# MinChoi0129/StreamMOS

Hardware: AMD Instinct MI355X
Metric: LiDAR scans/sec (StreamMOS streaming inference + voxel voting) (higher is better)
Workload: dtype f32; 1 GPU; configs[1]: full StreamMOS streaming inference, 1 sequence per GPU, B=4 TTA x T=3 x N=160000 padded points (120k-point synthetic HDL-64E scans), 8-frame voxel voting on; tta=4, frame_point_num=160000, parallelism=sequence-shard x1, padding_tail=point head skipped (logits zero)

## Files before the change

include/smos.h:

```cpp
#ifndef SMOS_H_
#define SMOS_H_

#include <stdint.h>

#ifdef __cplusplus
extern "C" {
#endif

#define SMOS_ABI_VERSION 4

enum smos_status {
  SMOS_OK = 0,
  SMOS_ERR_ARG = 1,
  SMOS_ERR_UNSUPPORTED = 2,
  SMOS_ERR_LAUNCH = 3
};

enum smos_dtype { SMOS_F32 = 0, SMOS_F16 = 1, SMOS_F64 = 2 };

typedef void* smos_stream_t;

int smos_abi_version(void);
const char* smos_last_error(void);
int smos_debug_set_conv_grid_cap(int32_t blocks);

int smos_voxel_maxpool_fwd(const void* feat, const int64_t* feat_stride, const void* ind, void* out,
                           const int64_t* out_stride, int64_t* voxel_max_idx, int64_t BS, int64_t C,
                           int64_t N, int32_t D, const int64_t* out_size, const float* scale,
                           int32_t dtype, int32_t* flag_ws, smos_stream_t stream);

int smos_voxel_maxpool_bwd(const void* feat, const int64_t* feat_stride, const void* ind, const void* out,
                           const void* grad_out, const int64_t* out_stride, void* grad_feat, int64_t BS,
                           int64_t C, int64_t N, int32_t D, const int64_t* out_size, const float* scale,
                           int32_t dtype, smos_stream_t stream);

int smos_bilinear_gather_fwd(const float* grid, const int64_t* grid_stride, const float* coord, int32_t K,
                             float* out, const int64_t* out_stride, int64_t B, int64_t C, int64_t H,
                             int64_t W, int64_t N, const float* scale, smos_stream_t stream);

int smos_bilinear_gather_bwd(const float* grad_out, const int64_t* grad_out_stride, const float* coord, int32_t K,
                             float* grad_grid, const int64_t* grad_grid_stride, int64_t B, int64_t C, int64_t H,
                             int64_t W, int64_t N, const float* scale, smos_stream_t stream);

int32_t smos_segsum_chunk(void);
int64_t smos_bilinear_gather_bwd_det_work_bytes(int64_t B, int64_t C, int64_t H, int64_t W, int64_t N);
int smos_bilinear_gather_bwd_det(const float* grad_out, const int64_t* grad_out_stride, const float* coord, int32_t K,
                                 float* grad_grid, const int64_t* grad_grid_stride, int64_t B, int64_t C, int64_t H,
                                 int64_t W, int64_t N, const float* scale, void* work, int64_t work_bytes,
                                 smos_stream_t stream);

int smos_gather_scatter_train_fwd(const float* grid, const int64_t* grid_stride, const float* gcoord, int32_t Kg,
                                  const float* gscale, const float* scoord, int32_t Ks, const float* sscale, float* out,
                                  const int64_t* out_stride, float* pts, const int64_t* pts_stride, int64_t B, int64_t C,
                                  int64_t Hg, int64_t Wg, int64_t N, int64_t Ho, int64_t Wo, int32_t* flag_ws,
                                  smos_stream_t stream);

int smos_gather_scatter_train_bwd(const float* grid, const int64_t* grid_stride, const float* gcoord, int32_t Kg,
                                  const float* gscale, const float* scoord, int32_t Ks, const float* sscale, const float* out,
                                  const int64_t* out_stride, const float* grad_out, const int64_t* grad_out_stride,
                                  const float* grad_pts, const int64_t* grad_pts_stride, float* grad_grid,
                                  const int64_t* grad_grid_stride, int64_t B, int64_t C, int64_t Hg, int64_t Wg, int64_t N,
                                  int64_t Ho, int64_t Wo, smos_stream_t stream);

int smos_gather_scatter_train_point_grad(const float* grid, const int64_t* grid_stride, const float* gcoord, int32_t Kg,
                                         const float* gscale, const float* scoord, int32_t Ks, const float* sscale,
                                         const float* out, const int64_t* out_stride, const float* grad_out,
                                         const int64_t* grad_out_stride, const float* grad_pts, const int64_t* grad_pts_stride,
                                         float* x, const int64_t* x_stride, int64_t B, int64_t C, int64_t Hg, int64_t Wg,
                                         int64_t N, int64_t Ho, int64_t Wo, smos_stream_t stream);

int32_t smos_seg_loss_tile(void);
int64_t smos_seg_loss_work_bytes(int64_t n, int32_t C);
int smos_seg_loss_fwd(const float* pred, const int64_t* pred_stride, const int64_t* target, int64_t B, int32_t C,
                      int64_t P, int64_t k, float top_weight, float lovasz_weight, int64_t ignore_index, float* coef,
                      float* loss, float* stats, void* work, int64_t work_bytes, smos_stream_t stream);
int smos_seg_loss_bwd(const float* pred, const int64_t* pred_stride, const int64_t* target, const float* coef,
                      const float* stats, const float* grad_out, int64_t B, int32_t C, int64_t P, int64_t k,
                      float top_weight, float lovasz_weight, int64_t ignore_index, float* grad,
                      const int64_t* grad_stride, smos_stream_t stream);

int smos_msda_fwd(const void* value, const int64_t* spatial_shapes, const int64_t* level_start_index,
                  const void* sampling_loc, const void* attn_weight, void* out, int64_t N, int64_t S,
                  int64_t M, int64_t D, int64_t L, int64_t Lq, int64_t P, int32_t dtype,
                  smos_stream_t stream);

int smos_tta_argmax(const float* pred, int64_t B, int64_t K, int64_t N, uint8_t* labels, float* prob,
                    smos_stream_t stream);

#define SMOS_VOTE_NX 512
#define SMOS_VOTE_NY 512
#define SMOS_VOTE_NZ 30
#define SMOS_VOTE_CELLS (512LL * 512LL * 30LL)

int smos_vote_clear(uint64_t* table, smos_stream_t stream);
int smos_vote_accumulate(const float* pts, int64_t n, int64_t pt_stride, const uint8_t* labels,
                         const double* pose_diff, int32_t recip_quantize, uint64_t* table,
                         smos_stream_t stream);
int smos_vote_accumulate_frames(int32_t count, const float* const* pts, const int64_t* n, const int64_t* pt_stride,
                                const uint8_t* const* labels, const double* const* pose_diff, int32_t recip_quantize,
                                uint64_t* table, smos_stream_t stream);
int smos_vote_resolve(const float* pts, int64_t n, int64_t pt_stride, const uint8_t* labels,
                      int32_t recip_quantize, const uint64_t* table, const int32_t* lut,
                      int32_t* out_labels, smos_stream_t stream);

int64_t smos_dbscan_work_bytes(int64_t n);
int smos_dbscan(const float* pts, int64_t n, int64_t pt_stride, double eps, int32_t min_samples, int32_t* labels,
                void* work, int64_t work_bytes, int32_t max_sweeps, smos_stream_t stream);
int smos_box_vote(const float* pts, int64_t n, int64_t pt_stride, const uint8_t* labels, const double* pose_diff,
                  const float* boxes, int32_t K, uint32_t* counts, smos_stream_t stream);

int64_t smos_instance_work_bytes(int64_t n);
int smos_instance_cluster(const float* pts, int64_t n, int64_t pt_stride, const uint8_t* bf, double eps,
                          int32_t min_samples, int32_t min_points, float floor_lift, int32_t max_boxes, int32_t* names,
                          float* boxes, int32_t* slot_of, int32_t* k_dev, int32_t* status, void* work, int64_t work_bytes,
                          smos_stream_t stream);
int smos_box_vote_dev(int32_t count, const float* const* pts, const int64_t* n, const int64_t* pt_stride,
                      const uint8_t* const* labels, const double* const* pose_diff, const float* boxes,
                      const int32_t* k_dev, int32_t max_boxes, uint32_t* counts, smos_stream_t stream);
int smos_instance_apply(const int32_t* names, const int32_t* slot_of, const uint32_t* counts, const int32_t* k_dev,
                        int32_t max_boxes, int32_t* labels, int64_t n, smos_stream_t stream);

int smos_pointnet_scatter(const float* xyzi, const float* coord, int32_t K, const float* w1, const float* b1,
                          const float* w2, const float* b2, float* bev, float* pts_out, int64_t po_b, int64_t po_n,
                          int64_t B, int64_t T, int64_t N, int64_t H, int64_t W, int32_t cin, int32_t cmid,
                          int32_t cout, smos_stream_t stream);
int64_t smos_stem_scan_state_words(int64_t cells);
int smos_stem_mark(const float* coord, int32_t K, int64_t B, int64_t T, int64_t N, int64_t H, int64_t W, int32_t* flags,
                   uint64_t* scan_state, smos_stream_t stream);
int smos_stem_scan(int32_t* flags, int64_t B, int64_t H, int64_t W, uint64_t* scan_state, int32_t* row_cell, int32_t* row_of,
                   int32_t* meta, float* rows, int64_t row_floats, smos_stream_t stream);
int smos_stem_gemm(const float* bev, const int32_t* row_cell, const int32_t* meta, const float* const* wprep4, float* const* y4,
                   int64_t Cin, int64_t Cout, smos_stream_t stream);
int smos_stem_epilogue(const float* const* y4, const int32_t* meta, const int32_t* row_of, const float* bias, float* out,
                       int64_t out_pitch, int64_t B, int64_t H, int64_t W, int64_t C, smos_stream_t stream);
int smos_msda_fwd_qp(const float* value, const float* qp, float* out, int64_t N, int64_t H, int64_t W, int64_t M, int64_t D,
                     int64_t P, smos_stream_t stream);

int smos_tfusion_project(int32_t n_jobs, const float* const* x, const int64_t* x_pitch, const float* const* wstream,
                         const float* const* bias, float* const* out, const int64_t* out_pitch, const int64_t* cout,
                         const int64_t* tokens, smos_stream_t stream);
int64_t smos_tfusion_layer_param_floats(int64_t ffn);
int64_t smos_tfusion_layer_stream_floats(int64_t ffn, int32_t has_next);
int smos_tfusion_layer(const float* sampled, const float* query, int64_t q_pitch, const float* wstream, const float* params,
                       float* out, int64_t o_pitch, float* qp_next, int64_t nq, int64_t tokens, int64_t ffn, float eps1,
                       float eps2, smos_stream_t stream);

int smos_tap_products_bf16x3(int32_t n_jobs, const float* const* x, const int64_t* x_pitch, const void* const* wlimbs,
                             float* const* out, const int64_t* out_pitch, const int64_t* cout, const int64_t* tokens,
                             smos_stream_t stream);

int smos_add_layer_norm(const float* x, const float* res, const float* gamma, const float* beta, float* out, int64_t rows,
                        int64_t C, float eps, smos_stream_t stream);

int64_t smos_conv_cl_sum_chunks(int64_t Ho, int64_t Wo);
int smos_conv_rows_cl(const float* x, int64_t x_pitch, const float* wprep, const float* bias, const float* res, int64_t res_pitch,
                      float* out, int64_t out_pitch, int64_t B, int64_t H, int64_t W, int64_t Cin, int64_t Cout, int32_t KH,
                      int32_t KW, int32_t mt, int32_t act, float* chan_sums, smos_stream_t stream);
int smos_conv_cl(const float* x, int64_t x_pitch, const float* wprep, const float* bias, const float* res, int64_t res_pitch,
                 float* out, int64_t out_pitch, int64_t B, int64_t H, int64_t W, int64_t Cin, int64_t Cout, int32_t KH,
                 int32_t KW, int32_t stride, int32_t pad_h, int32_t pad_w, int32_t mt, int32_t act, float* chan_sums,
                 smos_stream_t stream);
int smos_conv_bf16_cl_supported(int64_t Cin, int64_t Cout, int32_t KH, int32_t KW, int32_t stride, int32_t has_res);
int smos_conv_bf16_cl(const float* x, int64_t x_pitch, const uint16_t* wprep, const float* bias, const float* res,
                      int64_t res_pitch, float* out, int64_t out_pitch, int64_t B, int64_t H, int64_t W, int64_t Cin,
                      int64_t Cout, int32_t KH, int32_t KW, int32_t stride, int32_t pad_h, int32_t pad_w, int32_t act,
                      float* chan_sums, smos_stream_t stream);
int64_t smos_conv_wino_sum_chunks(int64_t H, int64_t W);
int smos_conv_wino_cl(const float* x, int64_t x_pitch, const float* wprep, const float* bias, const float* res, int64_t res_pitch,
                      float* out, int64_t out_pitch, int64_t B, int64_t H, int64_t W, int64_t Cin, int64_t Cout, int32_t mb,
                      int32_t act, float* chan_sums, smos_stream_t stream);

int smos_conv_wino1d_cl(const float* x, int64_t x_pitch, const float* wprep, const float* bias, float* out, int64_t out_pitch,
                        int64_t B, int64_t H, int64_t W, int64_t Cin, int64_t Cout, int64_t KH, int64_t KW, int32_t mb, int32_t act,
                        smos_stream_t stream);

int smos_upconv_xy_ok(int64_t Hs, int64_t Ho);
int smos_upconv_xy(const float* conv_a, int64_t a_pitch, const float* bias, const float* z1, int64_t H1, int64_t W1, const float* z2,
                   int64_t H2, int64_t W2, float* out, int64_t out_pitch, int64_t B, int64_t Ho, int64_t Wo, int64_t C, int32_t act,
                   smos_stream_t stream);
int smos_upconv_xy_units(const float* conv_a, int64_t a_pitch, const float* bias, const float* z1, int64_t H1, int64_t W1,
                         const float* z2, int64_t H2, int64_t W2, float* out, int64_t out_pitch, int64_t B, int64_t Ho, int64_t Wo,
                         int64_t C, int32_t act, int32_t strip, int64_t max_blocks, smos_stream_t stream);
int smos_upconv_xpass(const float* z, float* t, int64_t B, int64_t Hs, int64_t Ws, int64_t C, int64_t Wo, smos_stream_t stream);
int smos_upconv_ypass(const float* conv_a, int64_t a_pitch, const float* bias, const float* t1, int64_t H1, const float* t2,
                      int64_t H2, float* out, int64_t out_pitch, int64_t B, int64_t Ho, int64_t Wo, int64_t C, int32_t act,
                      smos_stream_t stream);
int smos_upconv_bwd_window(int64_t n_src, int64_t n_dst);
int smos_upconv_bwd_ypass(const float* g, int64_t g_pitch, float* s, int64_t B, int64_t Ho, int64_t Wo, int64_t C, int64_t Hs,
                          int64_t max_blocks, smos_stream_t stream);
int smos_upconv_bwd_xpass(const float* s, float* gz, int64_t gz_pitch, int64_t B, int64_t Hs, int64_t Ws, int64_t C, int64_t Wo,
                          int64_t max_blocks, smos_stream_t stream);

int64_t smos_point_head_weight_floats(void);
int smos_point_head(const float* rows, int64_t row_pitch, const float* wprep, float* out, int64_t B, int64_t N, int64_t K1,
                    int64_t M1, int64_t M2, int64_t M3, const int32_t* n_live, smos_stream_t stream);

int smos_point_head_gather(const float* rows, int64_t row_pitch, const float* wprep, float* out, int64_t B, int64_t N,
                           int64_t K1, int64_t M1, int64_t M2, int64_t M3, const int32_t* n_live, const float* grid,
                           int64_t grid_pitch, int64_t Hg, int64_t Wg, const float* gcoord, int32_t Kg,
                           int64_t g_batch_stride, const float* gscale, smos_stream_t stream);

int smos_pointnet_scatter_rows(const float* xyzi, const float* coord, int32_t K, const float* w1, const float* b1,
                               const float* w2, const float* b2, float* rows, const int32_t* row_of, float* pts_out,
                               int64_t po_b, int64_t po_n, int64_t B, int64_t T, int64_t N, int64_t H, int64_t W, int32_t cin,
                               int32_t cmid, int32_t cout, const int32_t* n_live, smos_stream_t stream);

int smos_prep_transform_mask(const float* scan, int64_t n, const double* pose_diff, const double* range6, float* moved,
                             int32_t* mask, smos_stream_t stream);
int smos_prep_emit(const float* moved, const int32_t* mask, const int32_t* prefix, int64_t n, int32_t t, int32_t T, int64_t N,
                   int32_t V, const float* tta_sx, const float* tta_sy, const double* range6, const int64_t* bev_size3,
                   const double* rv4, float* xyzi, float* coord, float* sphere, smos_stream_t stream);
int smos_prep_unpad_labels(const uint8_t* labels, int64_t N, const int32_t* mask, const int32_t* prefix, int64_t n,
                           uint8_t* raw, smos_stream_t stream);

int64_t smos_train_prep_work_bytes(int64_t n_max);
int smos_train_prep_build(const void* const* scans, const void* const* label_words, const int64_t* n, const double* first_pose,
                          const double* second_pose, const double* range6, const int64_t* bev_size3, const double* rv4,
                          int64_t N, const uint32_t* words, const double* noise, uint64_t seed, uint64_t sample_index,
                          double noise_mean, double noise_std, const double* shift3, double scale, int32_t v_flip,
                          int32_t h_flip, double rot_cos, double rot_sin, const int32_t* lut, int32_t n_maps, int32_t lut_len,
                          void* const* xyzi, void* const* coord, void* const* sphere, void* const* targets, void* const* bev,
                          int32_t* counts, void* work, int64_t work_bytes, smos_stream_t stream);
int smos_train_prep_draws(uint64_t seed, uint64_t sample_index, int64_t N, double noise_mean, double noise_std,
                          uint32_t* words, double* noise, smos_stream_t stream);

int64_t smos_copy_paste_work_bytes(int64_t n0);
int smos_copy_paste_begin(const void* const* scans, const void* const* label_words, const int64_t* n, const double* first_pose,
                          int64_t slots, int32_t count, void* pts, void* words, void* angles, void* flags, int32_t* status,
                          smos_stream_t stream);
int smos_copy_paste_object(const void* scan0, const void* label_words0, const double* first_pose0, const int64_t* n, int64_t slots,
                           void* pts, void* words, void* angles, void* flags, int32_t* status, int32_t count, int32_t number,
                           const void* object_points, int32_t m, int64_t slot, const double* footprint, const double* shift_x5,
                           const double* shift_y5, const uint8_t* order20, const double* cos20, const double* sin20,
                           const double* noise, uint64_t seed, uint64_t sample_index, uint32_t paste_word, void* work,
                           int64_t work_bytes, smos_stream_t stream);
int smos_copy_paste_draws(uint64_t seed, uint64_t sample_index, int32_t number, int32_t m, double* noise, smos_stream_t stream);

int smos_msda_bwd(const void* grad_out, const void* value, const int64_t* spatial_shapes, const int64_t* level_start_index,
                  const void* sampling_loc, const void* attn_weight, void* grad_value, void* grad_sampling_loc,
                  void* grad_attn_weight, int64_t N, int64_t S, int64_t M, int64_t D, int64_t L, int64_t Lq, int64_t P,
                  int32_t dtype, smos_stream_t stream);

int64_t smos_msda_bwd_det_work_bytes(int64_t N, int64_t S, int64_t M, int64_t D, int64_t L, int64_t Lq, int64_t P);
int smos_msda_bwd_det(const float* grad_out, const float* value, const int64_t* spatial_shapes, const int64_t* level_start_index,
                      const float* sampling_loc, const float* attn_weight, float* grad_value, float* grad_sampling_loc,
                      float* grad_attn_weight, int64_t N, int64_t S, int64_t M, int64_t D, int64_t L, int64_t Lq, int64_t P,
                      void* work, int64_t work_bytes, smos_stream_t stream);

int smos_bias_act_cl(const float* x, int64_t x_pitch, const float* bias, const float* res, int64_t res_pitch, float* out,
                     int64_t out_pitch, int64_t P, int64_t C, int32_t act, smos_stream_t stream);
int smos_downsample_epilogue_cl(const float* a, int64_t a_pitch, const float* p, int64_t p_pitch, const float* bias, float* out,
                                int64_t out_pitch, int64_t B, int64_t C, int64_t H, int64_t W, int32_t stride,
                                smos_stream_t stream);
int smos_channel_gate_residual_cl(const float* y, int64_t y_pitch, const float* bias, const float* w1, const float* b1,
                                  const float* w2, const float* b2, const float* xres, int64_t res_pitch, float* out,
                                  int64_t out_pitch, float* ws, int64_t ws_floats, int64_t B, int64_t C, int64_t Cr, int64_t HW,
                                  smos_stream_t stream);
int smos_channel_gate_apply_cl(const float* y, int64_t y_pitch, const float* bias, const float* w1, const float* b1,
                               const float* w2, const float* b2, const float* xres, int64_t res_pitch, float* out,
                               int64_t out_pitch, const float* chan_sums, int64_t chunks, float* gate_ws, int64_t B, int64_t C,
                               int64_t Cr, int64_t HW, smos_stream_t stream);
int64_t smos_basic_block_ws_floats(int64_t B, int64_t H, int64_t W, int64_t C);
int smos_basic_block_cl(const float* x, int64_t x_pitch, const float* u1, const float* b1, const float* u2, const float* b2,
                        const float* gw1, const float* gb1, const float* gw2, const float* gb2, int64_t Cr, float* y,
                        int64_t y_pitch, float* out, int64_t out_pitch, float* ws, int64_t B, int64_t H, int64_t W, int64_t C,
                        int32_t mb, smos_stream_t stream);
int smos_unbalance_block_cl(const float* x, int64_t x_pitch, const float* ua, const float* ba, int64_t kha, int64_t kwa,
                            const float* ub, const float* bb, int64_t khb, int64_t kwb, const float* uc, const float* bc,
                            float* both, int64_t both_pitch, float* out, int64_t out_pitch, int64_t B, int64_t H, int64_t W,
                            int64_t C, int32_t mb, smos_stream_t stream);
int smos_zero_views_cl(int32_t n, float* const* ptrs, const int64_t* rows, const int64_t* row_floats, const int64_t* pitches,
                       smos_stream_t stream);
int smos_upsample_concat_cl(const float* const* src, const int64_t* src_c, const int64_t* src_h, const int64_t* src_w,
                            const int64_t* src_pitch, int32_t n_src, float* out, int64_t B, int64_t Ho, int64_t Wo,
                            smos_stream_t stream);
int smos_downsample_pool_branch(const float* x, int64_t x_pitch, const float* wpairs, const float* a, int64_t a_pitch,
                                const float* bias, float* out, int64_t out_pitch, int64_t B, int64_t H, int64_t W, int64_t Cin,
                                int64_t Cout, int32_t stride, smos_stream_t stream);
int smos_gather_scatter_cl(const float* grid, int64_t grid_pitch, const float* gcoord, int32_t Kg, int64_t g_batch_stride,
                           const float* gscale, const float* scoord, int32_t Ks, int64_t s_batch_stride, const float* sscale,
                           float* out, int64_t out_pitch, float* pts_out, int64_t po_b, int64_t po_n, int64_t B, int64_t C,
                           int64_t Hg, int64_t Wg, int64_t N, int64_t Ho, int64_t Wo, const int32_t* n_live,
                           smos_stream_t stream);

int smos_label_words(const uint8_t* labels, int64_t n, int32_t lut, int32_t* words, const uint32_t* gt, const int32_t* gt_map,
                     int32_t map_n, uint64_t* counts, smos_stream_t stream);
int smos_label_count_voted(const int32_t* voted, int64_t n, int32_t* words, const uint32_t* gt, const int32_t* gt_map,
                           int32_t map_n, uint64_t* counts, smos_stream_t stream);

int32_t smos_point_mlp_chunk(void);
int32_t smos_point_mlp_fold_floats(void);
int32_t smos_point_mlp_stat_doubles(void);
int64_t smos_point_mlp_work_bytes(int64_t P);
int smos_point_mlp_fwd(const float* x, int64_t S, int64_t N, int32_t training, const void* const* params, const double* eps_mom,
                       float* y, float* fold, double* dstat, void* work, int64_t work_bytes, smos_stream_t stream);
int smos_point_mlp_bwd(const float* x, const float* grad_y, int64_t S, int64_t N, int32_t training, const void* const* params,
                       const double* eps_mom, const float* fold, const double* dstat, void* const* grads, void* work,
                       int64_t work_bytes, smos_stream_t stream);

int32_t smos_point_head_train_chunk(void);
int32_t smos_point_head_train_fold_floats(void);
int32_t smos_point_head_train_stat_doubles(void);
int64_t smos_point_head_train_work_bytes(int64_t P);
int64_t smos_point_head_train_mask_words(int64_t P);
int smos_point_head_train_masks(const uint8_t* keep1, const uint8_t* keep2, const int64_t* seed, int64_t B, int64_t N,
                                uint32_t* masks, smos_stream_t stream);
int smos_point_head_train_fwd(const float* a, const float* b, const float* c, const int64_t* pitch, const uint32_t* masks,
                              double scale, int64_t B, int64_t N, int32_t training, const void* const* params,
                              const double* eps_mom, float* logits, float* fold, double* dstat, void* work, int64_t work_bytes,
                              smos_stream_t stream);
int smos_point_head_train_bwd(const float* a, const float* b, const float* c, const int64_t* pitch, const uint32_t* masks,
                              double scale, const float* grad_logits, int64_t B, int64_t N, int32_t training, const float* fold,
                              void* const* grads, void* work, int64_t work_bytes, smos_stream_t stream);

#ifdef __cplusplus
}
#endif
#endif
```

profiles/kinds.py:

```python
KIND = (
    (("conv_igemm", "conv_rows", "conv_wino"), "conv_cl[", 1),
    (("conv_bf16",), "conv_bf16[", 1),
    (("gather_scatter_cl",), "gather_scatter_cl[", 1),
    (("pointnet_scatter",), "pointnet_scatter[", 1),
    (("point_head",), "point_head[", 1),
    (("stem_gemm",), "stem_gemm[", 1),
    (("stem_epilogue",), "stem_epilogue[", 1),
    (("upconv_xpass",), "upconv_xpass[", 1),
    (("upconv_ypass", "upconv_fused"), "upconv_ypass[", 1),
    (("upconv_xy",), "upconv_xy[", 1),
    (("msda_fwd",), "msda_fwd[", 1),
    (("pool_branch",), "downsample_pool_branch[", 1),
    (("tfusion_layer",), "tfusion_layer[", 1),
    (("tfusion_project", "tap_bf16x3"), "tfusion_project[", 1),
    (("stem_mark", "stem_scan"), "stem_mark+scan[", 2),
)


def steady_step(rows, key):
    rows = sorted(rows, key=key)
    marks = [i for i, r in enumerate(rows) if "tta_argmax" in r["Kernel_Name"]]
    if len(marks) < 2:
        return rows
    return rows[marks[-2] + 1:marks[-1] + 1]


def match(step, labels):
    used, pairs, problems = set(), [], []
    for frags, prefix, per in KIND:
        want = [l for l in labels if l.startswith(prefix)]
        have = [i for i, r in enumerate(step) if any(f in r["Kernel_Name"] for f in frags)]
        if len(want) * per != len(have):
            if want or have:
                problems.append("%d dispatches of %s vs %d labels x %d" % (len(have), "/".join(frags), len(want), per))
            continue
        for k, l in enumerate(want):
            idx = have[k * per:(k + 1) * per]
            used.update(idx)
            pairs.append((l, [step[i] for i in idx]))
    for i, r in enumerate(step):
        if i not in used:
            pairs.append((None, [r]))
    return pairs, problems
```

profiles/label_durations.py:

```python
import collections
import csv
import json
import os
import sys

sys.path.insert(0, os.path.dirname(os.path.dirname(os.path.abspath(__file__))))
sys.path.insert(0, os.path.dirname(os.path.abspath(__file__)))
import kinds

import bench

rows = list(csv.DictReader(open(sys.argv[1])))
labels = json.load(open(sys.argv[2]))
ctx = {}
if len(sys.argv) > 3:
    try:
        line = json.loads(open(sys.argv[3]).read().strip().splitlines()[-1])
        if line.get("stem_rows_per_launch") is not None:
            ctx["stem_rows"] = line["stem_rows_per_launch"]
        if line.get("stem_class_rows"):
            ctx["stem_class_rows"] = line["stem_class_rows"]
        if line.get("live_fraction") is not None:
            ctx["live_fraction"] = line["live_fraction"]
    except (OSError, ValueError, IndexError):
        pass
step = kinds.steady_step(rows, key=lambda r: int(r["Start_Timestamp"]))
pairs, problems = kinds.match(step, labels)
for p in problems:
    sys.stderr.write("label_durations: %s -- left unlabelled\n" % p)
def family_of(label, kernel_name):
    for frag in ("conv_wino1d", "conv_wino", "conv_igemm", "conv_rows"):
        if frag in kernel_name:
            return frag
    return label.split("[", 1)[0] if label else kernel_name.split("(")[0].split("<")[0][:60]


agg = collections.OrderedDict()
for label, disp in pairs:
    name = label if label else disp[0]["Kernel_Name"].split("(")[0][:90]
    d = sum(int(r["End_Timestamp"]) - int(r["Start_Timestamp"]) for r in disp) / 1e3
    a = agg.setdefault(name, [0, 0.0, label is not None, family_of(label, disp[0]["Kernel_Name"])])
    a[0] += 1
    a[1] += d
w = csv.writer(sys.stdout)
w.writerow(["label", "family", "launches_per_step", "mean_us", "total_us", "alg_flops", "exec_flops", "alg_bytes", "bound", "achieved",
            "unit", "frac", "alg_frac"])
total = 0.0
fams = collections.OrderedDict()
for name, (n, us, labelled, fam) in sorted(agg.items(), key=lambda kv: -kv[1][1]):
    total += us
    mean = us / n
    fl = by = ex = 0
    if labelled:
        try:
            fl, by = bench.algorithmic_flops(name, ctx), bench.algorithmic_bytes(name, ctx)
            ex = bench.executed_launch_flops(name, ctx=ctx, family=fam)
        except (ValueError, KeyError, IndexError):
            pass
    f = fams.setdefault(fam, [0, 0.0, 0.0, 0.0, 0.0, labelled])
    f[0] += n
    f[1] += us
    f[2] += n * fl
    f[3] += n * ex
    f[4] += n * by
    t_m, t_h = ex / (bench.FP32_PEAK_TFLOPS * 1e12), by / (bench.HBM_PEAK_GBS * 1e9)
    if ex and t_m > t_h:
        ach = ex / (mean * 1e-6) / 1e12
        w.writerow([name, fam, n, "%.2f" % mean, "%.1f" % us, fl, ex, by, "mfma", "%.1f" % ach, "TFLOP/s", "%.4f" % (ach / bench.FP32_PEAK_TFLOPS),
                    "%.4f" % (fl / (mean * 1e-6) / 1e12 / bench.FP32_PEAK_TFLOPS)])
    elif by:
        ach = by / (mean * 1e-6) / 1e9
        w.writerow([name, fam, n, "%.2f" % mean, "%.1f" % us, fl, ex, by, "hbm", "%.1f" % ach, "GB/s", "%.4f" % (ach / bench.HBM_PEAK_GBS), ""])
    else:
        w.writerow([name, fam, n, "%.2f" % mean, "%.1f" % us, "", "", "", "", "", "", "", ""])
w.writerow(["# kernels of the step: %d, summed %.1f us" % (len(step), total)])
w.writerow(["# per kernel family (launches, us, FLOPs and bytes are sums over the step; frac as bench.py's roofline object computes it)"])
for fam, (n, us, fl, ex, by, labelled) in sorted(fams.items(), key=lambda kv: -kv[1][1]):
    t_m, t_h = ex / (bench.FP32_PEAK_TFLOPS * 1e12), by / (bench.HBM_PEAK_GBS * 1e9)
    if ex and t_m > t_h:
        ach = ex / (us * 1e-6) / 1e12
        w.writerow(["family:" + fam, fam, n, "%.2f" % (us / n), "%.1f" % us, int(fl), int(ex), int(by), "mfma", "%.1f" % ach, "TFLOP/s",
                    "%.4f" % (ach / bench.FP32_PEAK_TFLOPS), "%.4f" % (fl / (us * 1e-6) / 1e12 / bench.FP32_PEAK_TFLOPS)])
    elif by:
        ach = by / (us * 1e-6) / 1e9
        w.writerow(["family:" + fam, fam, n, "%.2f" % (us / n), "%.1f" % us, int(fl), int(ex), int(by), "hbm", "%.1f" % ach, "GB/s",
                    "%.4f" % (ach / bench.HBM_PEAK_GBS), ""])
    else:
        w.writerow(["family:" + fam, fam, n, "%.2f" % (us / n), "%.1f" % us, "", "", "", "", "", "", "", ""])
```

streammos_amd/_lib.py:

```python
import ctypes
import os

_PKG = os.path.dirname(os.path.abspath(__file__))
LIB_PATH = os.environ.get("SMOS_HIP_LIB") or os.path.join(_PKG, "lib", "libsmos_hip.so")

c_i64p = ctypes.POINTER(ctypes.c_int64)
c_f32p = ctypes.POINTER(ctypes.c_float)
c_f64p = ctypes.POINTER(ctypes.c_double)
vp = ctypes.c_void_p
i64 = ctypes.c_int64
i32 = ctypes.c_int32

SIGNATURES = {
    "smos_abi_version": [],
    "smos_debug_set_conv_grid_cap": [i32],
    "smos_voxel_maxpool_fwd": [vp, c_i64p, vp, vp, c_i64p, vp, i64, i64, i64, i32, c_i64p, c_f32p, i32, vp, vp],
    "smos_voxel_maxpool_bwd": [vp, c_i64p, vp, vp, vp, c_i64p, vp, i64, i64, i64, i32, c_i64p, c_f32p, i32, vp],
    "smos_bilinear_gather_fwd": [vp, c_i64p, vp, i32, vp, c_i64p, i64, i64, i64, i64, i64, c_f32p, vp],
    "smos_bilinear_gather_bwd": [vp, c_i64p, vp, i32, vp, c_i64p, i64, i64, i64, i64, i64, c_f32p, vp],
    "smos_segsum_chunk": [],
    "smos_bilinear_gather_bwd_det_work_bytes": [i64, i64, i64, i64, i64],
    "smos_bilinear_gather_bwd_det": [vp, c_i64p, vp, i32, vp, c_i64p, i64, i64, i64, i64, i64, c_f32p, vp, i64, vp],
    "smos_gather_scatter_train_fwd": [vp, c_i64p, vp, i32, c_f32p, vp, i32, c_f32p, vp, c_i64p, vp, c_i64p, i64, i64, i64, i64, i64, i64, i64, vp, vp],
    "smos_gather_scatter_train_bwd": [vp, c_i64p, vp, i32, c_f32p, vp, i32, c_f32p, vp, c_i64p, vp, c_i64p, vp, c_i64p, vp, c_i64p,
                                      i64, i64, i64, i64, i64, i64, i64, vp],
    "smos_gather_scatter_train_point_grad": [vp, c_i64p, vp, i32, c_f32p, vp, i32, c_f32p, vp, c_i64p, vp, c_i64p, vp, c_i64p, vp, c_i64p,
                                             i64, i64, i64, i64, i64, i64, i64, vp],
    "smos_seg_loss_tile": [],
    "smos_seg_loss_work_bytes": [i64, i32],
    "smos_seg_loss_fwd": [vp, c_i64p, vp, i64, i32, i64, i64, ctypes.c_float, ctypes.c_float, i64, vp, vp, vp, vp, i64, vp],
    "smos_seg_loss_bwd": [vp, c_i64p, vp, vp, vp, vp, i64, i32, i64, i64, ctypes.c_float, ctypes.c_float, i64, vp, c_i64p, vp],
    "smos_msda_fwd": [vp, vp, vp, vp, vp, vp, i64, i64, i64, i64, i64, i64, i64, i32, vp],
    "smos_msda_bwd": [vp, vp, vp, vp, vp, vp, vp, vp, vp, i64, i64, i64, i64, i64, i64, i64, i32, vp],
    "smos_msda_bwd_det_work_bytes": [i64, i64, i64, i64, i64, i64, i64],
    "smos_msda_bwd_det": [vp, vp, vp, vp, vp, vp, vp, vp, vp, i64, i64, i64, i64, i64, i64, i64, vp, i64, vp],
    "smos_tta_argmax": [vp, i64, i64, i64, vp, vp, vp],
    "smos_vote_clear": [vp, vp],
    "smos_vote_accumulate": [vp, i64, i64, vp, c_f64p, i32, vp, vp],
    "smos_vote_accumulate_frames": [i32, ctypes.POINTER(vp), c_i64p, c_i64p, ctypes.POINTER(vp), ctypes.POINTER(c_f64p), i32, vp, vp],
    "smos_vote_resolve": [vp, i64, i64, vp, i32, vp, vp, vp, vp],
    "smos_dbscan_work_bytes": [i64],
    "smos_dbscan": [vp, i64, i64, ctypes.c_double, i32, vp, vp, i64, i32, vp],
    "smos_box_vote": [vp, i64, i64, vp, c_f64p, vp, i32, vp, vp],
    "smos_instance_work_bytes": [i64],
    "smos_instance_cluster": [vp, i64, i64, vp, ctypes.c_double, i32, i32, ctypes.c_float, i32, vp, vp, vp, vp, vp, vp, i64, vp],
    "smos_box_vote_dev": [i32, ctypes.POINTER(vp), c_i64p, c_i64p, ctypes.POINTER(vp), ctypes.POINTER(c_f64p), vp, vp, i32, vp, vp],
    "smos_instance_apply": [vp, vp, vp, vp, i32, vp, i64, vp],
    "smos_pointnet_scatter": [vp, vp, i32, vp, vp, vp, vp, vp, vp, i64, i64, i64, i64, i64, i64, i64, i32, i32, i32, vp],
    "smos_stem_scan_state_words": [i64],
    "smos_stem_mark": [vp, i32, i64, i64, i64, i64, i64, vp, vp, vp],
    "smos_stem_scan": [vp, i64, i64, i64, vp, vp, vp, vp, vp, i64, vp],
    "smos_stem_gemm": [vp, vp, vp, ctypes.POINTER(vp), ctypes.POINTER(vp), i64, i64, vp],
    "smos_stem_epilogue": [ctypes.POINTER(vp), vp, vp, vp, vp, i64, i64, i64, i64, i64, vp],
    "smos_pointnet_scatter_rows": [vp, vp, i32, vp, vp, vp, vp, vp, vp, vp, i64, i64, i64, i64, i64, i64, i64, i32, i32, i32, vp, vp],
    "smos_point_head_weight_floats": [],
    "smos_point_head": [vp, i64, vp, vp, i64, i64, i64, i64, i64, i64, vp, vp],
    "smos_point_head_gather": [vp, i64, vp, vp, i64, i64, i64, i64, i64, i64, vp, vp, i64, i64, i64, vp, i32, i64, c_f32p, vp],
    "smos_conv_cl_sum_chunks": [i64, i64],
    "smos_conv_cl": [vp, i64, vp, vp, vp, i64, vp, i64, i64, i64, i64, i64, i64, i32, i32, i32, i32, i32, i32, i32, vp, vp],
    "smos_conv_rows_cl": [vp, i64, vp, vp, vp, i64, vp, i64, i64, i64, i64, i64, i64, i32, i32, i32, i32, vp, vp],
    "smos_conv_bf16_cl_supported": [i64, i64, i32, i32, i32, i32],
    "smos_conv_bf16_cl": [vp, i64, vp, vp, vp, i64, vp, i64, i64, i64, i64, i64, i64, i32, i32, i32, i32, i32, i32, vp, vp],
    "smos_conv_wino_sum_chunks": [i64, i64],
    "smos_conv_wino_cl": [vp, i64, vp, vp, vp, i64, vp, i64, i64, i64, i64, i64, i64, i32, i32, vp, vp],
    "smos_basic_block_ws_floats": [i64, i64, i64, i64],
    "smos_basic_block_cl": [vp, i64, vp, vp, vp, vp, vp, vp, vp, vp, i64, vp, i64, vp, i64, vp, i64, i64, i64, i64, i32, vp],
    "smos_unbalance_block_cl": [vp, i64, vp, vp, i64, i64, vp, vp, i64, i64, vp, vp, vp, i64, vp, i64, i64, i64, i64, i64, i32, vp],
    "smos_zero_views_cl": [i32, ctypes.POINTER(vp), c_i64p, c_i64p, c_i64p, vp],
    "smos_msda_fwd_qp": [vp, vp, vp, i64, i64, i64, i64, i64, i64, vp],
    "smos_add_layer_norm": [vp, vp, vp, vp, vp, i64, i64, ctypes.c_float, vp],
    "smos_tfusion_project": [i32, ctypes.POINTER(vp), c_i64p, ctypes.POINTER(vp), ctypes.POINTER(vp), ctypes.POINTER(vp), c_i64p, c_i64p, c_i64p, vp],
    "smos_tfusion_layer_param_floats": [i64],
    "smos_tfusion_layer_stream_floats": [i64, i32],
    "smos_tfusion_layer": [vp, vp, i64, vp, vp, vp, i64, vp, i64, i64, i64, ctypes.c_float, ctypes.c_float, vp],
    "smos_tap_products_bf16x3": [i32, ctypes.POINTER(vp), c_i64p, ctypes.POINTER(vp), ctypes.POINTER(vp), c_i64p, c_i64p, c_i64p, vp],
    "smos_conv_wino1d_cl": [vp, i64, vp, vp, vp, i64, i64, i64, i64, i64, i64, i64, i64, i32, i32, vp],
    "smos_upconv_xpass": [vp, vp, i64, i64, i64, i64, i64, vp],
    "smos_upconv_ypass": [vp, i64, vp, vp, i64, vp, i64, vp, i64, i64, i64, i64, i64, i32, vp],
    "smos_upconv_xy_ok": [i64, i64],
    "smos_upconv_xy": [vp, i64, vp, vp, i64, i64, vp, i64, i64, vp, i64, i64, i64, i64, i64, i32, vp],
    "smos_upconv_xy_units": [vp, i64, vp, vp, i64, i64, vp, i64, i64, vp, i64, i64, i64, i64, i64, i32, i32, i64, vp],
    "smos_upconv_bwd_window": [i64, i64],
    "smos_upconv_bwd_ypass": [vp, i64, vp, i64, i64, i64, i64, i64, i64, vp],
    "smos_upconv_bwd_xpass": [vp, vp, i64, i64, i64, i64, i64, i64, i64, vp],
    "smos_prep_transform_mask": [vp, i64, c_f64p, c_f64p, vp, vp, vp],
    "smos_prep_emit": [vp, vp, vp, i64, i32, i32, i64, i32, c_f32p, c_f32p, c_f64p, c_i64p, c_f64p, vp, vp, vp, vp],
    "smos_prep_unpad_labels": [vp, i64, vp, vp, i64, vp, vp],
    "smos_train_prep_work_bytes": [i64],
    "smos_train_prep_build": [ctypes.POINTER(vp), ctypes.POINTER(vp), c_i64p, c_f64p, c_f64p, c_f64p, c_i64p, c_f64p, i64, vp, vp,
                              ctypes.c_uint64, ctypes.c_uint64, ctypes.c_double, ctypes.c_double, c_f64p, ctypes.c_double, i32, i32,
                              ctypes.c_double, ctypes.c_double, vp, i32, i32, ctypes.POINTER(vp), ctypes.POINTER(vp),
                              ctypes.POINTER(vp), ctypes.POINTER(vp), ctypes.POINTER(vp), vp, vp, i64, vp],
    "smos_train_prep_draws": [ctypes.c_uint64, ctypes.c_uint64, i64, ctypes.c_double, ctypes.c_double, vp, vp, vp],
    "smos_copy_paste_work_bytes": [i64],
    "smos_copy_paste_begin": [ctypes.POINTER(vp), ctypes.POINTER(vp), c_i64p, c_f64p, i64, i32, vp, vp, vp, vp, vp, vp],
    "smos_copy_paste_object": [vp, vp, c_f64p, c_i64p, i64, vp, vp, vp, vp, vp, i32, i32, vp, i32, i64, vp, c_f64p, c_f64p,
                               ctypes.POINTER(ctypes.c_uint8), c_f64p, c_f64p, vp, ctypes.c_uint64, ctypes.c_uint64, ctypes.c_uint32,
                               vp, i64, vp],
    "smos_copy_paste_draws": [ctypes.c_uint64, ctypes.c_uint64, i32, i32, vp, vp],
    "smos_bias_act_cl": [vp, i64, vp, vp, i64, vp, i64, i64, i64, i32, vp],
    "smos_downsample_epilogue_cl": [vp, i64, vp, i64, vp, vp, i64, i64, i64, i64, i64, i32, vp],
    "smos_channel_gate_residual_cl": [vp, i64, vp, vp, vp, vp, vp, vp, i64, vp, i64, vp, i64, i64, i64, i64, i64, vp],
    "smos_channel_gate_apply_cl": [vp, i64, vp, vp, vp, vp, vp, vp, i64, vp, i64, vp, i64, vp, i64, i64, i64, i64, vp],
    "smos_upsample_concat_cl": [ctypes.POINTER(vp), c_i64p, c_i64p, c_i64p, c_i64p, i32, vp, i64, i64, i64, vp],
    "smos_downsample_pool_branch": [vp, i64, vp, vp, i64, vp, vp, i64, i64, i64, i64, i64, i64, i32, vp],
    "smos_gather_scatter_cl": [vp, i64, vp, i32, i64, c_f32p, vp, i32, i64, c_f32p, vp, i64, vp, i64, i64, i64, i64, i64, i64, i64, i64, i64, vp, vp],
    "smos_label_words": [vp, i64, i32, vp, vp, vp, i32, vp, vp],
    "smos_label_count_voted": [vp, i64, vp, vp, vp, i32, vp, vp],
    "smos_point_mlp_chunk": [],
    "smos_point_mlp_fold_floats": [],
    "smos_point_mlp_stat_doubles": [],
    "smos_point_mlp_work_bytes": [i64],
    "smos_point_mlp_fwd": [vp, i64, i64, i32, ctypes.POINTER(vp), c_f64p, vp, vp, vp, vp, i64, vp],
    "smos_point_mlp_bwd": [vp, vp, i64, i64, i32, ctypes.POINTER(vp), c_f64p, vp, vp, ctypes.POINTER(vp), vp, i64, vp],
    "smos_point_head_train_chunk": [],
    "smos_point_head_train_fold_floats": [],
    "smos_point_head_train_stat_doubles": [],
    "smos_point_head_train_work_bytes": [i64],
    "smos_point_head_train_mask_words": [i64],
    "smos_point_head_train_masks": [vp, vp, vp, i64, i64, vp, vp],
    "smos_point_head_train_fwd": [vp, vp, vp, c_i64p, vp, ctypes.c_double, i64, i64, i32, ctypes.POINTER(vp), c_f64p, vp, vp, vp, vp, i64, vp],
    "smos_point_head_train_bwd": [vp, vp, vp, c_i64p, vp, ctypes.c_double, vp, i64, i64, i32, vp, ctypes.POINTER(vp), vp, i64, vp],
}

INT64_RESULTS = (
    "smos_bilinear_gather_bwd_det_work_bytes", "smos_seg_loss_work_bytes", "smos_msda_bwd_det_work_bytes", "smos_dbscan_work_bytes",
    "smos_instance_work_bytes", "smos_stem_scan_state_words", "smos_point_head_weight_floats", "smos_conv_cl_sum_chunks",
    "smos_conv_wino_sum_chunks", "smos_basic_block_ws_floats", "smos_tfusion_layer_param_floats", "smos_tfusion_layer_stream_floats",
    "smos_train_prep_work_bytes", "smos_copy_paste_work_bytes", "smos_point_mlp_work_bytes",
    "smos_point_head_train_work_bytes", "smos_point_head_train_mask_words",
)

ABI_VERSION = 4

_lib = None


def load():
    global _lib
    if _lib is not None:
        return _lib
    if not os.path.isfile(LIB_PATH):
        raise RuntimeError(
            "streammos_amd: %s is missing -- the HIP kernels are not built. Run "
            "`python -m streammos_amd.build` (or __graft_entry__.build()). There is no CPU fallback." % LIB_PATH)
    import torch
    bundled = os.path.join(os.path.dirname(torch.__file__), "lib", "libamdhip64.so")
    if os.path.isfile(bundled):
        ctypes.CDLL(bundled, mode=ctypes.RTLD_GLOBAL)
    lib = ctypes.CDLL(LIB_PATH)
    lib.smos_abi_version.argtypes = []
    lib.smos_abi_version.restype = ctypes.c_int
    have = lib.smos_abi_version()
    if have != ABI_VERSION:
        raise RuntimeError("streammos_amd: %s has ABI version %d, this package binds version %d -- rebuild it "
                           "(`python -m streammos_amd.build -f`)" % (LIB_PATH, have, ABI_VERSION))
    for name, argtypes in SIGNATURES.items():
        fn = getattr(lib, name, None)
        if fn is None:
            raise RuntimeError("streammos_amd: %s has no %s -- it was built from an older tree; rebuild it "
                               "(`python -m streammos_amd.build -f`)" % (LIB_PATH, name))
        fn.argtypes = argtypes
        fn.restype = ctypes.c_int64 if name in INT64_RESULTS else ctypes.c_int
    lib.smos_last_error.argtypes = []
    lib.smos_last_error.restype = ctypes.c_char_p
    _lib = lib
    return lib


def check(rc, what):
    if rc != 0:
        msg = load().smos_last_error().decode(errors="replace")
        raise RuntimeError("%s failed (smos status %d): %s" % (what, rc, msg))


def entry(name):
    return getattr(_lib or load(), name)


def call(name, *args):
    rc = getattr(_lib or load(), name)(*args)
    if rc:
        check(rc, name)


def query(name, *args):
    return int(getattr(_lib or load(), name)(*args))


def i64_array(values):
    return (ctypes.c_int64 * len(values))(*[int(v) for v in values])


def f32_array(values):
    return (ctypes.c_float * len(values))(*[float(v) for v in values])


def f64_array(values):
    return (ctypes.c_double * len(values))(*[float(v) for v in values])
```

streammos_amd/csrc/blocks.hip:

```cpp
#include "smos_common.h"

extern "C" int64_t smos_basic_block_ws_floats(int64_t B, int64_t H, int64_t W, int64_t C) {
  return B * C * (smos_conv_wino_sum_chunks(H, W) + 1);
}

extern "C" int smos_basic_block_cl(const float* x, int64_t x_pitch, const float* u1, const float* b1, const float* u2,
                                   const float* b2, const float* gw1, const float* gb1, const float* gw2, const float* gb2,
                                   int64_t Cr, float* y, int64_t y_pitch, float* out, int64_t out_pitch, float* ws, int64_t B,
                                   int64_t H, int64_t W, int64_t C, int32_t mb, smos_stream_t stream) {
  SMOS_REQUIRE(x && u1 && u2 && y && out && y != out && x != y, "basic_block_cl: null pointer, or y aliases x / out");
  int rc = smos_conv_wino_cl(x, x_pitch, u1, b1, nullptr, 0, y, y_pitch, B, H, W, C, C, mb,  1, nullptr, stream);
  if (rc) return rc;
  if (!gw1)
    return smos_conv_wino_cl(y, y_pitch, u2, b2, x, x_pitch, out, out_pitch, B, H, W, C, C, mb, 1, nullptr, stream);
  SMOS_REQUIRE(gb1 && gw2 && gb2 && b2 && ws && Cr > 0 && x != out, "basic_block_cl: gate parameters / scratch missing, or out aliases x");
  const int64_t chunks = smos_conv_wino_sum_chunks(H, W);
  rc = smos_conv_wino_cl(y, y_pitch, u2, nullptr, nullptr, 0, out, out_pitch, B, H, W, C, C, mb,  0, ws, stream);
  if (rc) return rc;
  return smos_channel_gate_apply_cl(out, out_pitch, b2, gw1, gb1, gw2, gb2, x, x_pitch, out, out_pitch, ws, chunks,
                                    ws + B * chunks * C, B, C, Cr, H * W, stream);
}

extern "C" int smos_unbalance_block_cl(const float* x, int64_t x_pitch, const float* ua, const float* ba, int64_t kha, int64_t kwa,
                                       const float* ub, const float* bb, int64_t khb, int64_t kwb, const float* uc, const float* bc,
                                       float* both, int64_t both_pitch, float* out, int64_t out_pitch, int64_t B, int64_t H,
                                       int64_t W, int64_t C, int32_t mb, smos_stream_t stream) {
  SMOS_REQUIRE(x && ua && ub && uc && both && out && both != out && x != both && x != out && both_pitch >= 2 * C,
               "unbalance_block_cl: null pointer, aliasing maps, or `both` narrower than 2 C channels");
  int rc = smos_conv_wino1d_cl(x, x_pitch, ua, ba, both, both_pitch, B, H, W, C, C, kha, kwa, mb, 1, stream);
  if (rc) return rc;
  rc = smos_conv_wino1d_cl(x, x_pitch, ub, bb, both + C, both_pitch, B, H, W, C, C, khb, kwb, mb, 1, stream);
  if (rc) return rc;
  return smos_conv_wino_cl(both, both_pitch, uc, bc, x, x_pitch, out, out_pitch, B, H, W, 2 * C, C, mb, 1, nullptr, stream);
}
```

streammos_amd/engine.py:

```python
import itertools
import os

import torch
import torch.nn.functional as F

from . import ops, profiling, scratch

RELU, LEAKY, NONE = ops.ACT_RELU, ops.ACT_LEAKY, ops.ACT_NONE
_gated_tags = itertools.count()


def _fold(conv_w, conv_b, bn, pre=None):
    w = conv_w.detach().double()
    b = conv_b.detach().double() if conv_b is not None else torch.zeros(w.shape[0], dtype=torch.float64, device=w.device)
    if pre is not None:
        s_in = pre.weight.detach().double() / torch.sqrt(pre.running_var.detach().double() + pre.eps)
        o_in = pre.bias.detach().double() - pre.running_mean.detach().double() * s_in
        b = b + (w.flatten(2).sum(2) * o_in[None, :]).sum(1)
        w = w * s_in[None, :, None, None]
    if bn is not None:
        s = bn.weight.detach().double() / torch.sqrt(bn.running_var.detach().double() + bn.eps)
        w = w * s[:, None, None, None]
        b = (b - bn.running_mean.detach().double()) * s + bn.bias.detach().double()
    return w.float().contiguous(memory_format=torch.channels_last), b.float().contiguous()


def _block_call(eng):
    return eng.block_call and eng.own_conv and eng.wino and not profiling.enabled()


class DownBlock:
    kind = "down"
    __slots__ = ("wa", "wp", "bias", "stride", "pool_ok", "pool_pack")

    def __init__(self, m):
        self.wa, ba = _fold(m.conv_branch[0].weight, None, m.conv_branch[1])
        self.wp, bp = _fold(m.pool_branch[0].weight, None, m.pool_branch[1])
        self.bias = (ba + bp).contiguous()
        self.stride = m.conv_branch[0].stride[0]
        cout, cin = self.wp.shape[0], self.wp.shape[1]
        self.pool_ok = cin <= 64 and ops.pool_branch_ok(cin, cout, self.stride)
        self.pool_pack = None

    def run(self, eng, x, out=None):
        a = eng._conv(x, self.wa, None, NONE, stride=self.stride)
        if (self.pool_ok and eng.pool_fused and eng.own_conv and
                x.shape[0] * x.shape[2] * x.shape[3] * x.stride(3) * 4 < (1 << 31)):
            if self.pool_pack is None:
                self.pool_pack = ops.pool_branch_prepare(self.wp)
            return ops.downsample_pool_branch(x, self.pool_pack, a, self.bias, self.stride, out=out if out is not None else a)
        q = eng._conv(x, self.wp, None, NONE)
        return ops.downsample_epilogue_cl(a, q, self.bias, self.stride, out=out if out is not None else a)


class UnbalanceBlock:
    kind = "unbalance"
    __slots__ = ("wa", "ba", "pa", "wb", "bb", "pb", "wc", "bc", "plan_ok", "plan")

    def __init__(self, m):
        self.wa, self.ba = _fold(m.layer7x3[0].weight, None, m.layer7x3[1])
        self.wb, self.bb = _fold(m.layer3x7[0].weight, None, m.layer3x7[1])
        self.wc, self.bc = _fold(m.layer3x3[0].weight, None, m.layer3x3[1])
        self.pa, self.pb = m.layer7x3[0].padding, m.layer3x7[0].padding
        c = self.wa.shape[0]
        self.plan_ok = (c % 16 == 0 and tuple(self.wa.shape[:2]) == (c, c) and tuple(self.wb.shape[:2]) == (c, c) and
                        tuple(self.wc.shape) == (c, 2 * c, 3, 3) and ops.conv_wino1d_ok(tuple(self.wa.shape[2:]), 1, c, c) and
                        ops.conv_wino1d_ok(tuple(self.wb.shape[2:]), 1, c, c))
        self.plan = None

    def run(self, eng, x, out=None):
        if self.plan_ok and _block_call(eng) and eng.wino1d and 2 * x.numel() <= (1 << 26):
            if self.plan is None:
                self.plan = ops.UnbalanceBlockPlan(self.wa, self.ba, self.wb, self.bb, self.wc, self.bc)
            return ops.unbalance_block_cl(x, self.plan, out=out)
        b, c, h, w = x.shape
        both = ops.empty_cl(b, 2 * c, h, w, x.device)
        eng._conv(x, self.wa, self.ba, RELU, out=both[:, :c])
        eng._conv(x, self.wb, self.bb, RELU, out=both[:, c:])
        return eng._conv(both, self.wc, self.bc, RELU, residual=x, out=out)


class BasicBlock:
    kind = "basic"
    __slots__ = ("w1", "b1", "w2", "b2", "att", "cw1", "cb1", "cw2", "cb2", "plan_ok", "plan", "tag")

    def __init__(self, m):
        self.w1, self.b1 = _fold(m.layer[0].weight, None, m.layer[1])
        self.w2, self.b2 = _fold(m.layer[3].weight, None, m.layer[4])
        self.att = m.use_att
        self.cw1 = self.cb1 = self.cw2 = self.cb2 = None
        if m.use_att:
            c1, c2 = m.channel_att.cnet[1], m.channel_att.cnet[3]
            self.cw1 = c1.weight.detach().reshape(c1.weight.shape[0], -1).contiguous()
            self.cb1 = c1.bias.detach().contiguous()
            self.cw2 = c2.weight.detach().reshape(c2.weight.shape[0], -1).contiguous()
            self.cb2 = c2.bias.detach().contiguous()
        c = self.w1.shape[0]
        self.plan_ok = tuple(self.w1.shape) == (c, c, 3, 3) and tuple(self.w2.shape) == (c, c, 3, 3) and ops.basic_block_ok(c, self.att)
        self.plan = None
        self.tag = next(_gated_tags) if m.use_att else None

    def run(self, eng, x, out=None):
        if (self.plan_ok and _block_call(eng) and (eng.fused_gate_sums or not self.att) and x.numel() <= (1 << 26)):
            if self.plan is None:
                self.plan = ops.BasicBlockPlan(self.w1, self.b1, self.w2, self.b2,
                                               (self.cw1, self.cb1, self.cw2, self.cb2) if self.att else None)
            ws = None
            if self.att:
                bsz, c, h, w = x.shape
                ws = eng._block_ws(self, bsz * c * (ops.conv_wino_sum_chunks(h, w) + 1))
            return ops.basic_block_cl(x, self.plan, out=out, ws=ws)
        y = eng._conv(x, self.w1, self.b1, RELU)
        if not self.att:
            return eng._conv(y, self.w2, self.b2, RELU, residual=x, out=out)
        bsz, c, h, w = y.shape
        k2 = tuple(self.w2.shape[2:])
        if (eng.own_conv and eng.fused_gate_sums and ops.gate_channels_ok(c) and ops.conv_cl_supported(y, c, k2) and
                (not eng._bf16 or ops.conv_bf16_ok(y, c, k2, chan_sums=True))):
            family = "bf16" if eng._bf16 else ops.conv_route(c, c, k2, 1, bsz * h * w, False, True, eng)[0]
            chunks = ops.conv_wino_sum_chunks(h, w) if family == "wino" else ops.conv_sum_chunks(h, w)
            ws = eng._block_ws(self, bsz * c * (chunks + 1))
            sums = ws[:bsz * chunks * c].view(bsz, chunks, c)
            y2 = eng._conv(y, self.w2, None, NONE, chan_sums=sums)
            return ops.channel_gate_apply_cl(y2, self.b2, self.cw1, self.cb1, self.cw2, self.cb2, x, sums, ws[bsz * chunks * c:],
                                             out=out if out is not None else y2)
        y2 = eng._conv(y, self.w2, None, NONE)
        need = (y2.shape[2] * y2.shape[3] // 512 + 2) * y2.shape[0] * y2.shape[1]
        return ops.channel_gate_residual_cl(y2, self.b2, self.cw1, self.cb1, self.cw2, self.cb2, x, eng._block_ws(self, need),
                                            out=out if out is not None else y2)


class FusionLayer:
    __slots__ = ("heads", "points", "value", "qproj", "out", "norm1", "lin1", "lin2", "norm2", "tf", "wv_stream", "wq_stream")

    def __init__(self, lyr):
        ca = lyr.cross_attn
        self.heads, self.points = ca.n_heads, ca.n_points
        self.value = (ca.value_proj.weight.detach(), ca.value_proj.bias.detach())
        self.qproj = (torch.cat((ca.sampling_offsets.weight.detach(), ca.attention_weights.weight.detach()), 0).contiguous(),
                      torch.cat((ca.sampling_offsets.bias.detach(), ca.attention_weights.bias.detach()), 0).contiguous())
        self.out = (ca.output_proj.weight.detach(), ca.output_proj.bias.detach())
        self.norm1 = (lyr.norm1.weight.detach(), lyr.norm1.bias.detach(), lyr.norm1.eps)
        self.lin1 = (lyr.linear1.weight.detach(), lyr.linear1.bias.detach())
        self.lin2 = (lyr.linear2.weight.detach(), lyr.linear2.bias.detach())
        self.norm2 = (lyr.norm2.weight.detach(), lyr.norm2.bias.detach(), lyr.norm2.eps)
        self.tf = self.wv_stream = self.wq_stream = None


CONV_PRECISIONS = ("fp32", "bf16")

SWITCHES = (
    ("sparse_stem", "SMOS_SPARSE_STEM", True, "bool"),
    ("tfusion", "SMOS_TFUSION", True, "bool"),
    ("upconv", "SMOS_UPCONV", True, "bool"),
    ("fused_head", "SMOS_FUSED_HEAD", True, "bool"),
    ("head_gather", "SMOS_HEAD_GATHER", True, "bool"),
    ("own_conv", "SMOS_OWN_CONV", True, "bool"),
    ("conv_rows_mt", "SMOS_CONV_ROWS_MT", 1, "int"),
    ("conv_rows", "SMOS_CONV_ROWS", 3, "int"),
    ("fused_gate_sums", "SMOS_GATE_SUMS", True, "bool"),
    ("wino", "SMOS_WINO", True, "bool"),
    ("wino1d", "SMOS_WINO1D", True, "bool"),
    ("pool_fused", "SMOS_POOL_FUSED", True, "bool"),
    ("block_call", "SMOS_BLOCK_CALL", True, "bool"),
)

TRAIN_SWITCHES = (
    ("seg_loss_own", "SMOS_SEG_LOSS", True, "bool"),
)


def read_switches(obj, table):
    for attr, var, default, kind in table:
        v = os.environ.get(var)
        v = ops.env_on(v) if kind == "bool" else (None if v is None else int(v))
        setattr(obj, attr, default if v is None else v)


class InferenceEngine:
    def __init__(self, net, layout="cl", conv_precision="fp32"):
        if layout != "cl":
            raise ValueError("layout=%r: the NCHW engine was removed, 'cl' (channels-last) is the only layout" % (layout,))
        if conv_precision not in CONV_PRECISIONS:
            raise ValueError("conv_precision must be one of %s, got %r" % (CONV_PRECISIONS, conv_precision))
        self.layout = layout
        self.conv_precision = conv_precision
        self._bf16 = conv_precision == "bf16"
        self._conv_layers = {}
        self.scratch = scratch.Table()
        self.device = next(net.parameters()).device
        read_switches(self, SWITCHES)
        if self._bf16:
            self.block_call = False
        self.bev_hw = tuple(net.bev_wl_shape)
        enc = net.bev_net

        l0, l1 = net.point_pre.layer[0].layer, net.point_pre.layer[1].layer
        self.pp1 = _fold(l0[1].weight, None, l0[2], pre=l0[0])
        self.pp2 = _fold(l1[0].weight, None, l1[1])

        self.header_bev = [self._block(m) for m in enc.header_bev]
        self.stem_w = None
        p0 = self.header_bev[0]
        if (p0.kind == "down" and p0.stride == 2 and p0.wa.shape[0] == 32 and p0.wa.shape[1] == 192 and
                tuple(p0.wa.shape[2:]) == (3, 3)):
            self.stem_w = ops.stem_prepare_weights(p0.wa, p0.wp)
        self.header_rv = [self._block(m) for m in enc.header_rv]
        self.res1_bev = [self._block(m) for m in enc.res1_bev]
        self.res1_rv = [self._block(m) for m in enc.res1_rv]
        self.res2 = [self._block(m) for m in enc.res2]

        self.query_embed = enc.query_embed.weight.detach()
        self.layers = [FusionLayer(lyr) for lyr in enc.deformattn_module.deformattn_layers]

        self._tf_ok = False
        try:
            for i, L in enumerate(self.layers):
                nxt = self.layers[i + 1].qproj if i + 1 < len(self.layers) else None
                L.tf = ops.TfusionLayer(L.out, L.norm1, L.lin1, L.lin2, L.norm2, next_qproj=nxt)
                L.wv_stream = ops.tfusion_pack_linear(L.value[0])
                L.wq_stream = ops.tfusion_pack_linear(L.qproj[0]) if i == 0 else None
            self._tf_ok = all(L.value[0].shape[0] // L.heads == 32 and L.points <= 8 and L.qproj[0].shape[0] % 4 == 0 for L in self.layers)
        except RuntimeError:
            self._tf_ok = False

        self.conv_1 = _fold(enc.conv_1.conv.weight, None, enc.conv_1.bn)
        self.conv_2 = _fold(enc.conv_2.conv.weight, None, enc.conv_2.bn)
        heads = (enc.aux_head1, enc.aux_head2, enc.aux_head3)
        ncls = heads[0].weight.shape[0]
        cin = [h.weight.shape[1] for h in heads]
        w = torch.zeros((3 * ncls, sum(cin), 1, 1), device=self.device)
        off = 0
        for i, h in enumerate(heads):
            w[i * ncls:(i + 1) * ncls, off:off + cin[i]] = h.weight.detach()
            off += cin[i]
        self.aux = (w.contiguous(), torch.cat([h.bias.detach() for h in heads]).contiguous(), ncls)
        self.grid2point_scale = tuple(net.bev_grid2point.scale_rate)
        w1 = self.conv_1[0]
        self.conv_1a = w1[:, :cin[0]].contiguous(memory_format=torch.channels_last)
        self.conv_1z = (ops.upconv_tap_weights(w1, cin[0], cin[0] + cin[1]), ops.upconv_tap_weights(w1, cin[0] + cin[1], sum(cin)))
        self.aux_split = [(h.weight.detach().contiguous(), h.bias.detach().contiguous()) for h in heads]

        m = net.point_post.merge_layer
        self.post1 = _fold(m[0].weight, None, m[1])
        self.post2 = _fold(m[3].weight, None, m[4])
        p = net.pred_layer.pred_layer[0]
        self.pred = (p.weight.detach().contiguous(), p.bias.detach().contiguous())
        self.refine = None
        if hasattr(net, "refine"):
            rm = net.refine.bf_point_post.merge_layer
            rp = net.refine.bf_pred_layer.pred_layer[0]
            self.refine = (_fold(rm[0].weight, None, rm[1]), _fold(rm[3].weight, None, rm[4]),
                           (rp.weight.detach().contiguous(), rp.bias.detach().contiguous()))
        self.head_w = self.refine_w = None
        try:
            self.head_w = ops.point_head_prepare(self.post1, self.post2, self.pred)
            if self.refine is not None:
                self.refine_w = ops.point_head_prepare(*self.refine)
        except RuntimeError:
            self.head_w = self.refine_w = None
        self._shapes = None
        self._lsi = None
        self._hw = None
        self.miopen_search = True

    def _block(self, m):
        from .refapi.networks import backbone as bb
        from .refapi.networks import multi_view_encoder as mve
        for cls, module in ((DownBlock, bb.DownSample2D), (UnbalanceBlock, mve.Unbalance_BasicBlock), (BasicBlock, bb.BasicBlock)):
            if isinstance(m, module):
                return cls(m)
        raise RuntimeError("InferenceEngine: unexpected module %s" % type(m).__name__)

    @staticmethod
    def _linear_relu(x, wb):
        w = wb[0].view(wb[0].shape[0], -1)
        try:
            return torch._addmm_activation(wb[1], x, w.t(), use_gelu=False)
        except (RuntimeError, AttributeError):
            return torch.relu_(torch.addmm(wb[1], x, w.t()))

    def _head_gathers(self, fuse, bev_feat, o1, o2):
        return (self.head_gather and self.fused_head and self.head_w is not None and self.refine is None
                and (o1, o2) == (64, 128) and fuse.shape[2] == 192 and fuse.stride(1) % 4 == 0
                and bev_feat.data_ptr() % 16 == 0 and bev_feat.stride(3) % 4 == 0)

    def _point_heads(self, fuse, aux, k, x2, n_live=None, gather=None):
        bs, n = fuse.shape[0], fuse.shape[1]
        rows = fuse.view(bs * n, -1)
        a3 = tuple(aux) if isinstance(aux, (tuple, list)) else (aux[:, :k], aux[:, k:2 * k], aux[:, 2 * k:])

        def head(l1, l2, pr, fused):
            if self.fused_head and fused is not None and fuse.stride(1) % 4 == 0:
                return ops.point_head(fuse, fused[0], fused[1], n_live=n_live, gather=gather).unsqueeze(-1)
            if gather is not None:
                raise RuntimeError("InferenceEngine: the BEV rows were left to the fused point head, which does not run")
            z = self._linear_relu(self._linear_relu(rows, l1), l2)
            out = torch.addmm(pr[1], z, pr[0].view(pr[0].shape[0], -1).t())
            return out.view(bs, n, -1).permute(0, 2, 1).contiguous().unsqueeze(-1)

        pred = head(self.post1, self.post2, self.pred, self.head_w)
        if self.refine is not None:
            return (pred, head(*self.refine, self.refine_w)) + a3 + (x2,)
        return (pred,) + a3 + (x2,)

    def _block_ws(self, p, n_floats):
        return self.scratch.get(p.tag, (n_floats,), torch.float32, self.device, zero=True)

    @staticmethod
    def _add_norm(a, b, norm, c):
        if c in (64, 128, 256, 512):
            return ops.add_layer_norm(a.contiguous(), b.contiguous(), norm[0], norm[1], norm[2] if len(norm) > 2 else 1e-5)
        return F.layer_norm(a + b, (c,), norm[0], norm[1], norm[2] if len(norm) > 2 else 1e-5)

    def _temporal_fusion(self, x2, memory):
        b, c, hh, ww = x2.shape
        dev = x2.device
        if self._shapes is None or self._hw != (hh, ww):
            self._hw = (hh, ww)
            self._shapes = torch.tensor([[hh, ww]], dtype=torch.long, device=dev)
            self._lsi = torch.zeros((1,), dtype=torch.long, device=dev)
            ys = (torch.arange(hh, dtype=torch.float32, device=dev) + 0.5) / hh
            xs = (torch.arange(ww, dtype=torch.float32, device=dev) + 0.5) / ww
            self._ref = torch.stack((xs[None, :].expand(hh, ww), ys[:, None].expand(hh, ww)), -1).reshape(1, hh * ww, 1, 1, 1, 2)
            self._norm = torch.tensor([ww, hh], dtype=torch.float32, device=dev)
        src = x2.permute(0, 2, 3, 1).reshape(b, hh * ww, c)
        if memory is None:
            query = self.query_embed.unsqueeze(0).expand(b, -1, -1)
        else:
            query = memory.permute(0, 2, 3, 1).reshape(b, hh * ww, c)
        lq = hh * ww
        if self.tfusion and self._tf_ok and c == 128:
            query = query if query.is_contiguous() else query.contiguous()
            jobs = [(src, L.wv_stream, L.value[1]) for L in self.layers] + [(query, self.layers[0].wq_stream, self.layers[0].qproj[1])]
            outs = []
            for k in range(0, len(jobs), 8):
                outs += ops.tfusion_project(jobs[k:k + 8])
            qp = outs[-1]
            for i, L in enumerate(self.layers):
                sampled = ops.msda_fwd_qp(outs[i].view(b, lq, L.heads, 32), qp.view(b, lq, -1), hh, ww, L.points)
                query, qp = ops.tfusion_layer(sampled, query, L.tf)
            return query.view(b, hh, ww, c).permute(0, 3, 1, 2)
        for L in self.layers:
            h, p = L.heads, L.points
            value = F.linear(src, *L.value).view(b, lq, h, c // h)
            qp = F.linear(query, *L.qproj)
            if c // h == 32 and p <= 8:
                sampled = ops.msda_fwd_qp(value.contiguous(), qp.contiguous(), hh, ww, p)
            else:
                off = qp[..., :h * p * 2].reshape(b, lq, h, 1, p, 2)
                attn = F.softmax(qp[..., h * p * 2:].reshape(b, lq, h, p), -1).view(b, lq, h, 1, p)
                loc = (self._ref + off / self._norm).contiguous()
                sampled = ops.msda_fwd(value.contiguous(), self._shapes, self._lsi, loc, attn.contiguous())
            query = self._add_norm(query, F.linear(sampled, *L.out), L.norm1, c)
            ffn = F.linear(self._linear_relu(query.view(b * lq, c), L.lin1).view(b, lq, -1), *L.lin2)
            query = self._add_norm(query, ffn, L.norm2, c)
        return query.contiguous().view(b, hh, ww, c).permute(0, 3, 1, 2)

    @torch.no_grad()
    def stage_forward(self, point_feat, pcds_coord, pcds_sphere_coord, memory=None):
        return self.decode(self.encode(point_feat, pcds_coord, pcds_sphere_coord), memory)

    def _conv_flags(self):
        if self.own_conv:
            return ops._NO_GUARD
        return torch.backends.cudnn.flags(enabled=True, benchmark=self.miopen_search)

    def encode(self, point_feat, pcds_coord, pcds_sphere_coord, n_live=None):
        with torch.no_grad(), self._conv_flags():
            return self._encode_cl(point_feat, pcds_coord, pcds_sphere_coord, n_live)

    def decode(self, enc, memory=None, want_aux=True, n_live=None):
        return self.decode_heads(enc, self.decode_memory(enc, memory), want_aux, n_live)

    def decode_memory(self, enc, memory=None):
        with torch.no_grad(), self._conv_flags():
            return self._temporal_fusion(self._stage_cl(enc["x1cat"], self.res2), memory)

    def decode_heads(self, enc, x2, want_aux=True, n_live=None):
        with torch.no_grad(), self._conv_flags():
            return self._decode_cl(enc, x2, want_aux, n_live)

    def conv_precision_stats(self):
        ran = [layer.ran_bf16 for layer in self._conv_layers.values() if layer.ran_bf16 is not None]
        return {"bf16": sum(ran), "fallback": len(ran) - sum(ran)}

    def _conv_layer(self, w):
        layer = self._conv_layers.get(id(w))
        if layer is None:
            layer = self._conv_layers[id(w)] = ops.ConvLayer(w)
        return layer

    def _conv(self, x, w, bias, act, stride=1, residual=None, out=None, chan_sums=None):
        cout, cin, kh, kw = w.shape
        layer = self._conv_layer(w)
        if self._bf16:
            layer.ran_bf16 = self.own_conv and ops.conv_bf16_ok(x, cout, (kh, kw), stride, residual, out, chan_sums)
            if layer.ran_bf16:
                return ops.conv_bf16_cl(x, layer.operand("bf16"), bias, act, cout, (kh, kw), stride=stride, residual=residual,
                                        out=out, chan_sums=chan_sums)
        easy = (cin % 32 == 0 and cout % 32 == 0 and cout <= 4 * cin and kh <= 7 and kw <= 7 and (stride == 1 or stride == 2) and
                x.numel() <= (1 << 26))
        if not self.own_conv or not (easy or ops.conv_cl_supported(x, cout, (kh, kw), stride, residual, out)):
            if chan_sums is not None:
                raise RuntimeError("InferenceEngine._conv: channel sums need the own conv kernel")
            y = F.conv2d(x, w, None, stride, (kh // 2, kw // 2))
            if bias is None and act == NONE and residual is None and out is None:
                return y
            return ops.bias_act_cl(y, bias, act, out=out if out is not None else y, residual=residual)
        b, _, h, wd = x.shape
        ho, wo = (h + 2 * (kh // 2) - kh) // stride + 1, (wd + 2 * (kw // 2) - kw) // stride + 1
        route = ops.conv_route(cin, cout, (kh, kw), stride, b * ho * wo, residual is not None, chan_sums is not None, self)
        family, tile = route
        wp = layer.operand(route)
        if family == "wino":
            return ops.conv_wino_cl(x, wp, bias, act, cout, mb=tile, residual=residual, out=out, chan_sums=chan_sums)
        if family == "wino1d":
            return ops.conv_wino1d_cl(x, wp, bias, act, cout, (kh, kw), mb=tile, out=out)
        if family == "rows":
            return ops.conv_rows_cl(x, wp, bias, act, cout, (kh, kw), mt=tile, residual=residual, out=out, chan_sums=chan_sums)
        return ops.conv_cl(x, wp, bias, act, cout, (kh, kw), stride=stride, mt=tile, residual=residual, out=out, chan_sums=chan_sums)

    def _block_cl(self, x, p, out=None):
        return p.run(self, x, out)

    def _stage_cl(self, x, blocks, out=None):
        for i, p in enumerate(blocks):
            x = p.run(self, x, out if i == len(blocks) - 1 else None)
        return x

    def _cross_view_cl(self, cat_buf, c, bev_xy, sphere, rv_blocks, rv_hw, scale, point_rows=None, n_live=None, rv=None):
        b = cat_buf.shape[0]
        back = cat_buf[:, c:]
        if rv is None:
            rv = ops.empty_cl(b, c, rv_hw[0], rv_hw[1], cat_buf.device)
            ops.zero_views_cl([rv, back])
        ops.gather_scatter_cl(cat_buf[:, :c], bev_xy, scale, sphere, scale, out=rv)
        rv = self._stage_cl(rv, rv_blocks)
        ops.gather_scatter_cl(rv, sphere, scale, bev_xy, scale, out=back, pts_out=point_rows, n_live=n_live)

    def _stem_sparse_cl(self, bev_cl, pcds_coord):
        plan = ops.stem_plan(pcds_coord, bev_cl.shape[1], bev_cl.shape[2])
        return ops.sparse_downsample(bev_cl, plan, self.stem_w, self.header_bev[0].bias, compact=False)

    def _encode_cl(self, point_feat, pcds_coord, pcds_sphere_coord, n_live=None):
        bs, t, cin, n, _ = point_feat.shape
        dev = point_feat.device
        bev_xy = pcds_coord[:, 0, :, :2, 0]
        sphere = pcds_sphere_coord[:, 0, :, :, 0]
        cpt = self.pp2[0].shape[0]
        hb, wb = self.bev_hw
        c_dec, c1 = self.conv_2[0].shape[0], self.res1_bev[-1].w2.shape[0]
        o1, o2 = cpt, cpt + c_dec
        fuse = torch.empty((bs, n, cpt + c_dec + c1), dtype=torch.float32, device=dev)
        c0 = self.header_bev[-1].w2.shape[0]
        x0cat = ops.empty_cl(bs, 2 * c0, hb // 2, wb // 2, dev)
        x1cat = ops.empty_cl(bs, 2 * c1, hb // 4, wb // 4, dev)
        hw0, hw1 = (32, 1024), (16, 512)
        rv0, rv1 = ops.empty_cl(bs, c0, hw0[0], hw0[1], dev), ops.empty_cl(bs, c1, hw1[0], hw1[1], dev)
        ops.zero_views_cl([rv0, x0cat[:, c0:], rv1, x1cat[:, c1:]])
        if self.sparse_stem and self.stem_w is not None:
            plan = ops.stem_plan(pcds_coord, hb, wb, row_floats=t * cpt)
            rows = ops.pointnet_scatter_rows(point_feat.float(), pcds_coord, self.pp1[0], self.pp1[1], self.pp2[0], self.pp2[1],
                                             plan, pts_out=fuse[:, :, :o1], n_live=n_live)
            x = ops.sparse_downsample(rows, plan, self.stem_w, self.header_bev[0].bias, compact=True)
            self._stage_cl(x, self.header_bev[1:], out=x0cat[:, :c0])
        else:
            bev_cl = torch.empty((bs, hb, wb, t * cpt), dtype=torch.float32, device=dev)
            ops.pointnet_scatter(point_feat.float(), pcds_coord, self.pp1[0], self.pp1[1], self.pp2[0], self.pp2[1], bev_cl,
                                 pts_out=fuse[:, :, :o1], zero_fill=True)
            self._stage_cl(bev_cl.permute(0, 3, 1, 2), self.header_bev, out=x0cat[:, :c0])
        self._cross_view_cl(x0cat, c0, bev_xy, sphere, self.header_rv, hw0, (0.5, 0.5), rv=rv0)
        self._stage_cl(x0cat, self.res1_bev, out=x1cat[:, :c1])
        self._cross_view_cl(x1cat, c1, bev_xy, sphere, self.res1_rv, hw1, (0.25, 0.25), point_rows=fuse[:, :, o2:], n_live=n_live,
                            rv=rv1)
        return {"x0cat": x0cat, "x1cat": x1cat, "fuse": fuse, "bev_xy": bev_xy, "o1": o1, "o2": o2}

    def _decode_cl(self, enc, x2, want_aux=True, n_live=None):
        x0cat, x1cat, fuse, bev_xy, o1, o2 = enc["x0cat"], enc["x1cat"], enc["fuse"], enc["bev_xy"], enc["o1"], enc["o2"]
        k = self.aux[2]
        if self.upconv:
            y = ops.upconv3x3(self._conv(x0cat, self.conv_1a, None, NONE), self.conv_1[1],
                              [(x1cat, self.conv_1z[0]), (x2, self.conv_1z[1])], LEAKY)
            size = tuple(x0cat.shape[2:])

            def head1x1(src, wb):
                bb, cc, hh, ww = src.shape
                rows = src.permute(0, 2, 3, 1).reshape(bb * hh * ww, cc)
                return torch.addmm(wb[1], rows, wb[0].reshape(wb[0].shape[0], -1).t()).view(bb, hh, ww, -1).permute(0, 3, 1, 2)

            aux = (None, None, None)
            if want_aux:
                aux = [head1x1(x0cat, self.aux_split[0])]
                for src, wb in ((x1cat, self.aux_split[1]), (x2, self.aux_split[2])):
                    aux.append(F.interpolate(head1x1(src, wb), size=size, mode="bilinear", align_corners=True))
        else:
            dec_in = ops.upsample_concat_cl([x0cat, x1cat, x2], tuple(x0cat.shape[2:]))
            y = self._conv(dec_in, self.conv_1[0], self.conv_1[1], LEAKY)
            aux = F.conv2d(dec_in, self.aux[0], self.aux[1]) if want_aux else (None, None, None)
        bev_feat = self._conv(y, self.conv_2[0], self.conv_2[1], LEAKY)
        if self._head_gathers(fuse, bev_feat, o1, o2):
            return self._point_heads(fuse, aux, k, x2, n_live, gather=(bev_feat, bev_xy, self.grid2point_scale))
        ops.gather_scatter_cl(bev_feat, bev_xy, self.grid2point_scale, pts_out=fuse[:, :, o1:o2], n_live=n_live)
        return self._point_heads(fuse, aux, k, x2, n_live)
```

streammos_amd/ops.py:

```python
import collections
import ctypes
import os

import numpy as np
import torch

from . import _lib, profiling
from .scratch import _NO_GUARD, _dev_index, _on, _raw_stream, _stream, shared
from .scratch import release as release_stream_workspaces

_DTYPE_CODE = {torch.float32: 0, torch.float16: 1, torch.float64: 2}


def env_on(text):
    text = (text or "").strip().lower()
    return None if text == "" else text not in ("0", "false", "off", "no")


class Switch:
    __slots__ = ("var", "default", "fallback", "explicit")

    def __init__(self, var, default, fallback=None):
        self.var, self.default, self.fallback, self.explicit = var, default, fallback, None

    def __call__(self):
        if self.explicit is not None:
            return self.explicit
        on = env_on(os.environ.get(self.var))
        if on is None:
            on = bool(self.fallback()) if self.fallback is not None else self.default
        return on

    def set(self, flag):
        prev, self.explicit = self.explicit, (None if flag is None else bool(flag))
        return prev


is_deterministic = Switch("SMOS_DETERMINISTIC", False, lambda: torch.are_deterministic_algorithms_enabled())
point_mlp_fused = Switch("SMOS_POINT_MLP", False)
point_head_fused = Switch("SMOS_POINT_HEAD_TRAIN", False)
conv1_fused = Switch("SMOS_CONV1_TRAIN", False)
bilinear_bwd_own = Switch("SMOS_BILINEAR_BWD", True)
set_deterministic, set_point_mlp_fused, set_point_head_fused = is_deterministic.set, point_mlp_fused.set, point_head_fused.set
cross_view_fused = Switch("SMOS_CROSS_VIEW_TRAIN", False)
set_conv1_fused, set_bilinear_bwd_own, set_cross_view_fused = conv1_fused.set, bilinear_bwd_own.set, cross_view_fused.set


def _require_cuda(name, *tensors):
    for t in tensors:
        if t is not None and not t.is_cuda:
            raise RuntimeError("%s: expected a tensor in GPU memory, got device=%s (no CPU path here)" % (name, t.device))


def _ptr(t):
    return None if t is None else t.data_ptr()


def _live_ptr(name, n_live):
    if n_live is None:
        return None
    if n_live.dtype != torch.int32 or n_live.numel() < 1:
        raise RuntimeError("%s: n_live must be a device int32 tensor" % name)
    return n_live.data_ptr()


def _dtype_code(name, t):
    code = _DTYPE_CODE.get(t.dtype)
    if code is None:
        raise RuntimeError("%s: unsupported dtype %s" % (name, t.dtype))
    return code


def voxel_maxpool_fwd(feat, ind, out, out_size, scale, voxel_max_idx=None):
    _require_cuda("voxel_maxpool_fwd", feat, ind, out, voxel_max_idx)
    if feat.dtype != ind.dtype or feat.dtype != out.dtype:
        raise RuntimeError("voxel_maxpool_fwd: feat/ind/out dtypes differ (%s, %s, %s)" % (feat.dtype, ind.dtype, out.dtype))
    if not ind.is_contiguous():
        raise RuntimeError("voxel_maxpool_fwd: pcds_ind must be contiguous")
    bs, c, n = feat.shape[0], feat.shape[1], feat.shape[2]
    d = ind.shape[2]
    if len(out_size) != d or len(scale) != d or ind.shape[0] != bs or ind.shape[1] != n:
        raise RuntimeError("voxel_maxpool_fwd: shape mismatch feat %s ind %s out_size %s" % (tuple(feat.shape), tuple(ind.shape), tuple(out_size)))
    if tuple(out.shape) != (bs, c) + tuple(int(s) for s in out_size):
        raise RuntimeError("voxel_maxpool_fwd: out has shape %s" % (tuple(out.shape),))
    if voxel_max_idx is not None and (voxel_max_idx.dtype != torch.int64 or not voxel_max_idx.is_contiguous()):
        raise RuntimeError("voxel_maxpool_fwd: voxel_max_idx must be contiguous int64")
    label = "voxel_maxpool_fwd[%dx%dx%d->%s]" % (bs, c, n, "x".join(str(int(s)) for s in out_size))
    flag = shared.get("maxpool_flag", (4,), torch.int32, feat.device, zero=True)
    with _on(feat.device), profiling.span(label):
        _lib.call("smos_voxel_maxpool_fwd", feat.data_ptr(), _lib.i64_array(feat.stride()[:3]), ind.data_ptr(), out.data_ptr(),
                  _lib.i64_array(out.stride()), _ptr(voxel_max_idx), bs, c, n, d, _lib.i64_array(out_size), _lib.f32_array(scale),
                  _dtype_code("voxel_maxpool_fwd", feat), flag.data_ptr(), _stream(feat))
    return out


def voxel_maxpool_bwd(feat, ind, out, grad_out, grad_feat, out_size, scale):
    _require_cuda("voxel_maxpool_bwd", feat, ind, out, grad_out, grad_feat)
    def _same_layout(a, b):
        return all(sa == sb for sa, sb, n in zip(a.stride(), b.stride(), a.shape) if n > 1)
    if not _same_layout(grad_out, out):
        grad_out = grad_out.contiguous()
        if not _same_layout(grad_out, out):
            raise RuntimeError("voxel_maxpool_bwd: grad_out layout must match out")
    if not _same_layout(grad_feat, feat):
        raise RuntimeError("voxel_maxpool_bwd: grad_feat layout must match feat")
    bs, c, n = feat.shape[0], feat.shape[1], feat.shape[2]
    with _on(feat.device):
        _lib.call("smos_voxel_maxpool_bwd", feat.data_ptr(), _lib.i64_array(feat.stride()[:3]), ind.data_ptr(), out.data_ptr(),
                  grad_out.data_ptr(), _lib.i64_array(out.stride()), grad_feat.data_ptr(), bs, c, n, ind.shape[2],
                  _lib.i64_array(out_size), _lib.f32_array(scale), _dtype_code("voxel_maxpool_bwd", feat), _stream(feat))
    return grad_feat


def segsum_chunk():
    return _lib.query("smos_segsum_chunk")


def _bilinear_gather_fwd(grid, coord, scale, out, point_major):
    if coord.dim() == 4:
        coord = coord[..., 0]
    if not coord.is_contiguous():
        coord = coord.contiguous()
    b, c, h, w = grid.shape
    n, k = coord.shape[1], coord.shape[2]
    if out is None:
        if point_major:
            out = torch.empty((b, n, c), dtype=torch.float32, device=grid.device).permute(0, 2, 1)
        else:
            out = torch.empty((b, c, n), dtype=torch.float32, device=grid.device)
    with _on(grid.device), profiling.span_f("bilinear_gather[%dx%dx%dx%d->%d]", (b, c, h, w, n)):
        _lib.call("smos_bilinear_gather_fwd", grid.data_ptr(), _lib.i64_array(grid.stride()), coord.data_ptr(), k, out.data_ptr(),
                  _lib.i64_array(out.stride()[:3]), b, c, h, w, n, _lib.f32_array(scale), _stream(grid))
    return out


def bilinear_gather_backward(grad_out, coord, scale, grid_shape, channels_last=True, deterministic=None):
    _require_cuda("bilinear_gather_backward", grad_out, coord)
    if grad_out.dtype != torch.float32 or coord.dtype != torch.float32:
        raise RuntimeError("bilinear_gather_backward: float32 only (got %s, %s)" % (grad_out.dtype, coord.dtype))
    if coord.dim() == 4:
        coord = coord[..., 0]
    if grad_out.dim() == 4:
        grad_out = grad_out[..., 0]
    if not coord.is_contiguous():
        coord = coord.contiguous()
    b, c, n = grad_out.shape
    h, w = int(grid_shape[-2]), int(grid_shape[-1])
    k = coord.shape[2]
    if coord.shape[0] != b or coord.shape[1] != n or (len(grid_shape) == 4 and (int(grid_shape[0]), int(grid_shape[1])) != (b, c)):
        raise RuntimeError("bilinear_gather_backward: shape mismatch grad_out %s coord %s grid %s"
                           % (tuple(grad_out.shape), tuple(coord.shape), tuple(grid_shape)))
    if channels_last:
        grad_grid = torch.empty((b, h, w, c), dtype=torch.float32, device=grad_out.device).permute(0, 3, 1, 2)
    else:
        grad_grid = torch.empty((b, c, h, w), dtype=torch.float32, device=grad_out.device)
    if is_deterministic() if deterministic is None else deterministic:
        need = _lib.query("smos_bilinear_gather_bwd_det_work_bytes", b, c, h, w, n)
        if need < 0:
            raise RuntimeError("bilinear_gather_backward: the deterministic form takes B * N < 2^29 points and B * H * W < 2^31 - 1 "
                               "pixels (got %d, %d)" % (b * n, b * h * w))
        with _on(grad_out.device), profiling.span_f("bilinear_gather_bwd_det[%dx%dx%dx%d<-%d]", (b, c, h, w, n)):
            work = torch.empty((need,), dtype=torch.uint8, device=grad_out.device)
            _lib.call("smos_bilinear_gather_bwd_det", grad_out.data_ptr(), _lib.i64_array(grad_out.stride()), coord.data_ptr(), k,
                      grad_grid.data_ptr(), _lib.i64_array(grad_grid.stride()), b, c, h, w, n, _lib.f32_array(scale),
                      work.data_ptr(), need, _stream(grad_out))
        return grad_grid
    with _on(grad_out.device), profiling.span_f("bilinear_gather_bwd[%dx%dx%dx%d<-%d]", (b, c, h, w, n)):
        _lib.call("smos_bilinear_gather_bwd", grad_out.data_ptr(), _lib.i64_array(grad_out.stride()), coord.data_ptr(), k,
                  grad_grid.data_ptr(), _lib.i64_array(grad_grid.stride()), b, c, h, w, n, _lib.f32_array(scale), _stream(grad_out))
    return grad_grid


class _BilinearGather(torch.autograd.Function):

    @staticmethod
    def forward(ctx, grid, coord, scale, out_box, point_major):
        ctx.save_for_backward(coord)
        ctx.scale, ctx.grid_shape = tuple(float(v) for v in scale), tuple(grid.shape)
        res = _bilinear_gather_fwd(grid, coord, scale, out_box[0], point_major)
        return res.detach() if out_box[0] is not None else res

    @staticmethod
    def backward(ctx, grad_out):
        coord, = ctx.saved_tensors
        return bilinear_gather_backward(grad_out, coord, ctx.scale, ctx.grid_shape, channels_last=True), None, None, None, None


def bilinear_gather(grid, coord, scale, out=None, point_major=False):
    grad_mode = torch.is_grad_enabled()
    if grad_mode and coord.requires_grad:
        raise RuntimeError("bilinear_gather: no gradient with respect to coord (the coordinates are data); detach it")
    _require_cuda("bilinear_gather", grid, coord, out)
    if grid.dtype != torch.float32 or coord.dtype != torch.float32:
        raise RuntimeError("bilinear_gather: float32 only (got %s, %s)" % (grid.dtype, coord.dtype))
    if grad_mode and grid.requires_grad:
        return _BilinearGather.apply(grid, coord, scale, (out,), point_major)
    return _bilinear_gather_fwd(grid, coord, scale, out, point_major)


def _gst_coord(t):
    if t.dim() == 4:
        t = t[..., 0]
    return t if t.is_contiguous() else t.contiguous()


def _gst_common(grid, gcoord, gscale, scoord, sscale, out):
    b, c, hg, wg = grid.shape
    head = (grid.data_ptr(), _lib.i64_array(grid.stride()), gcoord.data_ptr(), gcoord.shape[2], _lib.f32_array(gscale),
            scoord.data_ptr(), scoord.shape[2], _lib.f32_array(sscale), out.data_ptr(), _lib.i64_array(out.stride()))
    return head, (b, c, hg, wg, gcoord.shape[1], out.shape[2], out.shape[3])


def _gst_strides(t):
    return None if t is None else _lib.i64_array(t.stride())


def _gather_scatter_train_fwd(grid, gcoord, gscale, scoord, out_size, sscale, want_points):
    b, c = grid.shape[:2]
    n = gcoord.shape[1]
    out = torch.zeros((b, c) + out_size, dtype=torch.float32, device=grid.device)
    pts = torch.empty((b, c, n), dtype=torch.float32, device=grid.device) if want_points else None
    flag = shared.get("maxpool_flag", (4,), torch.int32, grid.device, zero=True)
    head, sizes = _gst_common(grid, gcoord, gscale, scoord, sscale, out)
    with _on(grid.device), profiling.span_f("gather_scatter_train_fwd[%dx%dx%dx%d->%d->%dx%d]", sizes):
        _lib.call("smos_gather_scatter_train_fwd", *head, _ptr(pts), _gst_strides(pts), *sizes, flag.data_ptr(), _stream(grid))
    return out, pts


def gather_scatter_train_point_grad(grid, gcoord, gscale, scoord, sscale, out, grad_out, grad_pts=None, x=None):
    _require_cuda("gather_scatter_train_point_grad", grid, gcoord, scoord, out, grad_out, grad_pts, x)
    gcoord, scoord = _gst_coord(gcoord), _gst_coord(scoord)
    head, sizes = _gst_common(grid, gcoord, gscale, scoord, sscale, out)
    if x is None:
        x = torch.empty((sizes[0], sizes[1], sizes[4]), dtype=torch.float32, device=grid.device)
    with _on(grid.device), profiling.span_f("gather_scatter_train_point_grad[%dx%dx%dx%d->%d->%dx%d]", sizes):
        _lib.call("smos_gather_scatter_train_point_grad", *head, grad_out.data_ptr(), _lib.i64_array(grad_out.stride()),
                  _ptr(grad_pts), _gst_strides(grad_pts), x.data_ptr(), _lib.i64_array(x.stride()), *sizes, _stream(grid))
    return x


def gather_scatter_train_backward(grid, gcoord, gscale, scoord, sscale, out, grad_out, grad_pts=None, channels_last=True,
                                  deterministic=None):
    _require_cuda("gather_scatter_train_backward", grid, gcoord, scoord, out, grad_out, grad_pts)
    gcoord, scoord = _gst_coord(gcoord), _gst_coord(scoord)
    head, sizes = _gst_common(grid, gcoord, gscale, scoord, sscale, out)
    b, c, hg, wg, n = sizes[:5]
    if is_deterministic() if deterministic is None else deterministic:
        x = shared.get("cross_view_point_grad", (b, c, n), torch.float32, grid.device)
        gather_scatter_train_point_grad(grid, gcoord, gscale, scoord, sscale, out, grad_out, grad_pts, x=x)
        return bilinear_gather_backward(x, gcoord, gscale, (b, c, hg, wg), channels_last=channels_last, deterministic=True)
    if channels_last:
        grad_grid = torch.empty((b, hg, wg, c), dtype=torch.float32, device=grid.device).permute(0, 3, 1, 2)
    else:
        grad_grid = torch.empty((b, c, hg, wg), dtype=torch.float32, device=grid.device)
    with _on(grid.device), profiling.span_f("gather_scatter_train_bwd[%dx%dx%dx%d<-%d<-%dx%d]", sizes):
        _lib.call("smos_gather_scatter_train_bwd", *head, grad_out.data_ptr(), _lib.i64_array(grad_out.stride()), _ptr(grad_pts),
                  _gst_strides(grad_pts), grad_grid.data_ptr(), _lib.i64_array(grad_grid.stride()), *sizes, _stream(grid))
    return grad_grid


class _GatherScatterTrain(torch.autograd.Function):

    @staticmethod
    def forward(ctx, grid, gcoord, scoord, gscale, out_size, sscale, want_points):
        out, pts = _gather_scatter_train_fwd(grid, gcoord, gscale, scoord, out_size, sscale, want_points)
        ctx.set_materialize_grads(False)
        if ctx.needs_input_grad[0]:
            ctx.save_for_backward(grid, gcoord, scoord, out)
            ctx.scales = (gscale, sscale)
        return (out, pts) if want_points else out

    @staticmethod
    @torch.autograd.function.once_differentiable
    def backward(ctx, grad_out, grad_pts=None):
        if grad_out is None and grad_pts is None:
            return (None,) * 7
        grid, gcoord, scoord, out = ctx.saved_tensors
        gscale, sscale = ctx.scales
        if grad_out is None:
            grad_out = torch.zeros_like(out)
        return (gather_scatter_train_backward(grid, gcoord, gscale, scoord, sscale, out, grad_out, grad_pts),
                None, None, None, None, None, None)


def gather_scatter_train(grid, gcoord, gscale, scoord, out_size, sscale, want_points=False):
    name = "gather_scatter_train"
    _require_cuda(name, grid, gcoord, scoord)
    if grid.dtype != torch.float32 or gcoord.dtype != torch.float32 or scoord.dtype != torch.float32:
        raise RuntimeError("%s: float32 only (got %s, %s, %s)" % (name, grid.dtype, gcoord.dtype, scoord.dtype))
    if gcoord.requires_grad or scoord.requires_grad:
        raise RuntimeError("%s: no gradient with respect to the coordinates (they are data); detach them" % name)
    gcoord, scoord = _gst_coord(gcoord), _gst_coord(scoord)
    out_size = tuple(int(v) for v in out_size)
    gscale, sscale = tuple(float(v) for v in gscale), tuple(float(v) for v in sscale)
    if (grid.dim() != 4 or gcoord.dim() != 3 or scoord.dim() != 3 or gcoord.shape[0] != grid.shape[0] or gcoord.shape[2] < 2
            or scoord.shape[2] < 2 or tuple(scoord.shape[:2]) != tuple(gcoord.shape[:2]) or len(out_size) != 2 or len(gscale) != 2
            or len(sscale) != 2 or min(out_size) < 1 or grid.shape[2] < 1 or grid.shape[3] < 1):
        raise RuntimeError("%s: shape mismatch grid %s gcoord %s scoord %s out_size %s"
                           % (name, tuple(grid.shape), tuple(gcoord.shape), tuple(scoord.shape), out_size))
    if gcoord.device != grid.device or scoord.device != grid.device:
        raise RuntimeError("%s: coordinates on %s / %s, grid on %s" % (name, gcoord.device, scoord.device, grid.device))
    if torch.is_grad_enabled() and grid.requires_grad:
        return _GatherScatterTrain.apply(grid, gcoord, scoord, gscale, out_size, sscale, bool(want_points))
    out, pts = _gather_scatter_train_fwd(grid, gcoord, gscale, scoord, out_size, sscale, bool(want_points))
    return (out, pts) if want_points else out


def seg_loss_tile():
    return _lib.query("smos_seg_loss_tile")


def _seg_loss_args(name, pred, target):
    _require_cuda(name, pred, target)
    if pred.dtype != torch.float32:
        raise RuntimeError("%s: float32 logits only (got %s)" % (name, pred.dtype))
    if target.dtype.is_floating_point or target.dtype.is_complex or target.dtype == torch.bool:
        raise RuntimeError("%s: integer labels only (got %s)" % (name, target.dtype))
    if pred.dim() == 4 and pred.shape[3] == 1:
        pred = pred[..., 0]
    if target.dim() == 3 and target.shape[2] == 1:
        target = target[..., 0]
    if pred.dim() != 3 or target.dim() != 2 or pred.shape[0] != target.shape[0] or pred.shape[2] != target.shape[1]:
        raise RuntimeError("%s: shape mismatch pred %s target %s (want [B,C,P(,1)] and [B,P(,1)])"
                           % (name, tuple(pred.shape), tuple(target.shape)))
    if pred.shape[1] not in (2, 3):
        raise RuntimeError("%s: %d classes; the kernels are built for C = 2 and C = 3" % (name, pred.shape[1]))
    if pred.shape[0] * pred.shape[2] == 0:
        raise RuntimeError("%s: no positions (pred %s)" % (name, tuple(pred.shape)))
    if target.device != pred.device:
        raise RuntimeError("%s: pred on %s, target on %s" % (name, pred.device, target.device))
    return pred, target.to(torch.int64).contiguous()


class _SegLoss(torch.autograd.Function):

    @staticmethod
    def forward(ctx, pred, target, k, top_weight, ignore_index, lovasz_weight):
        p3 = pred[..., 0] if pred.dim() == 4 else pred
        b, c, p = p3.shape
        n = b * p
        need = _lib.query("smos_seg_loss_work_bytes", n, c)
        if need <= 0:
            raise RuntimeError("seg_loss: %d positions x %d classes is more than the sort is set up for" % (n, c))
        dev = pred.device
        work = shared.get("seg_loss", (need,), torch.uint8, dev)
        coef = torch.empty((c + 1, n), dtype=torch.float32, device=dev)
        loss = torch.empty((), dtype=torch.float32, device=dev)
        stats = torch.empty(2, dtype=torch.float32, device=dev)
# ... 519 lines not shown
    if k.dtype != torch.int32 or k.numel() != 1 or k.device != labels.device:
        raise RuntimeError("instance_apply: k must be an int32 [1] tensor on the labels' device")
    with _on(labels.device):
        _lib.call("smos_instance_apply", names.data_ptr(), slot_of.data_ptr(), counts.data_ptr(), k.data_ptr(), counts.shape[0],
                  labels.data_ptr(), n, _stream(labels))
    return labels


def _label_args(name, words, gt, gt_map, counts, n, device):
    _require_cuda(name, words, gt, gt_map, counts)
    if words is not None and (words.dtype != torch.int32 or not words.is_contiguous() or words.numel() < n
                              or words.data_ptr() % 16 or words.device != device):
        raise RuntimeError("%s: words must be a contiguous, 16-byte aligned int32 tensor of >= n elements on the labels' device" % name)
    if gt is None:
        return _ptr(words), None, None, 0, None
    if gt_map is None or counts is None:
        raise RuntimeError("%s: counting needs gt_map and counts" % name)
    if gt.dtype not in (torch.int32, torch.uint32) or not gt.is_contiguous() or gt.numel() != n or gt.data_ptr() % 16:
        raise RuntimeError("%s: gt must be a contiguous, 16-byte aligned 32-bit tensor with one word per label" % name)
    if gt_map.dtype != torch.int32 or not gt_map.is_contiguous() or gt_map.dim() != 1:
        raise RuntimeError("%s: gt_map must be a contiguous int32 vector" % name)
    if counts.dtype not in (torch.int64, torch.uint64) or not counts.is_contiguous() or counts.numel() != 6:
        raise RuntimeError("%s: counts must be a contiguous 64-bit tensor of 6 counters" % name)
    if not (gt.device == gt_map.device == counts.device == device):
        raise RuntimeError("%s: every tensor must be on the labels' device" % name)
    return _ptr(words), gt.data_ptr(), gt_map.data_ptr(), gt_map.numel(), counts.data_ptr()


def label_words(labels, words=None, lut=True, gt=None, gt_map=None, counts=None):
    _require_cuda("label_words", labels)
    if labels.dtype != torch.uint8 or labels.dim() != 1 or not labels.is_contiguous() or labels.data_ptr() % 4:
        raise RuntimeError("label_words: labels must be a contiguous, 4-byte aligned uint8 vector")
    n = labels.shape[0]
    if words is None:
        words = torch.empty(n, dtype=torch.int32, device=labels.device)
    w, g, gm, mn, c = _label_args("label_words", words, gt, gt_map, counts, n, labels.device)
    with _on(labels.device):
        _lib.call("smos_label_words", labels.data_ptr(), n, 1 if lut else 0, w, g, gm, mn, c, _stream(labels))
    return words


def voted_label_counts(voted, gt, gt_map, counts, words=None):
    _require_cuda("voted_label_counts", voted)
    if voted.dtype != torch.int32 or voted.dim() != 1 or not voted.is_contiguous() or voted.data_ptr() % 16:
        raise RuntimeError("voted_label_counts: voted must be a contiguous, 16-byte aligned int32 vector")
    n = voted.shape[0]
    w, g, gm, mn, c = _label_args("voted_label_counts", words, gt, gt_map, counts, n, voted.device)
    with _on(voted.device):
        _lib.call("smos_label_count_voted", voted.data_ptr(), n, w, g, gm, mn, c, _stream(voted))
    return words


ACT_NONE, ACT_RELU, ACT_LEAKY = 0, 1, 2


def _rows(name, t, c):
    if t.dim() != 3 or t.shape[2] != c or t.stride(2) != 1:
        raise RuntimeError("%s: expected point rows [B, N, %d] with contiguous channels, got %s / %s" % (name, c, tuple(t.shape), t.stride()))
    return t.stride(0), t.stride(1)


def pointnet_scatter(xyzi, coord, w1, b1, w2, b2, bev, pts_out=None, zero_fill=False):
    _require_cuda("pointnet_scatter", xyzi, coord, w1, b1, w2, b2, bev, pts_out)
    b, t, cin, n = xyzi.shape[:4]
    k = coord.shape[3]
    if not (xyzi.is_contiguous() and coord.is_contiguous() and bev.is_contiguous()):
        raise RuntimeError("pointnet_scatter: xyzi, coord and bev must be contiguous")
    h, w = bev.shape[1], bev.shape[2]
    cout = w2.shape[0]
    if bev.shape[3] != t * cout:
        raise RuntimeError("pointnet_scatter: bev has %d channels, expected %d" % (bev.shape[3], t * cout))
    po_b = po_n = 0
    if pts_out is not None:
        po_b, po_n = _rows("pointnet_scatter", pts_out, cout)
    with _on(xyzi.device), profiling.span_f("pointnet_scatter[%dx%dx%d->%dx%d]", (b, t, n, h, w)):
        if zero_fill:
            bev.zero_()
        _lib.call("smos_pointnet_scatter", xyzi.data_ptr(), coord.data_ptr(), k, w1.data_ptr(), b1.data_ptr(), w2.data_ptr(),
                  b2.data_ptr(), bev.data_ptr(), _ptr(pts_out), po_b, po_n, b, t, n, h, w, cin, w1.shape[0], cout, _stream(xyzi))
    return bev


def point_head_k_order():
    s = torch.arange(96)[:, None]
    h = torch.arange(2)[None, :]
    return 64 * (s >> 5) + 32 * h + (s & 31)


def point_head_prepare(l1, l2, l3):
    w1, b1 = l1[0].reshape(l1[0].shape[0], -1).float(), l1[1].float()
    w2, b2 = l2[0].reshape(l2[0].shape[0], -1).float(), l2[1].float()
    w3, b3 = l3[0].reshape(l3[0].shape[0], -1).float(), l3[1].float()
    if tuple(w1.shape) != (96, 192) or tuple(w2.shape) != (64, 96) or w3.shape[1] != 64 or w3.shape[0] > 32:
        raise RuntimeError("point_head_prepare: expected 192 -> 96 -> 64 -> (<=32), got %s %s %s" % (tuple(w1.shape), tuple(w2.shape), tuple(w3.shape)))
    dev = w1.device
    lane = torch.arange(64, device=dev)
    m, h = lane & 31, lane >> 5
    a1 = w1.view(3, 32, 192)[:, :, point_head_k_order().to(dev)].permute(0, 2, 3, 1).reshape(3, 96, 64)

    def acc_order(n_steps):
        s = torch.arange(n_steps, device=dev)[:, None]
        return 32 * (s >> 4) + 8 * ((s & 15) >> 2) + 4 * h[None, :] + (s & 3)
    ch2 = acc_order(48)
    a2 = torch.stack([w2[mt * 32 + m[None, :].expand(48, 64), ch2] for mt in range(2)])
    w3p = torch.zeros((32, 64), device=dev)
    w3p[:w3.shape[0]] = w3
    a3 = w3p[m[None, :].expand(32, 64), acc_order(32)]
    b3p = torch.zeros(32, device=dev)
    b3p[:b3.shape[0]] = b3
    flat = torch.cat([a1.reshape(-1), a2.reshape(-1), a3.reshape(-1), b1, b2, b3p]).contiguous()
    if flat.numel() != _lib.query("smos_point_head_weight_floats"):
        raise RuntimeError("point_head_prepare: weight block has %d floats" % flat.numel())
    return flat, int(w3.shape[0])


def point_head(rows, wprep, m3, out=None, n_live=None, gather=None):
    _require_cuda("point_head", rows, wprep, out, n_live)
    if rows.dtype != torch.float32 or rows.dim() != 3 or rows.stride(2) != 1 or rows.stride(0) != rows.shape[1] * rows.stride(1):
        raise RuntimeError("point_head: rows must be a float32 [B, N, C] tensor with dense point rows")
    live = _live_ptr("point_head", n_live)
    b, n = rows.shape[0], rows.shape[1]
    if gather is not None:
        grid, gcoord, gscale = gather
        _require_cuda("point_head", grid, gcoord)
        if grid.dtype != torch.float32 or grid.shape[0] != b or grid.shape[1] != 64:
            raise RuntimeError("point_head: the gathered map must be a float32 channels-last [B, 64, Hg, Wg] view, got %s" % (tuple(grid.shape),))
        gp = _cl("point_head", grid)
        kg, gbs = _coord_view("point_head", gcoord, b, n)
    if out is None:
        out = torch.empty((b, m3, n), dtype=torch.float32, device=rows.device)
    head = (rows.data_ptr(), rows.stride(1), wprep.data_ptr(), out.data_ptr(), b, n, 192, 96, 64, m3, live)
    with _on(rows.device), profiling.span_f("point_head[%dx%d]", (b, n)):
        if gather is None:
            _lib.call("smos_point_head", *head, _stream(rows))
        else:
            _lib.call("smos_point_head_gather", *head, grid.data_ptr(), gp, grid.shape[2], grid.shape[3], gcoord.data_ptr(), kg, gbs,
                      _lib.f32_array(gscale), _stream(rows))
    return out


def conv_prepare(w, mt, order="taps"):
    cout, cin, kh, kw = w.shape
    if cin % 32 or cout % (32 * mt) or mt not in (1, 2, 4) or order not in ("taps", "rows") or (order == "rows" and mt > 2):
        raise RuntimeError("conv_prepare: Cin %% 32 == 0 and Cout %% (32 * mt) == 0 required (got %s, mt=%d, order=%s)" % (tuple(w.shape), mt, order))
    v = w.float().reshape(cout // (32 * mt), mt, 32, cin // 32, 4, 2, 4, kh, kw)
    if order == "rows":
        v = v.permute(0, 7, 3, 8, 4, 1, 5, 2, 6)
    else:
        v = v.permute(0, 7, 8, 3, 4, 1, 5, 2, 6)
    return v.reshape(-1).contiguous()


def conv_cl_supported(x, cout, kernel, stride=1, residual=None, out=None):
    kh, kw = kernel
    b, cin, h, w = x.shape
    if cin % 32 or cout % 32 or cout > 2048 or not (1 <= kh <= 7 and 1 <= kw <= 7) or stride not in (1, 2):
        return False
    ho, wo = (h + 2 * (kh // 2) - kh) // stride + 1, (w + 2 * (kw // 2) - kw) // stride + 1
    if ho <= 0 or wo <= 0:
        return False

    def pitch(t, c):
        return t.stride(3) if t is not None and t.dim() == 4 and t.stride(1) == 1 else c
    limit = 1 << 31
    if b * h * w * pitch(x, cin) * 4 >= limit or b * ho * wo * pitch(out, cout) * 4 >= limit:
        return False
    if residual is not None and b * ho * wo * pitch(residual, cout) * 4 >= limit:
        return False
    return True


def conv_rows_ok(kernel, stride, cin, cout):
    kh, kw = kernel
    return stride == 1 and kw in (3, 5, 7) and kh in (1, 3, 5, 7) and cin % 32 == 0 and cout % 32 == 0


def _conv_operands(name, x, wprep, bias, cout, ho, wo, residual=None, out=None, chan_sums=None, sum_chunks=None):
    _require_cuda(name, x, wprep, bias, residual, out, chan_sums)
    b = x.shape[0]
    if out is None:
        out = empty_cl(b, cout, ho, wo, x.device)
    elif tuple(out.shape) != (b, cout, ho, wo):
        raise RuntimeError("%s: out has shape %s, expected %s" % (name, tuple(out.shape), (b, cout, ho, wo)))
    if residual is not None and tuple(residual.shape) != (b, cout, ho, wo):
        raise RuntimeError("%s: residual has shape %s" % (name, tuple(residual.shape)))
    if chan_sums is not None and (residual is not None or not chan_sums.is_contiguous() or chan_sums.dtype != torch.float32 or
                                  tuple(chan_sums.shape) != (b, sum_chunks(ho, wo), cout)):
        raise RuntimeError("%s: chan_sums must be contiguous float32 [B, %s(Ho, Wo), Cout], without a residual"
                           % (name, sum_chunks.__name__))
    return out, (x.data_ptr(), _cl(name, x), wprep.data_ptr(), _ptr(bias), _ptr(residual),
                 _cl(name, residual) if residual is not None else 0,
                 out.data_ptr(), _cl(name, out))


def _conv_label(name, x, cout, ho, wo, kernel, residual=None):
    return "%s[%dx%dx%dx%d->%dx%dx%dk%dx%d%s]" % ((name,) + tuple(x.shape) + (cout, ho, wo) + tuple(kernel) +
                                                ("+res" if residual is not None else "",))


def _conv_launch(fn_name, family, args, keep, x, label_fn):
    dev = x.device
    if not profiling.enabled():
        fn = _lib.entry(fn_name)
        with _on(dev):
            rc = fn(*args, _raw_stream(_dev_index(dev)))
        if rc:
            _lib.check(rc, fn_name)
        return
    label = label_fn()
    with _on(dev), profiling.span(label, family):
        _lib.call(fn_name, *args, _stream(x))
    if profiling._replay_label == label:
        def again(keep=keep):
            with _on(keep[0].device), profiling.span(label, family):
                _lib.call(fn_name, *args, _stream(keep[0]))
        profiling.offer_replay(label, again)


def conv_rows_cl(x, wprep, bias, act, cout, kernel, mt=1, residual=None, out=None, chan_sums=None):
    b, cin, h, w = x.shape
    kh, kw = kernel
    if not conv_rows_ok(kernel, 1, cin, cout) or wprep.numel() != cout * cin * kh * kw or mt not in (1, 2) or cout % (32 * mt):
        raise RuntimeError("conv_rows_cl: unsupported shape %s k%dx%d -> %d" % (tuple(x.shape), kh, kw, cout))
    out, head = _conv_operands("conv_rows_cl", x, wprep, bias, cout, h, w, residual, out, chan_sums, conv_sum_chunks)
    args = head + (b, h, w, cin, cout, kh, kw, int(mt), int(act), _ptr(chan_sums))
    _conv_launch("smos_conv_rows_cl", "conv_rows", args, (x, wprep, bias, residual, out, chan_sums), x,
                 lambda: _conv_label("conv_cl", x, cout, h, w, kernel, residual))
    return out


_CONV_MIN_WAVE_TILES = int(os.environ.get("SMOS_CONV_MIN_WAVE_TILES", "2048"))


def conv_mt(cout, n_pixels, residual=False):
    tiles32 = (n_pixels + 31) // 32
    for mt in ((2, 1) if residual else (4, 2, 1)):
        if cout % (32 * mt) == 0 and tiles32 * (cout // (32 * mt)) >= _CONV_MIN_WAVE_TILES:
            return mt
    return 1


def conv_sum_chunks(ho, wo):
    return ((ho + 3) // 4) * ((wo + 31) // 32) * 4


def conv_cl(x, wprep, bias, act, cout, kernel, stride=1, padding=None, mt=1, residual=None, out=None, chan_sums=None):
    b, cin, h, w = x.shape
    kh, kw = kernel
    ph, pw = padding if padding is not None else (kh // 2, kw // 2)
    ho, wo = (h + 2 * ph - kh) // stride + 1, (w + 2 * pw - kw) // stride + 1
    if wprep.numel() != cout * cin * kh * kw:
        raise RuntimeError("conv_cl: weight block has %d floats, expected %d" % (wprep.numel(), cout * cin * kh * kw))
    out, head = _conv_operands("conv_cl", x, wprep, bias, cout, ho, wo, residual, out, chan_sums, conv_sum_chunks)
    args = head + (b, h, w, cin, cout, kh, kw, stride, ph, pw, mt, int(act), _ptr(chan_sums))
    _conv_launch("smos_conv_cl", "conv_igemm", args, (x, wprep, bias, residual, out, chan_sums), x,
                 lambda: _conv_label("conv_cl", x, cout, ho, wo, kernel, residual))
    return out


def conv_bf16_prepare(w):
    cout, cin, kh, kw = w.shape
    if cin % 32 or cout % 32:
        raise RuntimeError("conv_bf16_prepare: Cin %% 32 == 0 and Cout %% 32 == 0 required (got %s)" % (tuple(w.shape),))
    v = w.detach().float().reshape(cout // 32, 32, cin // 32, 2, 2, 8, kh, kw)
    v = v.permute(2, 6, 7, 0, 3, 4, 1, 5)
    return v.to(torch.bfloat16).reshape(-1).contiguous()


_bf16_shape_ok = {}


def conv_bf16_ok(x, cout, kernel, stride=1, residual=None, out=None, chan_sums=None):
    if chan_sums is not None and residual is not None:
        return False
    if not conv_cl_supported(x, cout, kernel, stride, residual, out):
        return False
    kh, kw = kernel
    key = (x.shape[1], cout, kh, kw, stride, residual is not None)
    ok = _bf16_shape_ok.get(key)
    if ok is None:
        ok = _bf16_shape_ok[key] = bool(_lib.query("smos_conv_bf16_cl_supported", *key[:5], int(key[5])))
    return ok


def conv_bf16_cl(x, wprep, bias, act, cout, kernel, stride=1, padding=None, residual=None, out=None, chan_sums=None):
    b, cin, h, w = x.shape
    kh, kw = kernel
    ph, pw = padding if padding is not None else (kh // 2, kw // 2)
    ho, wo = (h + 2 * ph - kh) // stride + 1, (w + 2 * pw - kw) // stride + 1
    if wprep.dtype != torch.bfloat16 or wprep.numel() != cout * cin * kh * kw:
        raise RuntimeError("conv_bf16_cl: weight block must hold %d bf16 (conv_bf16_prepare), got %d %s" %
                           (cout * cin * kh * kw, wprep.numel(), wprep.dtype))
    if x.dtype != torch.float32 or (bias is not None and (bias.dtype != torch.float32 or bias.numel() != cout)):
        raise RuntimeError("conv_bf16_cl: x and bias must be float32 (bias of Cout entries)")
    if (out is not None and out.dtype != torch.float32) or (residual is not None and residual.dtype != torch.float32):
        raise RuntimeError("conv_bf16_cl: out and residual must be float32")
    out, head = _conv_operands("conv_bf16_cl", x, wprep, bias, cout, ho, wo, residual, out, chan_sums, conv_sum_chunks)
    args = head + (b, h, w, cin, cout, kh, kw, stride, ph, pw, int(act), _ptr(chan_sums))
    _conv_launch("smos_conv_bf16_cl", "conv_bf16", args, (x, wprep, bias, residual, out, chan_sums), x,
                 lambda: _conv_label("conv_bf16", x, cout, ho, wo, kernel, residual))
    return out


_WINO_G = ((1.0, 0.0, 0.0), (0.5, 0.5, 0.5), (0.5, -0.5, 0.5), (0.0, 0.0, 1.0))


def conv_wino_prepare(w, mb):
    cout, cin, kh, kw = w.shape
    if (kh, kw) != (3, 3) or cin % 16 or mb not in (1, 2) or cout % (16 * mb):
        raise RuntimeError("conv_wino_prepare: 3x3 kernel, Cin %% 16 == 0 and Cout %% (16 * mb) == 0 required (got %s, mb=%d)"
                           % (tuple(w.shape), mb))
    g = torch.tensor(_WINO_G, dtype=torch.float64, device=w.device)
    u = (g @ w.double() @ g.t()).float()
    v = u.reshape(cout // (16 * mb), mb, 16, cin // 16, 4, 4, 4, 4)
    v = v.permute(0, 3, 5, 1, 6, 4, 2, 7)
    return v.reshape(-1).contiguous()


def conv_wino_ok(kernel, stride, cin, cout):
    return tuple(kernel) == (3, 3) and stride == 1 and cin % 16 == 0 and cout % 16 == 0


def conv_wino_mb(cout, n_items16=None):
    return 2 if cout % 32 == 0 else 1


def conv_wino_sum_chunks(h, w):
    return ((h + 7) // 8) * ((w + 31) // 32) * 4


def conv_wino_cl(x, wprep, bias, act, cout, mb=2, residual=None, out=None, chan_sums=None):
    b, cin, h, w = x.shape
    if not conv_wino_ok((3, 3), 1, cin, cout) or mb not in (1, 2) or cout % (16 * mb) or wprep.numel() != 16 * cout * cin:
        raise RuntimeError("conv_wino_cl: unsupported shape %s -> %d (mb=%d)" % (tuple(x.shape), cout, mb))
    out, head = _conv_operands("conv_wino_cl", x, wprep, bias, cout, h, w, residual, out, chan_sums, conv_wino_sum_chunks)
    args = head + (b, h, w, cin, cout, int(mb), int(act), _ptr(chan_sums))
    _conv_launch("smos_conv_wino_cl", "conv_wino", args, (x, wprep, bias, residual, out, chan_sums), x,
                 lambda: _conv_label("conv_cl", x, cout, h, w, (3, 3), residual))
    return out


class BasicBlockPlan:
    __slots__ = ("c", "mb", "gated", "cr", "ptrs", "_keep")

    def __init__(self, w1, b1, w2, b2, gate=None):
        c = w1.shape[0]
        if tuple(w1.shape) != (c, c, 3, 3) or tuple(w2.shape) != (c, c, 3, 3) or c % 16:
            raise RuntimeError("BasicBlockPlan: two [C, C, 3, 3] weights with C %% 16 == 0 expected, got %s / %s"
                               % (tuple(w1.shape), tuple(w2.shape)))
        _require_cuda("BasicBlockPlan", w1, b1, w2, b2, *(gate or ()))
        self.c, self.mb = c, conv_wino_mb(c)
        u1, u2 = conv_wino_prepare(w1, self.mb), conv_wino_prepare(w2, self.mb)
        b1, b2 = b1.float().contiguous(), b2.float().contiguous()
        self.gated = gate is not None
        g = [t.float().contiguous() for t in gate] if self.gated else []
        if self.gated and (tuple(g[0].shape) != (g[0].shape[0], c) or tuple(g[2].shape) != (c, g[0].shape[0])):
            raise RuntimeError("BasicBlockPlan: gate MLP must be [Cr, C], [Cr], [C, Cr], [C]")
        self.cr = g[0].shape[0] if self.gated else 0
        self._keep = (u1, b1, u2, b2, g)
        self.ptrs = (u1.data_ptr(), b1.data_ptr(), u2.data_ptr(), b2.data_ptr()) + \
            (tuple(t.data_ptr() for t in g) if self.gated else (None, None, None, None)) + (self.cr,)


class UnbalanceBlockPlan:
    __slots__ = ("c", "mb", "ptrs_a", "ptrs_b", "ptrs_c", "_keep")

    def __init__(self, wa, ba, wb, bb, wc, bc):
        c = wa.shape[0]
        ka, kb = tuple(wa.shape[2:]), tuple(wb.shape[2:])
        if (tuple(wa.shape[:2]) != (c, c) or tuple(wb.shape[:2]) != (c, c) or tuple(wc.shape) != (c, 2 * c, 3, 3) or
                not conv_wino1d_ok(ka, 1, c, c) or not conv_wino1d_ok(kb, 1, c, c)):
            raise RuntimeError("UnbalanceBlockPlan: unexpected weights %s %s %s" % (tuple(wa.shape), tuple(wb.shape), tuple(wc.shape)))
        _require_cuda("UnbalanceBlockPlan", wa, ba, wb, bb, wc, bc)
        self.c, self.mb = c, conv_wino_mb(c)
        ua, ub = conv_wino1d_prepare(wa, self.mb), conv_wino1d_prepare(wb, self.mb)
        uc = conv_wino_prepare(wc, self.mb)
        ba, bb, bc = (t.float().contiguous() for t in (ba, bb, bc))
        self._keep = (ua, ub, uc, ba, bb, bc)
        self.ptrs_a = (ua.data_ptr(), ba.data_ptr(), ka[0], ka[1])
        self.ptrs_b = (ub.data_ptr(), bb.data_ptr(), kb[0], kb[1])
        self.ptrs_c = (uc.data_ptr(), bc.data_ptr())


def unbalance_block_cl(x, plan, both=None, out=None):
    _require_cuda("unbalance_block_cl", x, both, out)
    b, c, h, w = x.shape
    if c != plan.c:
        raise RuntimeError("unbalance_block_cl: %d channels, the block has %d" % (c, plan.c))
    dev = x.device
    if both is None:
        both = empty_cl(b, 2 * c, h, w, dev)
    if out is None:
        out = empty_cl(b, c, h, w, dev)
    if both.shape != (b, 2 * c, h, w) or out.shape != x.shape:
        raise RuntimeError("unbalance_block_cl: both must be [B,2C,H,W] and out have x's shape %s" % (tuple(x.shape),))
    with _on(dev):
        _lib.call("smos_unbalance_block_cl", x.data_ptr(), _cl("unbalance_block_cl", x), *plan.ptrs_a, *plan.ptrs_b, *plan.ptrs_c,
                  both.data_ptr(), _cl("unbalance_block_cl", both), out.data_ptr(), _cl("unbalance_block_cl", out), b, h, w, c,
                  plan.mb, _raw_stream(_dev_index(dev)))
    return out


def gate_channels_ok(c):
    return c % 32 == 0 and c <= 256 and 1024 % c == 0


def basic_block_ok(c, gated):
    return c % 16 == 0 and (not gated or gate_channels_ok(c))


def basic_block_cl(x, plan, y=None, out=None, ws=None):
    _require_cuda("basic_block_cl", x, y, out, ws)
    b, c, h, w = x.shape
    if c != plan.c:
        raise RuntimeError("basic_block_cl: %d channels, the block has %d" % (c, plan.c))
    dev = x.device
    if y is None:
        y = empty_cl(b, c, h, w, dev)
    if out is None:
        out = empty_cl(b, c, h, w, dev)
    if y.shape != x.shape or out.shape != x.shape:
        raise RuntimeError("basic_block_cl: y / out must have x's shape %s" % (tuple(x.shape),))
    wsp = None
    if plan.gated:
        if (ws is None or ws.dtype != torch.float32 or not ws.is_contiguous() or
                ws.numel() < _lib.query("smos_basic_block_ws_floats", b, h, w, c)):
            raise RuntimeError("basic_block_cl: a gated block needs smos_basic_block_ws_floats floats of contiguous scratch")
        wsp = ws.data_ptr()
    with _on(dev):
        _lib.call("smos_basic_block_cl", x.data_ptr(), _cl("basic_block_cl", x), *plan.ptrs, y.data_ptr(), _cl("basic_block_cl", y),
                  out.data_ptr(), _cl("basic_block_cl", out), wsp, b, h, w, c, plan.mb, _raw_stream(_dev_index(dev)))
    return out


def msda_fwd_qp(value, qp, h, w, points):
    _require_cuda("msda_fwd_qp", value, qp)
    n, s, m, d = value.shape
    if not (value.is_contiguous() and qp.is_contiguous()) or s != h * w or qp.shape[-1] != m * points * 3 or value.dtype != torch.float32:
        raise RuntimeError("msda_fwd_qp: expected contiguous float32 value [N,H*W,M,D] and qp [N,H*W,M*P*3]")
    out = torch.empty((n, s, m * d), dtype=torch.float32, device=value.device)
    with _on(value.device), profiling.span_f("msda_fwd[%dx%dx%dx%d]", (n, s, m, d)):
        _lib.call("smos_msda_fwd_qp", value.data_ptr(), qp.data_ptr(), out.data_ptr(), n, h, w, m, d, points, _stream(value))
    return out


def add_layer_norm(x, res, gamma, beta, eps=1e-5):
    _require_cuda("add_layer_norm", x, res, gamma, beta)
    if not x.is_contiguous() or (res is not None and (not res.is_contiguous() or res.shape != x.shape)):
        raise RuntimeError("add_layer_norm: x and res must be contiguous and of equal shape")
    c = x.shape[-1]
    out = torch.empty_like(x)
    with _on(x.device):
        _lib.call("smos_add_layer_norm", x.data_ptr(), _ptr(res), gamma.data_ptr(), beta.data_ptr(), out.data_ptr(), x.numel() // c,
                  c, float(eps), _stream(x))
    return out


def _tf_pairs(w):
    o, k = w.shape
    v = w.float().reshape(o // 16, 16, k // 16, 4, 4)
    return v.permute(0, 2, 3, 1, 4).reshape(o // 16, k // 16, 64, 4)


def tfusion_pack_linear(w):
    cout, k = w.shape
    if k != 128 or cout > 2048:
        raise RuntimeError("tfusion_pack_linear: expected [<=2048, 128], got %s" % (tuple(w.shape),))
    pad = (cout + 63) // 64 * 64
    wp = torch.zeros((pad, k), dtype=torch.float32, device=w.device)
    wp[:cout] = w
    return _tf_pairs(wp).reshape(-1).contiguous()


class TfusionLayer:

    def __init__(self, out, norm1, lin1, lin2, norm2, next_qproj=None):
        wo, bo = out
        w1, b1 = lin1
        w2, b2 = lin2
        ffn = w1.shape[0]
        if tuple(wo.shape) != (128, 128) or w1.shape[1] != 128 or tuple(w2.shape) != (128, ffn) or ffn % 32:
            raise RuntimeError("TfusionLayer: built for d_model 128 and an FFN width that is a multiple of 32")
        dev = wo.device
        po, p1, p2 = _tf_pairs(wo), _tf_pairs(w1), _tf_pairs(w2)
        slots = [po.reshape(8, 8, 64, 4)]
        l2 = p2.permute(1, 0, 2, 3)
        n_t = ffn // 16
        slots.append(p1[0:1])
        if n_t > 1:
            slots.append(torch.stack((p1[1:], l2[:-1]), 1).reshape(-1, 8, 64, 4))
        slots.append(l2[-1:])
        self.nq = 0
        bq = torch.zeros(64, dtype=torch.float32, device=dev)
        if next_qproj is not None:
            wq, bqv = next_qproj
            self.nq = int(wq.shape[0])
            if self.nq > 64 or self.nq % 4 or wq.shape[1] != 128:
                raise RuntimeError("TfusionLayer: the next projection must have 4..64 output channels (multiple of 4)")
            wqp = torch.zeros((64, 128), dtype=torch.float32, device=dev)
            wqp[:self.nq] = wq
            bq[:self.nq] = bqv
            slots.append(_tf_pairs(wqp).reshape(4, 8, 64, 4))
        self.stream = torch.cat(slots).reshape(-1).contiguous()
        self.params = torch.cat([bo.float(), norm1[0].float(), norm1[1].float(), b1.float(), b2.float(), norm2[0].float(),
                                 norm2[1].float(), bq]).contiguous()
        self.ffn = int(ffn)
        self.eps1 = float(norm1[2]) if len(norm1) > 2 else 1e-5
        self.eps2 = float(norm2[2]) if len(norm2) > 2 else 1e-5
        if (self.stream.numel() != _lib.query("smos_tfusion_layer_stream_floats", self.ffn, 1 if self.nq else 0) or
                self.params.numel() != _lib.query("smos_tfusion_layer_param_floats", self.ffn)):
            raise RuntimeError("TfusionLayer: packed sizes disagree with the kernel's")


def _token_rows(name, t):
    c = t.shape[-1]
    if t.dtype != torch.float32 or t.stride(-1) != 1:
        raise RuntimeError("%s: float32 rows with contiguous channels expected" % name)
    rows = t.reshape(-1, c) if t.is_contiguous() else t
    if rows.dim() != 2:
        raise RuntimeError("%s: a dense [..., C] tensor or a pitched [tokens, C] view expected, got %s / %s" % (name, tuple(t.shape), t.stride()))
    return rows.shape[0], rows.stride(0)


def tfusion_project(jobs):
    n = len(jobs)
    if not 1 <= n <= 8:
        raise RuntimeError("tfusion_project: 1..8 jobs")
    xs, pit, ws, bs, outs, ops_, couts, toks = ((ctypes.c_void_p * n)(), (ctypes.c_int64 * n)(), (ctypes.c_void_p * n)(), (ctypes.c_void_p * n)(),
                                                (ctypes.c_void_p * n)(), (ctypes.c_int64 * n)(), (ctypes.c_int64 * n)(), (ctypes.c_int64 * n)())
    res = []
    for j, job in enumerate(jobs):
        x, w, b = job[0], job[1], job[2]
        bias = None if isinstance(b, int) else b
        _require_cuda("tfusion_project", x, w, bias)
        tk, pitch = _token_rows("tfusion_project", x)
        if x.shape[-1] != 128:
            raise RuntimeError("tfusion_project: 128-channel token rows expected")
        cout = int(b) if bias is None else int(bias.shape[0])
        if w.numel() != (cout + 63) // 64 * 64 * 128:
            raise RuntimeError("tfusion_project: weight stream of %d floats for %d outputs" % (w.numel(), cout))
        if len(job) > 3 and job[3] is not None:
            out = job[3]
            _require_cuda("tfusion_project", out)
            if out.dim() != 2 or tuple(out.shape) != (tk, cout) or out.stride(1) != 1 or out.dtype != torch.float32:
                raise RuntimeError("tfusion_project: out must be a float32 [tokens, cout] view with contiguous channels")
        else:
            out = torch.empty((tk, cout), dtype=torch.float32, device=x.device)
        res.append(out)
        xs[j], pit[j], ws[j], outs[j], ops_[j], couts[j], toks[j] = x.data_ptr(), pitch, w.data_ptr(), out.data_ptr(), out.stride(0), cout, tk
        bs[j] = _ptr(bias)
    x0 = jobs[0][0]
    label = ("tfusion_project[%s]" % ",".join("%dx128->%d" % (int(toks[j]), int(couts[j])) for j in range(n))
             if profiling.enabled() else None)
    with _on(x0.device), profiling.span(label):
        _lib.call("smos_tfusion_project", n, xs, pit, ws, bs, outs, ops_, couts, toks, _stream(x0))
    return res


def tfusion_layer(sampled, query, prep, out=None):
    _require_cuda("tfusion_layer", sampled, query, out)
    tokens, sp = _token_rows("tfusion_layer", sampled)
    tq, qp = _token_rows("tfusion_layer", query)
    if sp != 128 or tq != tokens or sampled.shape[-1] != 128 or query.shape[-1] != 128:
        raise RuntimeError("tfusion_layer: sampled must be dense [tokens, 128] and query hold as many 128-channel rows")
    if out is None:
        out = torch.empty((tokens, 128), dtype=torch.float32, device=sampled.device)
    to, op = _token_rows("tfusion_layer", out)
    if to != tokens or out.shape[-1] != 128:
        raise RuntimeError("tfusion_layer: out must hold [tokens, 128]")
    nxt = torch.empty((tokens, prep.nq), dtype=torch.float32, device=sampled.device) if prep.nq else None
    with _on(sampled.device), profiling.span_f("tfusion_layer[%dx128x%d%s]", (tokens, prep.ffn, "+q%d" % prep.nq if prep.nq else "")):
        _lib.call("smos_tfusion_layer", sampled.data_ptr(), query.data_ptr(), qp, prep.stream.data_ptr(), prep.params.data_ptr(),
                  out.data_ptr(), op, _ptr(nxt), prep.nq, tokens, prep.ffn, prep.eps1, prep.eps2, _stream(sampled))
    return out, nxt


def tap_limbs_split(w):
    w = w.float()
    hi = w.to(torch.bfloat16)
    r = w - hi.float()
    mid = r.to(torch.bfloat16)
    lo = (r - mid.float()).to(torch.bfloat16)
    return lo, mid, hi


def tap_limbs_pack(w):
    cout, k = w.shape
    if k != 128 or cout > 2048:
        raise RuntimeError("tap_limbs_pack: expected [<=2048, 128], got %s" % (tuple(w.shape),))
    pad = (cout + 31) // 32 * 32
    wp = torch.zeros((pad, k), dtype=torch.float32, device=w.device)
    wp[:cout] = w
    v = torch.stack(tap_limbs_split(wp)).reshape(3, pad // 32, 32, 8, 2, 8)
    return v.permute(1, 3, 0, 4, 2, 5).reshape(-1).contiguous()


def tap_limbs_unpack(stream, cout):
    pad = (cout + 31) // 32 * 32
    v = stream.reshape(pad // 32, 8, 3, 2, 32, 8).permute(2, 0, 4, 1, 3, 5)
    return tuple(v.reshape(3, pad, 128)[:, :cout].float())


def tap_products_bf16x3(jobs):
    n = len(jobs)
    if not 1 <= n <= 8:
        raise RuntimeError("tap_products_bf16x3: 1..8 jobs")
    xs, pit, ws, outs, ops_, couts, toks = ((ctypes.c_void_p * n)(), (ctypes.c_int64 * n)(), (ctypes.c_void_p * n)(), (ctypes.c_void_p * n)(),
                                            (ctypes.c_int64 * n)(), (ctypes.c_int64 * n)(), (ctypes.c_int64 * n)())
    res = []
    for j, job in enumerate(jobs):
        x, w, cout = job[0], job[1], int(job[2])
        _require_cuda("tap_products_bf16x3", x, w)
        tk, pitch = _token_rows("tap_products_bf16x3", x)
        if x.shape[-1] != 128:
            raise RuntimeError("tap_products_bf16x3: 128-channel token rows expected")
        if w.dtype != torch.bfloat16 or w.numel() != (cout + 31) // 32 * 32 * 128 * 3 or not w.is_contiguous():
            raise RuntimeError("tap_products_bf16x3: limb stream of %d %s elements for %d outputs" % (w.numel(), w.dtype, cout))
        if len(job) > 3 and job[3] is not None:
            out = job[3]
            _require_cuda("tap_products_bf16x3", out)
            if out.dim() != 2 or tuple(out.shape) != (tk, cout) or out.stride(1) != 1 or out.dtype != torch.float32:
                raise RuntimeError("tap_products_bf16x3: out must be a float32 [tokens, cout] view with contiguous channels")
        else:
            out = torch.empty((tk, cout), dtype=torch.float32, device=x.device)
        res.append(out)
        xs[j], pit[j], ws[j], outs[j], ops_[j], couts[j], toks[j] = x.data_ptr(), pitch, w.data_ptr(), out.data_ptr(), out.stride(0), cout, tk
    x0 = jobs[0][0]
    label = ("tfusion_project[%s]" % ",".join("%dx128->%d" % (int(toks[j]), int(couts[j])) for j in range(n))
             if profiling.enabled() else None)
    with _on(x0.device), profiling.span(label):
        _lib.call("smos_tap_products_bf16x3", n, xs, pit, ws, outs, ops_, couts, toks, _stream(x0))
    return res


class TapWeights:

    def __init__(self, w, c0, c1):
        cout = w.shape[0]
        self.cout, self.cin = cout, c1 - c0
        self.nk = w[:, c0:c1].permute(2, 3, 0, 1).reshape(9 * cout, c1 - c0).float().contiguous()
        self.kn = self.nk.t().contiguous()
        self.zero = torch.zeros(9 * cout, dtype=torch.float32, device=w.device)
        self._conv = None
        self._stream = None
        self._limbs = None

    def stream(self, parts=1):
        if self._stream is None:
            self._stream = {}
        if parts not in self._stream:
            n = self.nk.shape[0] // parts
            self._stream[parts] = [tfusion_pack_linear(self.nk[i * n:(i + 1) * n]) for i in range(parts)]
        return self._stream[parts]

    def limb_stream(self, parts=1):
        if self._limbs is None:
            self._limbs = {}
        if parts not in self._limbs:
            n = self.nk.shape[0] // parts
            self._limbs[parts] = [tap_limbs_pack(self.nk[i * n:(i + 1) * n]) for i in range(parts)]
        return self._limbs[parts]

    def conv_operand(self):
        if self._conv is None:
            self._conv = conv_prepare(self.nk.view(9 * self.cout, self.cin, 1, 1), 4)
        return self._conv


def upconv_tap_weights(w, c0, c1):
    return TapWeights(w, c0, c1)


_TAP_GEMM = os.environ.get("SMOS_TAP_GEMM", "x3")
_TAP_GEMM_OWN = _TAP_GEMM == "conv"
_TAP_PARTS = int(os.environ.get("SMOS_TAP_PARTS", "3"))
_UPCONV_XY = os.environ.get("SMOS_UPCONV_XY", "1") != "0"
_TAP_JOB_BYTES = (1 << 31) - 4096
_TAP_JOB_ROWS = (1 << 22) - 64


def upconv_tap_products(x, wt):
    b, cin, hs, ws = x.shape
    if _TAP_GEMM_OWN and cin % 32 == 0 and (9 * wt.cout) % 128 == 0:
        return conv_cl(x, wt.conv_operand(), None, 0, 9 * wt.cout, (1, 1), mt=4).permute(0, 2, 3, 1).reshape(b * hs * ws, 9 * wt.cout)
    rows = x.permute(0, 2, 3, 1).reshape(b * hs * ws, cin)
    return torch.addmm(wt.zero, rows, wt.kn)


def upconv3x3(conv_a, bias, sources, act, out=None):
    _require_cuda("upconv3x3", conv_a, bias, out)
    b, c, ho, wo = conv_a.shape
    if out is None:
        out = conv_a
    st = _stream(conv_a)
    if not 1 <= len(sources) <= 2:
        raise RuntimeError("upconv3x3: one or two upsampled sources, got %d" % len(sources))
    fused = _UPCONV_XY and all(_lib.query("smos_upconv_xy_ok", src[0].shape[2], ho) for src in sources)
    zs, ts = [], []
    pre = {}
    if _TAP_GEMM in ("tf", "x3"):
# ... 36 lines not shown
            z2, h2, w2 = zs[1] if len(zs) > 1 else (None, 0, 0)
            with profiling.span("upconv_xy[%dx%dx%dx%d<-%s]" % (b, ho, wo, c, "+".join("%dx%d" % (h, w) for _, h, w in zs))
                                if profiling.enabled() else None):
                _lib.call("smos_upconv_xy", conv_a.data_ptr(), _cl("upconv3x3", conv_a), bias.data_ptr(), z1.data_ptr(), h1, w1,
                          _ptr(z2), h2, w2, out.data_ptr(), _cl("upconv3x3", out), b, ho, wo, c, int(act), st)
            return out
        t1, h1 = ts[0]
        t2, h2 = ts[1] if len(ts) > 1 else (None, 0)
        with profiling.span_f("upconv_ypass[%dx%dx%dx%d]", (b, ho, wo, c)):
            _lib.call("smos_upconv_ypass", conv_a.data_ptr(), _cl("upconv3x3", conv_a), bias.data_ptr(), t1.data_ptr(), h1,
                      _ptr(t2), h2, out.data_ptr(), _cl("upconv3x3", out), b, ho, wo, c, int(act), st)
    return out


def upconv_xy_units(conv_a, bias, z1, z2, act, strip, max_blocks=0, out=None):
    _require_cuda("upconv_xy_units", conv_a, bias, out, z1 and z1[0], z2 and z2[0])
    b, c, ho, wo = conv_a.shape
    if out is None:
        out = conv_a
    for z in (z1, z2):
        if z is not None and (tuple(z[0].shape) != (b * z[1] * z[2], 9 * c) or not z[0].is_contiguous()):
            raise RuntimeError("upconv_xy_units: tap products must be a contiguous [B*Hs*Ws, 9*C] matrix, got %s" % (tuple(z[0].shape),))
    (p1, h1, w1), (p2, h2, w2) = ((z[0].data_ptr(), z[1], z[2]) if z is not None else (None, 0, 0) for z in (z1, z2))
    with _on(conv_a.device):
        _lib.call("smos_upconv_xy_units", conv_a.data_ptr(), _cl("upconv_xy_units", conv_a), bias.data_ptr(), p1, h1, w1, p2, h2,
                  w2, out.data_ptr(), _cl("upconv_xy_units", out), b, ho, wo, c, int(act), int(strip), int(max_blocks),
                  _stream(conv_a))
    return out


_CONV1_OUT = os.environ.get("SMOS_CONV1_OUT", "cl")


def _as_cl(t, dense=False):
    b, c, h, w = t.shape
    s0, s1, s2, pitch = t.stride()
    if s1 == 1 and s2 == w * pitch and (b == 1 or s0 == h * w * pitch) and (pitch == c if dense else pitch >= c) and pitch % 4 == 0 \
            and t.data_ptr() % 16 == 0:
        return t
    out = empty_cl(b, c, h, w, t.device)
    out.copy_(t)
    return out


def upconv_adjoint(g, hs, ws, max_blocks=0, out=None, scratch=None):
    _require_cuda("upconv_adjoint", g, out, scratch)
    if g.dim() != 4 or g.dtype != torch.float32:
        raise RuntimeError("upconv_adjoint: g must be a float32 [B,C,Ho,Wo] map, got %s %s" % (tuple(g.shape), g.dtype))
    b, c, ho, wo = g.shape
    hs, ws = int(hs), int(ws)
    gp = _cl("upconv_adjoint", g)
    if scratch is None:
        scratch = torch.empty((b, 3, hs, wo, c), dtype=torch.float32, device=g.device)
    elif scratch.dtype != torch.float32 or scratch.numel() != b * 3 * hs * wo * c or not scratch.is_contiguous():
        raise RuntimeError("upconv_adjoint: scratch must be a contiguous float32 [B,3,Hs,Wo,C] tensor")
    if out is None:
        out = torch.empty((b * hs * ws, 9 * c), dtype=torch.float32, device=g.device)
    elif out.dim() != 2 or tuple(out.shape) != (b * hs * ws, 9 * c) or out.stride(1) != 1 or out.dtype != torch.float32:
        raise RuntimeError("upconv_adjoint: out must be a float32 [B*Hs*Ws, 9*C] view with contiguous channels")
    zp = out.stride(0) if out.shape[0] > 1 else max(out.stride(0), 9 * c)
    with _on(g.device):
        st = _stream(g)
        with profiling.span_f("upconv_bwd_ypass[%dx%dx%dx%d->%d]", (b, ho, wo, c, hs)):
            _lib.call("smos_upconv_bwd_ypass", g.data_ptr(), gp, scratch.data_ptr(), b, ho, wo, c, hs, int(max_blocks), st)
        with profiling.span_f("upconv_bwd_xpass[%dx%dx%dx%d<-%d]", (b, hs, ws, c, wo)):
            _lib.call("smos_upconv_bwd_xpass", scratch.data_ptr(), out.data_ptr(), zp, b, hs, ws, c, wo, int(max_blocks), st)
    return out


def _upconv_dx(gz, w, shape):
    b, cin, hs, ws = shape
    nk = w.permute(2, 3, 0, 1).reshape(-1, cin).float()
    return torch.mm(gz, nk).view(b, hs, ws, cin).permute(0, 3, 1, 2)


def _upconv_dw(gz, x):
    cin = x.shape[1]
    rows = _as_cl(x, dense=True).permute(0, 2, 3, 1).reshape(-1, cin)
    return torch.mm(gz.t(), rows).view(3, 3, -1, cin).permute(2, 3, 0, 1)


class _Upconv3x3Train(torch.autograd.Function):

    @staticmethod
    def forward(ctx, conv_a, *xw):
        b, c, ho, wo = conv_a.shape
        a = _as_cl(conv_a)
        out = a if a is not conv_a else empty_cl(b, c, ho, wo, conv_a.device)
        srcs = [(_as_cl(xw[i], dense=True), TapWeights(xw[i + 1], 0, xw[i + 1].shape[1])) for i in range(0, len(xw), 2)]
        upconv3x3(a, torch.zeros(c, dtype=torch.float32, device=conv_a.device), srcs, 0, out=out)
        ctx.save_for_backward(*xw)
        return out.contiguous() if _CONV1_OUT == "nchw" else out

    @staticmethod
    @torch.autograd.function.once_differentiable
    def backward(ctx, g):
        xw = ctx.saved_tensors
        need = ctx.needs_input_grad
        grads = [g if need[0] else None]
        gcl = None
        for i in range(0, len(xw), 2):
            x, w = xw[i], xw[i + 1]
            dx = dw = None
            if need[1 + i] or need[2 + i]:
                if gcl is None:
                    gcl = _as_cl(g.float())
                gz = upconv_adjoint(gcl, x.shape[2], x.shape[3])
                if need[1 + i]:
                    dx = _upconv_dx(gz, w, x.shape)
                if need[2 + i]:
                    dw = _upconv_dw(gz, x)
            grads += [dx, dw]
        return tuple(grads)


def upconv3x3_train(conv_a, sources):
    _require_cuda("upconv3x3_train", conv_a)
    if conv_a.dim() != 4 or conv_a.dtype != torch.float32 or conv_a.numel() == 0:
        raise RuntimeError("upconv3x3_train: conv_a must be a non-empty float32 [B,C,Ho,Wo] map, got %s %s" % (tuple(conv_a.shape), conv_a.dtype))
    b, c = conv_a.shape[:2]
    if c % 4 or 9 * c > 2048:
        raise RuntimeError("upconv3x3_train: %d output channels; the tap-product kernels take multiples of 4 up to 224" % c)
    sources = list(sources)
    if not 1 <= len(sources) <= 2:
        raise RuntimeError("upconv3x3_train: one or two upsampled sources, got %d" % len(sources))
    flat = []
    for i, src in enumerate(sources):
        if len(src) != 2:
            raise RuntimeError("upconv3x3_train: source %d must be (x_src, w_src)" % i)
        x, w = src
        _require_cuda("upconv3x3_train", x, w)
        if x.dim() != 4 or x.dtype != torch.float32 or x.shape[0] != b or x.shape[1] != 128 or x.numel() == 0:
            raise RuntimeError("upconv3x3_train: source %d is %s %s, want float32 [%d,128,Hs,Ws]" % (i, tuple(x.shape), x.dtype, b))
        if tuple(w.shape) != (c, 128, 3, 3) or w.dtype != torch.float32:
            raise RuntimeError("upconv3x3_train: weights of source %d are %s %s, want float32 [%d,128,3,3]" % (i, tuple(w.shape), w.dtype, c))
        if x.device != conv_a.device or w.device != conv_a.device:
            raise RuntimeError("upconv3x3_train: source %d on %s / %s, conv_a on %s" % (i, x.device, w.device, conv_a.device))
        flat += [x, w]
    return _Upconv3x3Train.apply(conv_a, *flat)


STEM_TAPS = (1, 2, 2, 4)
_STEM_Y = ("stem_y0", "stem_y1", "stem_y2", "stem_y3")


def stem_prepare_weights(wa, wp):
    cout, cin = wa.shape[0], wa.shape[1]
    out = []
    for cls in range(4):
        ey, ex = cls >> 1, cls & 1
        kys, kxs = ((0, 2) if ey else (1,)), ((0, 2) if ex else (1,))
        w = torch.cat([wa[:, :, ky, kx] for ky in kys for kx in kxs] + [wp[:, :, 0, 0]], 0).float()
        km = w.shape[0] // 32
        out.append(w.view(km, 32, 2, cin // 2).permute(0, 3, 2, 1).reshape(km, cin // 2, 64).contiguous())
    return out


class StemPlan:

    def __init__(self, b, h, w, row_cell, row_of, meta, rows):
        self.b, self.h, self.w = b, h, w
        self.row_cell, self.row_of, self.meta, self.rows = row_cell, row_of, meta, rows

    def class_rows(self):
        return self.meta[8:12] - self.meta[4:8]


def stem_plan(coord, h, w, row_floats=0):
    _require_cuda("stem_plan", coord)
    if coord.dtype != torch.float32 or not coord.is_contiguous():
        raise RuntimeError("stem_plan: coord must be contiguous float32")
    b, t, n, k = coord.shape[:4]
    dev = coord.device
    cells = b * h * w
    words = _lib.query("smos_stem_scan_state_words", cells)
    if words < 0:
        raise RuntimeError("stem_plan: grid too large for the scan")
    flags = shared.get("stem_flags", (cells,), torch.int32, dev, zero=True)
    state = shared.get("stem_scan_state", (words,), torch.int64, dev)
    row_cell = shared.get("stem_row_cell", (cells,), torch.int32, dev)
    row_of = shared.get("stem_row_of", (cells,), torch.int32, dev)
    meta = shared.get("stem_meta", (12,), torch.int32, dev, zero=True)
    rows = None
    if row_floats:
        rows = shared.get("stem_rows", (min(cells, b * t * n), row_floats), torch.float32, dev)
    st = _stream(coord)
    with _on(dev), profiling.span_f("stem_mark+scan[%dx%dx%d]", (b, h, w)):
        _lib.call("smos_stem_mark", coord.data_ptr(), k, b, t, n, h, w, flags.data_ptr(), state.data_ptr(), st)
        _lib.call("smos_stem_scan", flags.data_ptr(), b, h, w, state.data_ptr(), row_cell.data_ptr(), row_of.data_ptr(),
                  meta.data_ptr(), _ptr(rows), row_floats, st)
    return StemPlan(b, h, w, row_cell, row_of, meta, rows)


def pointnet_scatter_rows(xyzi, coord, w1, b1, w2, b2, plan, pts_out=None, n_live=None):
    _require_cuda("pointnet_scatter_rows", xyzi, coord, w1, b1, w2, b2, pts_out, n_live)
    live = _live_ptr("pointnet_scatter_rows", n_live)
    b, t, cin, n = xyzi.shape[:4]
    k = coord.shape[3]
    if not (xyzi.is_contiguous() and coord.is_contiguous()):
        raise RuntimeError("pointnet_scatter_rows: xyzi and coord must be contiguous")
    cout = w2.shape[0]
    rows = plan.rows
    if rows is None or rows.shape[1] != t * cout:
        raise RuntimeError("pointnet_scatter_rows: the plan carries no row table of %d floats per row" % (t * cout))
    po_b = po_n = 0
    if pts_out is not None:
        po_b, po_n = _rows("pointnet_scatter_rows", pts_out, cout)
    st = _stream(xyzi)
    with _on(xyzi.device), profiling.span_f("pointnet_scatter[%dx%dx%d->%dx%d]", (b, t, n, plan.h, plan.w)):
        _lib.call("smos_pointnet_scatter_rows", xyzi.data_ptr(), coord.data_ptr(), k, w1.data_ptr(), b1.data_ptr(), w2.data_ptr(),
                  b2.data_ptr(), rows.data_ptr(), plan.row_of.data_ptr(), _ptr(pts_out), po_b, po_n, b, t, n, plan.h, plan.w, cin,
                  w1.shape[0], cout, live, st)
    return rows


def sparse_downsample(src, plan, wprep, bias, compact, out=None):
    _require_cuda("sparse_downsample", src, bias, out, *wprep)
    b, h, w = plan.b, plan.h, plan.w
    cin = src.shape[-1]
    dev = src.device
    if src.dtype != torch.float32 or not src.is_contiguous() or (not compact and src.numel() != b * h * w * cin):
        raise RuntimeError("sparse_downsample: src must be contiguous float32 with B*H*W rows of Cin")
    if compact and src.dim() != 2:
        raise RuntimeError("sparse_downsample: the compact row table is [rows, Cin]")
    cout = bias.shape[0]
    per = b * (h // 2) * (w // 2)
    ys = [shared.get(tag, (per, (taps + 1) * cout), torch.float32, dev)
          for tag, taps in zip(_STEM_Y, STEM_TAPS)]
    if out is None:
        out = empty_cl(b, cout, (h + 2 - 3) // 2 + 1, (w + 2 - 3) // 2 + 1, dev)
    y_ptrs = (ctypes.c_void_p * 4)(*[y.data_ptr() for y in ys])
    w_ptrs = (ctypes.c_void_p * 4)(*[wt.data_ptr() for wt in wprep])
    st = _stream(src)
    tag = "[%dx%dx%dx%d]" % (b, h, w, cin) if profiling.enabled() else ""
    with _on(dev):
        with profiling.span("stem_gemm" + tag):
            _lib.call("smos_stem_gemm", src.data_ptr(), None if compact else plan.row_cell.data_ptr(), plan.meta.data_ptr(), w_ptrs,
                      y_ptrs, cin, cout, st)
        with profiling.span("stem_epilogue" + tag):
            _lib.call("smos_stem_epilogue", y_ptrs, plan.meta.data_ptr(), plan.row_of.data_ptr(), bias.data_ptr(), out.data_ptr(),
                      _cl("sparse_downsample", out), b, h, w, cout, st)
    return out


_WINO1D_KERNELS = ((5, 3), (7, 3), (3, 5), (3, 7))


def conv_wino1d_ok(kernel, stride, cin, cout, residual=None, chan_sums=None):
    return (tuple(kernel) in _WINO1D_KERNELS and stride == 1 and cin % 16 == 0 and cout % 16 == 0 and residual is None and
            chan_sums is None)


def conv_wino1d_prepare(w, mb):
    cout, cin, kh, kw = w.shape
    if (kh, kw) not in _WINO1D_KERNELS or cin % 16 or mb not in (1, 2) or cout % (16 * mb):
        raise RuntimeError("conv_wino1d_prepare: 5x3 / 7x3 / 3x5 / 3x7 kernel, Cin %% 16 == 0 and Cout %% (16 * mb) == 0 required "
                           "(got %s, mb=%d)" % (tuple(w.shape), mb))
    g = torch.tensor(_WINO_G, dtype=torch.float64, device=w.device)
    wl = w.double() if kw == 3 else w.double().transpose(2, 3)
    kl = wl.shape[2]
    u = (wl @ g.t()).float()
    v = u.reshape(cout // (16 * mb), mb, 16, cin // 16, 4, 4, kl, 4)
    v = v.permute(0, 3, 5, 6, 1, 4, 2, 7)
    return v.reshape(-1).contiguous()


def conv_wino1d_cl(x, wprep, bias, act, cout, kernel, mb=2, out=None):
    b, cin, h, w = x.shape
    kh, kw = kernel
    if not conv_wino1d_ok(kernel, 1, cin, cout) or mb not in (1, 2) or cout % (16 * mb) or wprep.numel() != 4 * max(kh, kw) * cout * cin:
        raise RuntimeError("conv_wino1d_cl: unsupported shape %s -> %d k%dx%d (mb=%d)" % (tuple(x.shape), cout, kh, kw, mb))
    out, head = _conv_operands("conv_wino1d_cl", x, wprep, bias, cout, h, w, out=out)
    args = head[:4] + head[6:] + (b, h, w, cin, cout, kh, kw, int(mb), int(act))
    _conv_launch("smos_conv_wino1d_cl", "conv_wino1d", args, (x, wprep, bias, out), x,
                 lambda: _conv_label("conv_cl", x, cout, h, w, kernel))
    return out


ConvSwitches = collections.namedtuple("ConvSwitches", "wino wino1d conv_rows conv_rows_mt", defaults=(True, True, 3, 1))


def conv_route(cin, cout, kernel, stride, n_out_pixels, has_residual, has_sums, switches):
    if switches.wino and conv_wino_ok(kernel, stride, cin, cout):
        return "wino", conv_wino_mb(cout)
    if switches.wino1d and not has_residual and not has_sums and conv_wino1d_ok(kernel, stride, cin, cout):
        return "wino1d", conv_wino_mb(cout)
    mt = conv_mt(cout, n_out_pixels, has_residual)
    if switches.conv_rows and mt <= switches.conv_rows_mt and conv_rows_ok(kernel, stride, cin, cout) and kernel[1] >= switches.conv_rows:
        return "rows", mt
    return "igemm", mt


class ConvLayer:
    __slots__ = ("w", "packed", "ran_bf16")
    _PREPARE = {"wino": conv_wino_prepare, "wino1d": conv_wino1d_prepare, "igemm": conv_prepare,
                "rows": lambda w, mt: conv_prepare(w, mt, order="rows")}

    def __init__(self, w):
        self.w, self.packed, self.ran_bf16 = w, {}, None

    def operand(self, key):
        wp = self.packed.get(key)
        if wp is None:
            wp = self.packed[key] = conv_bf16_prepare(self.w) if key == "bf16" else self._PREPARE[key[0]](self.w, key[1])
        return wp


def empty_cl(b, c, h, w, device, zero=False):
    if zero:
        return torch.zeros((b, h, w, c), dtype=torch.float32, device=device).permute(0, 3, 1, 2)
    return torch.empty_strided((b, c, h, w), (h * w * c, 1, w * c, c), dtype=torch.float32, device=device)


def _cl(name, t):
    b, c, h, w = t.shape
    s0, s1, s2, pitch = t.stride()
    if s1 != 1 or s2 != w * pitch or (b > 1 and s0 != h * w * pitch) or pitch < c:
        raise RuntimeError("%s: expected a channels-last [B,C,H,W] view, got shape %s strides %s" % (name, tuple(t.shape), t.stride()))
    return pitch


def bias_act_cl(x, bias, act, out=None, residual=None):
    _require_cuda("bias_act_cl", x, bias, out, residual)
    b, c, h, w = x.shape
    if out is None:
        out = empty_cl(b, c, h, w, x.device)
    with _on(x.device):
        _lib.call("smos_bias_act_cl", x.data_ptr(), _cl("bias_act_cl", x), _ptr(bias), _ptr(residual),
                  _cl("bias_act_cl", residual) if residual is not None else 0, out.data_ptr(), _cl("bias_act_cl", out), b * h * w,
                  c, act, _stream(x))
    return out


def downsample_epilogue_cl(a, p, bias, stride, out=None):
    _require_cuda("downsample_epilogue_cl", a, p, bias, out)
    b, c, h, w = p.shape
    if out is None:
        out = empty_cl(b, c, a.shape[2], a.shape[3], a.device)
    with _on(a.device):
        _lib.call("smos_downsample_epilogue_cl", a.data_ptr(), _cl("downsample_epilogue_cl", a), p.data_ptr(),
                  _cl("downsample_epilogue_cl", p), bias.data_ptr(), out.data_ptr(), _cl("downsample_epilogue_cl", out), b, c, h, w,
                  stride, _stream(a))
    return out


def pool_branch_prepare(w):
    w2 = w.reshape(w.shape[0], -1)
    if w2.shape[0] != w2.shape[1] or w2.shape[0] not in (32, 64, 128):
        raise RuntimeError("pool_branch_prepare: Cin == Cout in {32, 64, 128} expected, got %s" % (tuple(w.shape),))
    return _tf_pairs(w2).reshape(-1).contiguous()


def pool_branch_ok(cin, cout, stride):
    return cin == cout and cin in (32, 64, 128) and stride in (1, 2) and not (cin == 128 and stride == 1)


def downsample_pool_branch(x, wpairs, a, bias, stride, out=None):
    _require_cuda("downsample_pool_branch", x, wpairs, a, bias, out)
    b, c, h, w = x.shape
    ho, wo = (h + 2 - 3) // stride + 1, (w + 2 - 3) // stride + 1
    if tuple(a.shape) != (b, c, ho, wo) or wpairs.numel() != c * c or not pool_branch_ok(c, c, stride):
        raise RuntimeError("downsample_pool_branch: unsupported shapes x %s a %s stride %d" % (tuple(x.shape), tuple(a.shape), stride))
    if out is None:
        out = empty_cl(b, c, ho, wo, x.device)
    elif tuple(out.shape) != (b, c, ho, wo):
        raise RuntimeError("downsample_pool_branch: out has shape %s" % (tuple(out.shape),))
    with _on(x.device), profiling.span_f("downsample_pool_branch[%dx%dx%dx%d/s%d]", (b, c, h, w, stride)):
        _lib.call("smos_downsample_pool_branch", x.data_ptr(), _cl("downsample_pool_branch", x), wpairs.data_ptr(), a.data_ptr(),
                  _cl("downsample_pool_branch", a), bias.data_ptr(), out.data_ptr(), _cl("downsample_pool_branch", out), b, h, w, c,
                  c, int(stride), _stream(x))
    return out


def channel_gate_residual_cl(y, bias, w1, b1, w2, b2, xres, ws, out=None):
    _require_cuda("channel_gate_residual_cl", y, bias, w1, b1, w2, b2, xres, ws, out)
    b, c, h, w = y.shape
    if out is None:
        out = empty_cl(b, c, h, w, y.device)
    with _on(y.device):
        _lib.call("smos_channel_gate_residual_cl", y.data_ptr(), _cl("channel_gate_residual_cl", y), bias.data_ptr(), w1.data_ptr(),
                  b1.data_ptr(), w2.data_ptr(), b2.data_ptr(), xres.data_ptr(), _cl("channel_gate_residual_cl", xres),
                  out.data_ptr(), _cl("channel_gate_residual_cl", out), ws.data_ptr(), ws.numel(), b, c, w1.shape[0], h * w,
                  _stream(y))
    return out


def channel_gate_apply_cl(y, bias, w1, b1, w2, b2, xres, chan_sums, gate_ws, out=None):
    _require_cuda("channel_gate_apply_cl", y, bias, w1, b1, w2, b2, xres, chan_sums, gate_ws, out)
    b, c, h, w = y.shape
    if chan_sums.dim() != 3 or chan_sums.shape[0] != b or chan_sums.shape[2] != c or not chan_sums.is_contiguous() or gate_ws.numel() < b * c:
        raise RuntimeError("channel_gate_apply_cl: chan_sums must be contiguous [B, chunks, C] and gate_ws hold B*C floats")
    if out is None:
        out = empty_cl(b, c, h, w, y.device)
    with _on(y.device):
        _lib.call("smos_channel_gate_apply_cl", y.data_ptr(), _cl("channel_gate_apply_cl", y), bias.data_ptr(), w1.data_ptr(),
                  b1.data_ptr(), w2.data_ptr(), b2.data_ptr(), xres.data_ptr(), _cl("channel_gate_apply_cl", xres), out.data_ptr(),
                  _cl("channel_gate_apply_cl", out), chan_sums.data_ptr(), chan_sums.shape[1], gate_ws.data_ptr(), b, c,
                  w1.shape[0], h * w, _stream(y))
    return out


def upsample_concat_cl(sources, size):
    import ctypes
    _require_cuda("upsample_concat_cl", *sources)
    b = sources[0].shape[0]
    ctot = sum(s.shape[1] for s in sources)
    out = empty_cl(b, ctot, size[0], size[1], sources[0].device)
    ptrs = (ctypes.c_void_p * len(sources))(*[s.data_ptr() for s in sources])
    with _on(out.device):
        _lib.call("smos_upsample_concat_cl", ptrs, _lib.i64_array([s.shape[1] for s in sources]),
                  _lib.i64_array([s.shape[2] for s in sources]), _lib.i64_array([s.shape[3] for s in sources]),
                  _lib.i64_array([_cl("upsample_concat_cl", s) for s in sources]), len(sources), out.data_ptr(), b, size[0],
                  size[1], _stream(out))
    return out


def zero_views_cl(views):
    if not 1 <= len(views) <= 4:
        raise RuntimeError("zero_views_cl: 1 .. 4 views")
    _require_cuda("zero_views_cl", *views)
    k = len(views)
    ptrs, rows, rf, pit = (ctypes.c_void_p * k)(), (ctypes.c_int64 * k)(), (ctypes.c_int64 * k)(), (ctypes.c_int64 * k)()
    for i, v in enumerate(views):
        b, c, h, w = v.shape
        if v.dtype != torch.float32 or v.device != views[0].device:
            raise RuntimeError("zero_views_cl: float32 views on one device")
        ptrs[i], rows[i], rf[i], pit[i] = v.data_ptr(), b * h * w, c, _cl("zero_views_cl", v)
    with _on(views[0].device):
        _lib.call("smos_zero_views_cl", k, ptrs, rows, rf, pit, _stream(views[0]))


def _coord_view(name, t, b, n):
    if t.dtype != torch.float32 or t.dim() != 3 or t.shape[0] != b or (n is not None and t.shape[1] != n) or t.shape[2] < 2:
        raise RuntimeError("%s: coordinates must be float32 [B, N, K >= 2], got %s %s" % (name, tuple(t.shape), t.dtype))
    s0, s1, s2 = t.stride()
    if s2 != 1 or s1 < 2 or s0 < 0:
        raise RuntimeError("%s: coordinate view with strides %s (the last dimension must be dense)" % (name, t.stride()))
    return s1, s0


def gather_scatter_cl(grid, gcoord, gscale, scoord=None, sscale=None, out=None, pts_out=None, n_live=None):
    _require_cuda("gather_scatter_cl", grid, gcoord, scoord, out, pts_out, n_live)
    live = _live_ptr("gather_scatter_cl", n_live)
    b, c, hg, wg = grid.shape
    n = gcoord.shape[1]
    kg, gbs = _coord_view("gather_scatter_cl", gcoord, b, None)
    ho = wo = ks = op = sbs = 0
    sc = ss = None
    if out is not None:
        ho, wo, op = out.shape[2], out.shape[3], _cl("gather_scatter_cl", out)
        ks, sbs = _coord_view("gather_scatter_cl", scoord, b, n)
        sc, ss = scoord.data_ptr(), _lib.f32_array(sscale)
    po_b = po_n = 0
    if pts_out is not None:
        po_b, po_n = _rows("gather_scatter_cl", pts_out, c)
    label = ("gather_scatter_cl[%dx%dx%dx%d->%d->%dx%d%s]" % (b, c, hg, wg, n, ho, wo,
                                                           "+pts" if pts_out is not None and out is not None else "")
             if profiling.enabled() else None)
    with _on(grid.device), profiling.span(label):
        _lib.call("smos_gather_scatter_cl", grid.data_ptr(), _cl("gather_scatter_cl", grid), gcoord.data_ptr(), kg, gbs,
                  _lib.f32_array(gscale), sc, ks, sbs, ss, _ptr(out), op, _ptr(pts_out), po_b, po_n, b, c, hg, wg, n, ho, wo, live,
                  _stream(grid))
```

Baseline: 343.9 scans/s.

## Add bf16x3 split-precision MFMA convolution for selected f32 layers

```diff
diff --git a/include/smos.h b/include/smos.h
--- a/include/smos.h
+++ b/include/smos.h
@@ -165,6 +165,10 @@
                       int64_t res_pitch, float* out, int64_t out_pitch, int64_t B, int64_t H, int64_t W, int64_t Cin,
                       int64_t Cout, int32_t KH, int32_t KW, int32_t stride, int32_t pad_h, int32_t pad_w, int32_t act,
                       float* chan_sums, smos_stream_t stream);
+int smos_conv_bf16x3_cl_supported(int64_t Cin, int64_t Cout, int32_t KH, int32_t KW, int32_t stride);
+int smos_conv_bf16x3_cl(const float* x, int64_t x_pitch, const uint16_t* wlimbs, const float* bias, float* out,
+                        int64_t out_pitch, int64_t B, int64_t H, int64_t W, int64_t Cin, int64_t Cout, int32_t KH, int32_t KW,
+                        int32_t stride, int32_t pad_h, int32_t pad_w, int32_t act, smos_stream_t stream);
 int64_t smos_conv_wino_sum_chunks(int64_t H, int64_t W);
 int smos_conv_wino_cl(const float* x, int64_t x_pitch, const float* wprep, const float* bias, const float* res, int64_t res_pitch,
                       float* out, int64_t out_pitch, int64_t B, int64_t H, int64_t W, int64_t Cin, int64_t Cout, int32_t mb,
@@ -269,6 +273,10 @@
                             const float* ub, const float* bb, int64_t khb, int64_t kwb, const float* uc, const float* bc,
                             float* both, int64_t both_pitch, float* out, int64_t out_pitch, int64_t B, int64_t H, int64_t W,
                             int64_t C, int32_t mb, smos_stream_t stream);
+int smos_unbalance_block_x3_cl(const float* x, int64_t x_pitch, const void* wa, const float* ba, int64_t kha, int64_t kwa,
+                               int32_t x3a, const void* wb, const float* bb, int64_t khb, int64_t kwb, int32_t x3b, const float* uc,
+                               const float* bc, float* both, int64_t both_pitch, float* out, int64_t out_pitch, int64_t B, int64_t H,
+                               int64_t W, int64_t C, int32_t mb, smos_stream_t stream);
 int smos_zero_views_cl(int32_t n, float* const* ptrs, const int64_t* rows, const int64_t* row_floats, const int64_t* pitches,
                        smos_stream_t stream);
 int smos_upsample_concat_cl(const float* const* src, const int64_t* src_c, const int64_t* src_h, const int64_t* src_w,
diff --git a/profiles/kinds.py b/profiles/kinds.py
--- a/profiles/kinds.py
+++ b/profiles/kinds.py
@@ -1,6 +1,6 @@
 KIND = (
-    (("conv_igemm", "conv_rows", "conv_wino"), "conv_cl[", 1),
-    (("conv_bf16",), "conv_bf16[", 1),
+    (("conv_igemm", "conv_rows", "conv_wino", "conv_bf16x3<"), "conv_cl[", 1),
+    (("conv_bf16<",), "conv_bf16[", 1),
     (("gather_scatter_cl",), "gather_scatter_cl[", 1),
     (("pointnet_scatter",), "pointnet_scatter[", 1),
     (("point_head",), "point_head[", 1),
diff --git a/profiles/label_durations.py b/profiles/label_durations.py
--- a/profiles/label_durations.py
+++ b/profiles/label_durations.py
@@ -29,7 +29,7 @@
 for p in problems:
     sys.stderr.write("label_durations: %s -- left unlabelled\n" % p)
 def family_of(label, kernel_name):
-    for frag in ("conv_wino1d", "conv_wino", "conv_igemm", "conv_rows"):
+    for frag in ("conv_bf16x3", "conv_wino1d", "conv_wino", "conv_igemm", "conv_rows"):
         if frag in kernel_name:
             return frag
     return label.split("[", 1)[0] if label else kernel_name.split("(")[0].split("<")[0][:60]
diff --git a/streammos_amd/_lib.py b/streammos_amd/_lib.py
--- a/streammos_amd/_lib.py
+++ b/streammos_amd/_lib.py
@@ -61,11 +61,15 @@
     "smos_conv_rows_cl": [vp, i64, vp, vp, vp, i64, vp, i64, i64, i64, i64, i64, i64, i32, i32, i32, i32, vp, vp],
     "smos_conv_bf16_cl_supported": [i64, i64, i32, i32, i32, i32],
     "smos_conv_bf16_cl": [vp, i64, vp, vp, vp, i64, vp, i64, i64, i64, i64, i64, i64, i32, i32, i32, i32, i32, i32, vp, vp],
+    "smos_conv_bf16x3_cl_supported": [i64, i64, i32, i32, i32],
+    "smos_conv_bf16x3_cl": [vp, i64, vp, vp, vp, i64, i64, i64, i64, i64, i64, i32, i32, i32, i32, i32, i32, vp],
     "smos_conv_wino_sum_chunks": [i64, i64],
     "smos_conv_wino_cl": [vp, i64, vp, vp, vp, i64, vp, i64, i64, i64, i64, i64, i64, i32, i32, vp, vp],
     "smos_basic_block_ws_floats": [i64, i64, i64, i64],
     "smos_basic_block_cl": [vp, i64, vp, vp, vp, vp, vp, vp, vp, vp, i64, vp, i64, vp, i64, vp, i64, i64, i64, i64, i32, vp],
     "smos_unbalance_block_cl": [vp, i64, vp, vp, i64, i64, vp, vp, i64, i64, vp, vp, vp, i64, vp, i64, i64, i64, i64, i64, i32, vp],
+    "smos_unbalance_block_x3_cl": [vp, i64, vp, vp, i64, i64, i32, vp, vp, i64, i64, i32, vp, vp, vp, i64, vp, i64, i64, i64, i64, i64, i32,
+                                   vp],
     "smos_zero_views_cl": [i32, ctypes.POINTER(vp), c_i64p, c_i64p, c_i64p, vp],
     "smos_msda_fwd_qp": [vp, vp, vp, i64, i64, i64, i64, i64, i64, vp],
     "smos_add_layer_norm": [vp, vp, vp, vp, vp, i64, i64, ctypes.c_float, vp],
diff --git a/streammos_amd/csrc/blocks.hip b/streammos_amd/csrc/blocks.hip
--- a/streammos_amd/csrc/blocks.hip
+++ b/streammos_amd/csrc/blocks.hip
@@ -33,3 +33,21 @@
   if (rc) return rc;
   return smos_conv_wino_cl(both, both_pitch, uc, bc, x, x_pitch, out, out_pitch, B, H, W, 2 * C, C, mb, 1, nullptr, stream);
 }
+
+extern "C" int smos_unbalance_block_x3_cl(const float* x, int64_t x_pitch, const void* wa, const float* ba, int64_t kha, int64_t kwa,
+                                          int32_t x3a, const void* wb, const float* bb, int64_t khb, int64_t kwb, int32_t x3b,
+                                          const float* uc, const float* bc, float* both, int64_t both_pitch, float* out,
+                                          int64_t out_pitch, int64_t B, int64_t H, int64_t W, int64_t C, int32_t mb,
+                                          smos_stream_t stream) {
+  SMOS_REQUIRE(x && wa && wb && uc && both && out && both != out && x != both && x != out && both_pitch >= 2 * C,
+               "unbalance_block_x3_cl: null pointer, aliasing maps, or `both` narrower than 2 C channels");
+  auto branch = [&](const void* w, const float* b, int64_t kh, int64_t kw, int32_t x3, float* dst) {
+    if (x3)
+      return smos_conv_bf16x3_cl(x, x_pitch, static_cast<const uint16_t*>(w), b, dst, both_pitch, B, H, W, C, C, (int32_t)kh, (int32_t)kw,
+                                 1, (int32_t)(kh / 2), (int32_t)(kw / 2), 1, stream);
+    return smos_conv_wino1d_cl(x, x_pitch, static_cast<const float*>(w), b, dst, both_pitch, B, H, W, C, C, kh, kw, mb, 1, stream);
+  };
+  if (int rc = branch(wa, ba, kha, kwa, x3a, both)) return rc;
+  if (int rc = branch(wb, bb, khb, kwb, x3b, both + C)) return rc;
+  return smos_conv_wino_cl(both, both_pitch, uc, bc, x, x_pitch, out, out_pitch, B, H, W, 2 * C, C, mb, 1, nullptr, stream);
+}
diff --git a/streammos_amd/csrc/conv_bf16x3.hip b/streammos_amd/csrc/conv_bf16x3.hip
--- /dev/null
+++ b/streammos_amd/csrc/conv_bf16x3.hip
@@ -0,0 +1,397 @@
+#include "conv_common.h"
+
+namespace smos {
+
+typedef __bf16 bf16x8 __attribute__((ext_vector_type(8)));
+
+struct ConvX3Args {
+  const float* x;
+  const u32x4* w;
+  const float* bias;
+  float* out;
+  int64_t xp, op;
+  int B, H, W, Ho, Wo;
+  int KH, KW, S, PH, PW;
+  int ntap, nstage;
+  int wc, rgn, rb;
+  int nq;
+  int nct, hb, xt;
+  int n_items;
+  int rr, cc, n_units;
+  float slope;
+  int x_bytes, o_bytes, w_bytes, cout;
+};
+
+constexpr int kX3PixQ = 12;
+constexpr int x3_units(int mt, int rw) { return mt * rw >= 4 ? 4 : mt * rw == 2 ? 6 : 8; }
+constexpr int x3_wquads(int mt) { return mt == 4 ? 6 : 3; }
+constexpr int kX3BlockQ = 192;
+constexpr int kX3LdsBudget = 80 * 1024;
+
+__device__ __forceinline__ unsigned x3_pack_bf16(float lo, float hi) {
+  unsigned r;
+  asm("v_cvt_pk_bf16_f32 %0, %1, %2" : "=v"(r) : "v"(lo), "v"(hi));
+  return r;
+}
+
+__device__ __forceinline__ void x3_split(unsigned u0, unsigned u1, unsigned& hi, unsigned& mid, unsigned& lo) {
+  const float v0 = __uint_as_float(u0), v1 = __uint_as_float(u1);
+  hi = x3_pack_bf16(v0, v1);
+  float r0 = __fsub_rn(v0, __uint_as_float(hi << 16)), r1 = __fsub_rn(v1, __uint_as_float(hi & 0xffff0000u));
+  mid = x3_pack_bf16(r0, r1);
+  r0 = __fsub_rn(r0, __uint_as_float(mid << 16));
+  r1 = __fsub_rn(r1, __uint_as_float(mid & 0xffff0000u));
+  lo = x3_pack_bf16(r0, r1);
+}
+
+__device__ __forceinline__ int x3_slot(int pix, int limb, int unit) { return pix * kX3PixQ + limb * 4 + (unit ^ ((pix >> 2) & 3)); }
+
+template <int MT, int RW, int KSS>
+__global__ __launch_bounds__(256, 2) void conv_bf16x3(ConvX3Args a) {
+  constexpr int NU = x3_units(MT, RW), WQ = x3_wquads(MT);
+  extern __shared__ __attribute__((aligned(16))) u32x4 lds[];
+  const int G = a.wc * MT;
+  const int piece_q = G * kX3BlockQ;
+  const int slot_q = KSS * piece_q;
+  u32x4* ring = lds;
+  u32x4* region = lds + 2 * slot_q;
+  float* bias_lds = reinterpret_cast<float*>(region + a.rr * a.cc * kX3PixQ);
+  const int tid = threadIdx.x;
+  const int lane = tid & 63, wave = __builtin_amdgcn_readfirstlane(tid >> 6);
+  const int p = lane & 31, h = lane >> 5;
+  const int wcg = wave % a.wc, wr = wave / a.wc;
+  const bool active = wr < a.rgn;
+
+  const int per_block = (a.n_items + (int)gridDim.x - 1) / (int)gridDim.x;
+  const int nb = (int)gridDim.x, xq = nb >> 3, xr = nb & 7, xcd = (int)blockIdx.x & 7;
+  const int lblock = (xcd < xr ? xcd * (xq + 1) : xr * (xq + 1) + (xcd - xr) * xq) + ((int)blockIdx.x >> 3);
+  const int first = lblock * per_block;
+  const int iters = a.n_items - first < per_block ? a.n_items - first : per_block;
+  const int total = iters * a.nstage;
+  if (total <= 0) return;
+
+  struct Item {
+    int b, yb, x0, ct;
+    bool valid;
+  };
+  auto item_of = [&](int it) __attribute__((always_inline)) {
+    Item t;
+    t.valid = it < iters;
+    const int q = t.valid ? first + it : first;
+    t.ct = q % a.nct;
+    int u = q / a.nct;
+    t.x0 = (u % a.xt) * 32;
+    u /= a.xt;
+    t.yb = (u % a.hb) * a.rb;
+    t.b = u / a.hb;
+    return t;
+  };
+
+  const __amdgpu_buffer_rsrc_t xsrd = __builtin_amdgcn_make_buffer_rsrc(const_cast<float*>(a.x), 0, a.x_bytes, 0x00020000);
+  const __amdgpu_buffer_rsrc_t wsrd = __builtin_amdgcn_make_buffer_rsrc(const_cast<u32x4*>(a.w), 0, a.w_bytes, 0x00020000);
+  const __amdgpu_buffer_rsrc_t osrd = __builtin_amdgcn_make_buffer_rsrc(a.out, 0, a.o_bytes, 0x00020000);
+  const __amdgpu_buffer_rsrc_t bsrd =
+      __builtin_amdgcn_make_buffer_rsrc(const_cast<float*>(a.bias), 0, a.bias ? a.cout * 4 : 0, 0x00020000);
+  float bias_r[8];
+#pragma unroll
+  for (int k = 0; k < 8; ++k) bias_r[k] = __uint_as_float(__builtin_amdgcn_raw_buffer_load_b32(bsrd, (unsigned)(tid + 256 * k) * 4u, 0, 0));
+
+  unsigned wvo[WQ];
+#pragma unroll
+  for (int k = 0; k < WQ; ++k) {
+    const int e = tid + 256 * k;
+    const int i = e >= piece_q ? 1 : 0;
+    wvo[k] = e < slot_q ? (unsigned)(i * a.nq * kX3BlockQ + (e - i * piece_q)) * 16u : 0x80000000u;
+  }
+  const int w_step = KSS * a.nq * kX3BlockQ * 16;
+  int pw_s = 0, pw_it = 0;
+  int w_soff = item_of(0).ct * G * kX3BlockQ * 16;
+  auto load_w = [&](u32x4 (&wr_)[WQ]) __attribute__((always_inline)) {
+#pragma unroll
+    for (int k = 0; k < WQ; ++k)
+      if (256 * k < slot_q) wr_[k] = __builtin_amdgcn_raw_buffer_load_b128(wsrd, wvo[k], w_soff, 0);
+    w_soff += w_step;
+    if (++pw_s == a.nstage) {
+      pw_s = 0;
+      if (pw_it + 1 < iters) ++pw_it;
+      w_soff = item_of(pw_it).ct * G * kX3BlockQ * 16;
+    }
+  };
+  auto park = [&](const u32x4 (&wr_)[WQ], int slot) __attribute__((always_inline)) {
+#pragma unroll
+    for (int k = 0; k < WQ; ++k)
+      if (tid + 256 * k < slot_q) ring[slot * slot_q + tid + 256 * k] = wr_[k];
+  };
+
+  int urc[NU];
+#pragma unroll
+  for (int k = 0; k < NU; ++k) {
+    const int u = tid + 256 * k;
+    const int pix = u >> 2;
+    urc[k] = u < a.n_units ? ((pix / a.cc) << 8) | (pix % a.cc) : -1;
+  }
+  u32x4 xr_[2 * NU];
+  auto load_region = [&](int it, int ch) __attribute__((always_inline)) {
+    const Item t = item_of(it);
+    const int y0 = t.yb * a.S - a.PH, x0 = t.x0 * a.S - a.PW;
+    const int xp = (int)a.xp;
+#pragma unroll
+    for (int k = 0; k < NU; ++k) {
+      const int yi = y0 + (urc[k] >> 8), xi = x0 + (urc[k] & 255);
+      const bool ok = t.valid & (urc[k] >= 0) & ((unsigned)yi < (unsigned)a.H) & ((unsigned)xi < (unsigned)a.W);
+      const unsigned off = ok ? (unsigned)(((t.b * a.H + yi) * a.W + xi) * xp + ch * 32 + (tid & 3) * 8) * 4u : 0x80000000u;
+      xr_[2 * k] = __builtin_amdgcn_raw_buffer_load_b128(xsrd, off, 0, 0);
+      xr_[2 * k + 1] = __builtin_amdgcn_raw_buffer_load_b128(xsrd, off + 16u, 0, 0);
+    }
+  };
+  auto write_region = [&]() __attribute__((always_inline)) {
+#pragma unroll
+    for (int k = 0; k < NU; ++k) {
+      const u32x4 lo = xr_[2 * k], hi = xr_[2 * k + 1];
+      unsigned fh[4], fm[4], fl[4];
+      x3_split(lo.x, lo.y, fh[0], fm[0], fl[0]);
+      x3_split(lo.z, lo.w, fh[1], fm[1], fl[1]);
+      x3_split(hi.x, hi.y, fh[2], fm[2], fl[2]);
+      x3_split(hi.z, hi.w, fh[3], fm[3], fl[3]);
+      const int u = tid + 256 * k;
+      if (urc[k] >= 0) {
+        const int s = x3_slot(u >> 2, 0, u & 3);
+        region[s] = u32x4{fh[0], fh[1], fh[2], fh[3]};
+        region[s + 4] = u32x4{fm[0], fm[1], fm[2], fm[3]};
+        region[s + 8] = u32x4{fl[0], fl[1], fl[2], fl[3]};
+      }
+    }
+  };
+
+  f32x16 acc[RW][MT];
+#pragma unroll
+  for (int rw = 0; rw < RW; ++rw)
+#pragma unroll
+    for (int mt = 0; mt < MT; ++mt)
+#pragma unroll
+      for (int r = 0; r < 16; ++r) acc[rw][mt][r] = 0.0f;
+
+  const int nch = a.nstage * KSS / (2 * a.ntap);
+  int c_s = 0, c_it = 0, c_ch = 0, c_ky = 0, c_kx = 0, c_ks = 0;
+  Item cur = item_of(0);
+
+  auto epilogue = [&]() __attribute__((always_inline)) {
+    const int x = cur.x0 + p;
+#pragma unroll
+    for (int rw = 0; rw < RW; ++rw) {
+      const int y = cur.yb + wr * RW + rw;
+      const bool store = (y < a.Ho) & (x < a.Wo);
+      const int pix = (cur.b * a.Ho + y) * a.Wo + x;
+#pragma unroll
+      for (int mt = 0; mt < MT; ++mt) {
+        const int cb = (cur.ct * G + wcg * MT + mt) * 32 + 4 * h;
+        const unsigned ooff = store ? (unsigned)(pix * (int)a.op + cb) * 4u : 0x80000000u;
+#pragma unroll
+        for (int g = 0; g < 4; ++g) {
+          const float4 bv = *reinterpret_cast<const float4*>(bias_lds + cb + 8 * g);
+          const float bb[4] = {bv.x, bv.y, bv.z, bv.w};
+          u32x4 ov;
+#pragma unroll
+          for (int c = 0; c < 4; ++c) {
+            ov[c] = __float_as_uint(conv_act(acc[rw][mt][4 * g + c] + bb[c], a.slope));
+            acc[rw][mt][4 * g + c] = 0.0f;
+          }
+          __builtin_amdgcn_raw_buffer_store_b128(ov, osrd, ooff + 32u * g, 0, 0);
+        }
+      }
+    }
+  };
+
+  auto compute = [&](int slot) __attribute__((always_inline)) {
+    const int pbase = (wr * RW * a.S + c_ky) * a.cc + c_kx + p * a.S;
+#pragma unroll
+    for (int i = 0; i < KSS; ++i) {
+      const int unit = 2 * (c_ks + i) + h;
+      bf16x8 xh[RW], xm[RW], xl[RW], wh[MT], wm[MT], wl[MT];
+#pragma unroll
+      for (int rw = 0; rw < RW; ++rw) {
+        const int s = x3_slot(pbase + rw * a.S * a.cc, 0, unit);
+        xh[rw] = __builtin_bit_cast(bf16x8, region[s]);
+        xm[rw] = __builtin_bit_cast(bf16x8, region[s + 4]);
+        xl[rw] = __builtin_bit_cast(bf16x8, region[s + 8]);
+      }
+      const u32x4* wq = ring + slot * slot_q + i * piece_q + wcg * MT * kX3BlockQ + lane;
+#pragma unroll
+      for (int mt = 0; mt < MT; ++mt) {
+        wl[mt] = __builtin_bit_cast(bf16x8, wq[mt * kX3BlockQ]);
+        wm[mt] = __builtin_bit_cast(bf16x8, wq[mt * kX3BlockQ + 64]);
+        wh[mt] = __builtin_bit_cast(bf16x8, wq[mt * kX3BlockQ + 128]);
+      }
+#define X3_PRODUCT(W_, X_)                                                                                        \
+  _Pragma("unroll") for (int rw = 0; rw < RW; ++rw) _Pragma("unroll") for (int mt = 0; mt < MT; ++mt)             \
+      acc[rw][mt] = __builtin_amdgcn_mfma_f32_32x32x16_bf16(W_[mt], X_[rw], acc[rw][mt], 0, 0, 0)
+      X3_PRODUCT(wh, xl);
+      X3_PRODUCT(wl, xh);
+      X3_PRODUCT(wm, xm);
+      X3_PRODUCT(wh, xm);
+      X3_PRODUCT(wm, xh);
+      X3_PRODUCT(wh, xh);
+#undef X3_PRODUCT
+    }
+  };
+
+  u32x4 wa[WQ], wb[WQ];
+#pragma unroll
+  for (int k = 0; k < WQ; ++k) wa[k] = wb[k] = u32x4{0u, 0u, 0u, 0u};
+  load_w(wa);
+  park(wa, 0);
+  load_w(wa);
+  load_w(wb);
+  load_region(0, 0);
+  write_region();
+#pragma unroll
+  for (int k = 0; k < 8; ++k)
+    if (256 * k + tid < a.cout) bias_lds[tid + 256 * k] = bias_r[k];
+  ring_barrier();
+
+  auto stage = [&](u32x4 (&wn)[WQ], int g) __attribute__((always_inline)) {
+    park(wn, (g + 1) & 1);
+    load_w(wn);
+    const bool chunk_first = (c_ky | c_kx | c_ks) == 0;
+    const bool chunk_last = c_ky == a.KH - 1 && c_kx == a.KW - 1 && c_ks + KSS == 2;
+    const bool item_last = c_s == a.nstage - 1;
+    if (chunk_first) {
+      if (c_ch + 1 < nch) load_region(c_it, c_ch + 1);
+      else load_region(c_it + 1, 0);
+    }
+    if (active) compute(g & 1);
+    if (chunk_last) {
+      ring_barrier();
+      write_region();
+    }
+    if (item_last && active) epilogue();
+    ring_barrier();
+    ++c_s;
+    c_ks += KSS;
+    if (c_ks == 2) {
+      c_ks = 0;
+      if (++c_kx == a.KW) {
+        c_kx = 0;
+        if (++c_ky == a.KH) {
+          c_ky = 0;
+          ++c_ch;
+        }
+      }
+    }
+    if (c_s == a.nstage) {
+      c_s = c_ch = 0;
+      ++c_it;
+      cur = item_of(c_it);
+    }
+  };
+
+  int g = 0;
+#pragma unroll 1
+  for (; g + 2 <= total; g += 2) {
+    stage(wa, g);
+    stage(wb, g + 1);
+  }
+  if (g < total) stage(wa, g);
+}
+
+}
+
+using namespace smos;
+
+namespace {
+
+struct X3Cfg {
+  int mt = 0, wc = 0, rw = 0, rgn = 0, rb = 0, rr = 0, cc = 0, kss = 0;
+  size_t lds = 0;
+};
+
+bool pick_cfg(int64_t Cout, int KH, int KW, int S, X3Cfg* out) {
+  const int64_t nq = Cout / 32;
+  bool found = false;
+  int64_t best_key = -1;
+  for (int mt : {4, 2, 1})
+    for (int wc : {1, 2, 4})
+      for (int rw : {2, 1})
+        for (int kss : {2, 1})
+          for (int idle : {1, 2, 4}) {
+          const int G = mt * wc, rgn = 4 / wc / idle;
+          if (G > 4 || nq % G || mt * rw > 4 || rgn < 1) continue;
+          const int rb = rgn * rw, rr = (rb - 1) * S + KH, cc = 31 * S + KW;
+          if (rr * cc * 4 > 256 * x3_units(mt, rw) || kss * G * kX3BlockQ > 256 * x3_wquads(mt)) continue;
+          const size_t lds = (size_t)(2 * kss * G * kX3BlockQ + rr * cc * kX3PixQ) * 16 + (size_t)Cout * 4;
+          if (lds > (size_t)kX3LdsBudget) continue;
+          const int64_t key = ((((4 - idle) * 8 + G) * 8 + mt) * 4 + rw) * 4 + kss;
+          if (key > best_key) {
+            best_key = key;
+            out->mt = mt; out->wc = wc; out->rw = rw; out->rgn = rgn; out->rb = rb; out->rr = rr; out->cc = cc; out->kss = kss; out->lds = lds;
+            found = true;
+          }
+        }
+  return found;
+}
+
+template <int MT, int RW, int KSS>
+int launch_x3(const ConvX3Args& a, size_t lds, hipStream_t s) {
+  KernelSetup ks;
+  if (int rc = kernel_setup(reinterpret_cast<const void*>(&conv_bf16x3<MT, RW, KSS>), kX3LdsBudget, 0, &ks, "conv_bf16x3_cl"))
+    return rc;
+  const int64_t cap = conv_grid_cap((int64_t)ks.cus * 2);
+  const unsigned grid = (unsigned)(a.n_items < cap ? a.n_items : cap);
+  hipLaunchKernelGGL((conv_bf16x3<MT, RW, KSS>), dim3(grid), dim3(256), lds, s, a);
+  return check_launch("conv_bf16x3_cl");
+}
+
+template <int KSS>
+int dispatch_x3(const ConvX3Args& a, const X3Cfg& c, hipStream_t s) {
+  if (c.mt == 4) return launch_x3<4, 1, KSS>(a, c.lds, s);
+  if (c.mt == 2) return c.rw == 2 ? launch_x3<2, 2, KSS>(a, c.lds, s) : launch_x3<2, 1, KSS>(a, c.lds, s);
+  return c.rw == 2 ? launch_x3<1, 2, KSS>(a, c.lds, s) : launch_x3<1, 1, KSS>(a, c.lds, s);
+}
+
+}
+
+extern "C" int smos_conv_bf16x3_cl_supported(int64_t Cin, int64_t Cout, int32_t KH, int32_t KW, int32_t stride) {
+  if (Cin <= 0 || Cout <= 0 || Cin % 32 || Cout % 32 || Cout > 2048 || KH < 1 || KW < 1 || KH > 7 || KW > 7 ||
+      (stride != 1 && stride != 2))
+    return 0;
+  X3Cfg c;
+  return pick_cfg(Cout, KH, KW, stride, &c) ? 1 : 0;
+}
+
+extern "C" int smos_conv_bf16x3_cl(const float* x, int64_t x_pitch, const uint16_t* wlimbs, const float* bias, float* out,
+                                   int64_t out_pitch, int64_t B, int64_t H, int64_t W, int64_t Cin, int64_t Cout, int32_t KH,
+                                   int32_t KW, int32_t stride, int32_t pad_h, int32_t pad_w, int32_t act, smos_stream_t stream) {
+  SMOS_REQUIRE(B > 0 && H > 0 && W > 0 && Cin > 0 && Cout > 0 && Cin % 32 == 0 && Cout % 32 == 0,
+               "conv_bf16x3_cl: Cin and Cout must be multiples of 32");
+  SMOS_REQUIRE(KH >= 1 && KW >= 1 && KH <= 7 && KW <= 7 && (stride == 1 || stride == 2) && pad_h >= 0 && pad_w >= 0 &&
+                   act >= 0 && act <= 2, "conv_bf16x3_cl: kernel up to 7 x 7, stride 1 or 2");
+  const int64_t Ho = (H + 2 * pad_h - KH) / stride + 1, Wo = (W + 2 * pad_w - KW) / stride + 1;
+  SMOS_REQUIRE(H + 2 * pad_h >= KH && W + 2 * pad_w >= KW && Ho > 0 && Wo > 0, "conv_bf16x3_cl: empty output");
+  ConvBytes nb;
+  if (int rc = conv_check_operands("conv_bf16x3_cl", x, x_pitch, wlimbs, bias, nullptr, 0, out, out_pitch, nullptr, Cin, Cout,
+                                   B * H * W, B * Ho * Wo, &nb))
+    return rc;
+  X3Cfg c;
+  SMOS_REQUIRE(pick_cfg(Cout, KH, KW, stride, &c),
+               "conv_bf16x3_cl: no block shape fits this kernel / stride (smos_conv_bf16x3_cl_supported)");
+  const int64_t nq = Cout / 32, G = c.mt * c.wc;
+  const int64_t hb = (Ho + c.rb - 1) / c.rb, xt = (Wo + 31) / 32, nct = nq / G;
+  SMOS_REQUIRE(B * hb * xt * nct < (1LL << 30) && Cout * Cin * KH * KW * 6 < (1LL << 31), "conv_bf16x3_cl: too many tiles");
+  ConvX3Args a;
+  a.x = x; a.w = reinterpret_cast<const u32x4*>(wlimbs); a.bias = bias; a.out = out;
+  a.xp = x_pitch; a.op = out_pitch;
+  a.B = (int)B; a.H = (int)H; a.W = (int)W; a.Ho = (int)Ho; a.Wo = (int)Wo;
+  a.KH = KH; a.KW = KW; a.S = stride; a.PH = pad_h; a.PW = pad_w;
+  a.ntap = KH * KW; a.nstage = a.ntap * (int)(Cin / 32) * (2 / c.kss);
+  a.wc = c.wc; a.rgn = c.rgn; a.rb = c.rb; a.nq = (int)nq;
+  a.nct = (int)nct; a.hb = (int)hb; a.xt = (int)xt;
+  a.n_items = (int)(B * hb * xt * nct);
+  a.rr = c.rr; a.cc = c.cc; a.n_units = c.rr * c.cc * 4;
+  a.slope = act_slope(act);
+  a.x_bytes = nb.x;
+  a.o_bytes = nb.o;
+  a.w_bytes = (int)(Cout * Cin * KH * KW * 6);
+  a.cout = (int)Cout;
+  const hipStream_t s = (hipStream_t)stream;
+  return c.kss == 2 ? dispatch_x3<2>(a, c, s) : dispatch_x3<1>(a, c, s);
+}
diff --git a/streammos_amd/engine.py b/streammos_amd/engine.py
--- a/streammos_amd/engine.py
+++ b/streammos_amd/engine.py
@@ -69,11 +69,12 @@
         self.plan = None
 
     def run(self, eng, x, out=None):
+        b, c, h, w = x.shape
         if self.plan_ok and _block_call(eng) and eng.wino1d and 2 * x.numel() <= (1 << 26):
             if self.plan is None:
                 self.plan = ops.UnbalanceBlockPlan(self.wa, self.ba, self.wb, self.bb, self.wc, self.bc)
-            return ops.unbalance_block_cl(x, self.plan, out=out)
-        b, c, h, w = x.shape
+            x3 = [eng.conv_x3 and ops.conv_bf16x3_ok(c, c, tuple(wt.shape[2:]), 1, b * h * w) for wt in (self.wa, self.wb)]
+            return ops.unbalance_block_cl(x, self.plan, out=out, x3=x3)
         both = ops.empty_cl(b, 2 * c, h, w, x.device)
         eng._conv(x, self.wa, self.ba, RELU, out=both[:, :c])
         eng._conv(x, self.wb, self.bb, RELU, out=both[:, c:])
@@ -165,6 +166,10 @@
     ("block_call", "SMOS_BLOCK_CALL", True, "bool"),
 )
 
+X3_SWITCHES = (
+    ("conv_x3", "SMOS_CONV_X3", True, "bool"),
+)
+
 TRAIN_SWITCHES = (
     ("seg_loss_own", "SMOS_SEG_LOSS", True, "bool"),
 )
@@ -190,6 +195,8 @@
         self.scratch = scratch.Table()
         self.device = next(net.parameters()).device
         read_switches(self, SWITCHES)
+        read_switches(self, X3_SWITCHES)
+        self.conv_x3 = ops.conv_x3() and not self._bf16
         if self._bf16:
             self.block_call = False
         self.bev_hw = tuple(net.bev_wl_shape)
@@ -410,6 +417,8 @@
             return ops.bias_act_cl(y, bias, act, out=out if out is not None else y, residual=residual)
         b, _, h, wd = x.shape
         ho, wo = (h + 2 * (kh // 2) - kh) // stride + 1, (wd + 2 * (kw // 2) - kw) // stride + 1
+        if self.conv_x3 and ops.conv_bf16x3_ok(cin, cout, (kh, kw), stride, b * ho * wo, residual is not None, chan_sums is not None):
+            return ops.conv_bf16x3_cl(x, layer.operand("x3"), bias, act, cout, (kh, kw), stride=stride, out=out)
         route = ops.conv_route(cin, cout, (kh, kw), stride, b * ho * wo, residual is not None, chan_sums is not None, self)
         family, tile = route
         wp = layer.operand(route)
diff --git a/streammos_amd/ops.py b/streammos_amd/ops.py
--- a/streammos_amd/ops.py
+++ b/streammos_amd/ops.py
@@ -44,6 +44,7 @@
 set_deterministic, set_point_mlp_fused, set_point_head_fused = is_deterministic.set, point_mlp_fused.set, point_head_fused.set
 cross_view_fused = Switch("SMOS_CROSS_VIEW_TRAIN", False)
 set_conv1_fused, set_bilinear_bwd_own, set_cross_view_fused = conv1_fused.set, bilinear_bwd_own.set, cross_view_fused.set
+conv_x3 = Switch("SMOS_CONV_X3", True)
 
 
 def _require_cuda(name, *tensors):
@@ -1169,6 +1170,47 @@
     return out
 
 
+def conv_bf16x3_prepare(w):
+    cout, cin, kh, kw = w.shape
+    if cin % 32 or cout % 32:
+        raise RuntimeError("conv_bf16x3_prepare: Cin %% 32 == 0 and Cout %% 32 == 0 required (got %s)" % (tuple(w.shape),))
+    v = torch.stack(tap_limbs_split(w.detach())).reshape(3, cout // 32, 32, cin // 32, 2, 2, 8, kh, kw)
+    v = v.permute(3, 7, 8, 4, 1, 0, 5, 2, 6)
+    return v.reshape(-1).contiguous()
+
+
+CONV_X3_LAYERS = frozenset({
+    (32, 32, 3, 7, 1), (64, 64, 5, 3, 1), (64, 64, 3, 5, 1), (128, 128, 1, 1, 1),
+})
+
+
+CONV_X3_MIN_PIXELS = 4096
+
+
+def conv_bf16x3_ok(cin, cout, kernel, stride, n_out_pixels, has_residual=False, has_sums=False):
+    return (not has_residual and not has_sums and n_out_pixels >= CONV_X3_MIN_PIXELS and
+            (cin, cout, kernel[0], kernel[1], stride) in CONV_X3_LAYERS)
+
+
+def conv_bf16x3_cl(x, wlimbs, bias, act, cout, kernel, stride=1, padding=None, out=None):
+    b, cin, h, w = x.shape
+    kh, kw = kernel
+    ph, pw = padding if padding is not None else (kh // 2, kw // 2)
+    ho, wo = (h + 2 * ph - kh) // stride + 1, (w + 2 * pw - kw) // stride + 1
+    if wlimbs.dtype != torch.bfloat16 or wlimbs.numel() != 3 * cout * cin * kh * kw:
+        raise RuntimeError("conv_bf16x3_cl: weight block must hold %d bf16 (conv_bf16x3_prepare), got %d %s" %
+                           (3 * cout * cin * kh * kw, wlimbs.numel(), wlimbs.dtype))
+    if x.dtype != torch.float32 or (bias is not None and (bias.dtype != torch.float32 or bias.numel() != cout)):
+        raise RuntimeError("conv_bf16x3_cl: x and bias must be float32 (bias of Cout entries)")
+    if out is not None and out.dtype != torch.float32:
+        raise RuntimeError("conv_bf16x3_cl: out must be float32")
+    out, head = _conv_operands("conv_bf16x3_cl", x, wlimbs, bias, cout, ho, wo, out=out)
+    args = head[:4] + head[6:] + (b, h, w, cin, cout, kh, kw, stride, ph, pw, int(act))
+    _conv_launch("smos_conv_bf16x3_cl", "conv_bf16x3", args, (x, wlimbs, bias, out), x,
+                 lambda: _conv_label("conv_cl", x, cout, ho, wo, kernel))
+    return out
+
+
 _WINO_G = ((1.0, 0.0, 0.0), (0.5, 0.5, 0.5), (0.5, -0.5, 0.5), (0.0, 0.0, 1.0))
 
 
@@ -1230,7 +1272,7 @@
 
 
 class UnbalanceBlockPlan:
-    __slots__ = ("c", "mb", "ptrs_a", "ptrs_b", "ptrs_c", "_keep")
+    __slots__ = ("c", "mb", "ptrs_a", "ptrs_b", "ptrs_c", "_keep", "_branches", "_x3")
 
     def __init__(self, wa, ba, wb, bb, wc, bc):
         c = wa.shape[0]
@@ -1247,9 +1289,20 @@
         self.ptrs_a = (ua.data_ptr(), ba.data_ptr(), ka[0], ka[1])
         self.ptrs_b = (ub.data_ptr(), bb.data_ptr(), kb[0], kb[1])
         self.ptrs_c = (uc.data_ptr(), bc.data_ptr())
-
-
-def unbalance_block_cl(x, plan, both=None, out=None):
+        self._branches, self._x3 = (wa, wb), None
+
+    def x3_ptrs(self, x3):
+        if self._x3 is None:
+            self._x3 = [None, None]
+        out = []
+        for i, (flag, ptrs) in enumerate(zip(x3, (self.ptrs_a, self.ptrs_b))):
+            if flag and self._x3[i] is None:
+                self._x3[i] = conv_bf16x3_prepare(self._branches[i])
+            out.append(((self._x3[i].data_ptr(),) + ptrs[1:] if flag else ptrs) + (int(bool(flag)),))
+        return out
+
+
+def unbalance_block_cl(x, plan, both=None, out=None, x3=(False, False)):
     _require_cuda("unbalance_block_cl", x, both, out)
     b, c, h, w = x.shape
     if c != plan.c:
@@ -1261,8 +1314,11 @@
         out = empty_cl(b, c, h, w, dev)
     if both.shape != (b, 2 * c, h, w) or out.shape != x.shape:
         raise RuntimeError("unbalance_block_cl: both must be [B,2C,H,W] and out have x's shape %s" % (tuple(x.shape),))
+    limbs = bool(x3[0] or x3[1])
+    ptrs_a, ptrs_b = plan.x3_ptrs(x3) if limbs else (plan.ptrs_a, plan.ptrs_b)
     with _on(dev):
-        _lib.call("smos_unbalance_block_cl", x.data_ptr(), _cl("unbalance_block_cl", x), *plan.ptrs_a, *plan.ptrs_b, *plan.ptrs_c,
+        _lib.call("smos_unbalance_block_x3_cl" if limbs else "smos_unbalance_block_cl", x.data_ptr(), _cl("unbalance_block_cl", x),
+                  *ptrs_a, *ptrs_b, *plan.ptrs_c,
                   both.data_ptr(), _cl("unbalance_block_cl", both), out.data_ptr(), _cl("unbalance_block_cl", out), b, h, w, c,
                   plan.mb, _raw_stream(_dev_index(dev)))
     return out
@@ -1905,7 +1961,11 @@
     def operand(self, key):
         wp = self.packed.get(key)
         if wp is None:
-            wp = self.packed[key] = conv_bf16_prepare(self.w) if key == "bf16" else self._PREPARE[key[0]](self.w, key[1])
+            if key == "bf16" or key == "x3":
+                wp = (conv_bf16_prepare if key == "bf16" else conv_bf16x3_prepare)(self.w)
+            else:
+                wp = self._PREPARE[key[0]](self.w, key[1])
+            self.packed[key] = wp
         return wp
 
 
```

Result: no change. 341.7 scans/s (-0.6%).
